# wiedenhoeft/HaMMLET

Hardware: AMD Instinct MI355X
Metric: block-updates/sec (Gibbs sweep) + HBM GB/s, 10^8 pos / 5 states (higher is better)
Workload: dtype f32; 1 GPU; c3_1e8_k5_dynamic; positions=100000000, states=5, block_structure=dynamic, chains=1, parallelism=chain-parallel x1

## Files before the change

### hammlet_amd/capi.py

```python
import ctypes as C
import os

import numpy as np

from . import build as _build

_lib = None


class HmlError(RuntimeError):
    def __init__(self, code, msg):
        super().__init__(msg)
        self.code = code


class HmlStats(C.Structure):
    _fields_ = [("sweeps", C.c_uint64), ("block_updates", C.c_uint64), ("uniform_fallbacks", C.c_uint64),
                ("forward_refits", C.c_uint64), ("forward_serial", C.c_uint64), ("forward_warmup", C.c_uint64),
                ("fused_fallbacks", C.c_uint64), ("buffer_growths", C.c_uint64), ("block_capacity", C.c_uint64)]


RECORD_CB = C.CFUNCTYPE(None, C.c_void_p, C.c_uint64, C.c_void_p)

_P = C.c_void_p
SIGNATURES = {
    "hml_last_error": (C.c_char_p, []),
    "hml_abi_version": (C.c_uint32, []),
    "hml_device_arch": (C.c_char_p, []),
    "hml_device_count": (C.c_int, [C.POINTER(C.c_int)]),
    "hml_create": (C.c_int, [C.POINTER(_P), C.c_int, C.c_uint64, C.c_uint32, _P]),
    "hml_destroy": (None, [_P]),
    "hml_load_observations": (C.c_int, [_P, _P, C.c_uint64]),
    "hml_load_observations_device": (C.c_int, [_P, _P, C.c_uint64]),
    "hml_attach_observations": (C.c_int, [_P, _P]),
    "hml_text_open": (C.c_int, [C.POINTER(_P), C.c_int, C.c_uint64]),
    "hml_text_close": (None, [_P]),
    "hml_text_buffer": (C.c_int, [_P, C.POINTER(_P), C.POINTER(C.c_uint64)]),
    "hml_text_commit": (C.c_int, [_P, C.c_uint64]),
    "hml_text_feed": (C.c_int, [_P, C.c_char_p, C.c_uint64]),
    "hml_text_reserve": (C.c_int, [_P, C.c_uint64]),
    "hml_text_finish": (C.c_int, [_P, C.POINTER(C.c_uint64), C.POINTER(C.c_int)]),
    "hml_text_values": (C.c_int, [_P, _P]),
    "hml_text_counters": (C.c_int, [_P, C.POINTER(C.c_uint64), C.POINTER(C.c_uint64), C.POINTER(C.c_uint64)]),
    "hml_set_dimensions": (C.c_int, [_P, C.c_int, C.c_int]),
    "hml_get_dimensions": (C.c_int, [_P, C.POINTER(C.c_int), C.POINTER(C.c_int)]),
    "hml_set_weights": (C.c_int, [_P, _P, C.c_uint64]),
    "hml_noise_sigma": (C.c_int, [_P, C.POINTER(C.c_double)]),
    "hml_scale_weights": (C.c_int, [_P, C.c_float]),
    "hml_autoprior": (C.c_int, [_P, C.c_float, C.c_float, _P]),
    "hml_set_model": (C.c_int, [_P, C.c_int, _P, C.c_float, C.c_float, C.c_float, C.c_int]),
    "hml_set_self_transitions": (C.c_int, [_P, C.c_int]),
    "hml_sample_prior": (C.c_int, [_P]),
    "hml_set_static_blocks": (C.c_int, [_P]),
    "hml_set_dynamic": (C.c_int, [_P, C.c_int]),
    "hml_create_blocks": (C.c_int, [_P, C.c_float]),
    "hml_iterate": (C.c_int, [_P, C.c_char, C.c_uint64, C.c_uint64]),
    "hml_iterate_many": (C.c_int, [_P, C.c_int, C.c_char, C.c_uint64, C.c_uint64]),
    "hml_set_recording": (C.c_int, [_P, C.c_int, RECORD_CB, _P]),
    "hml_set_option": (C.c_int, [_P, C.c_char_p, C.c_int]),
    "hml_sync": (C.c_int, [_P]),
    "hml_get_num_blocks": (C.c_int, [_P, C.POINTER(C.c_uint64)]),
    "hml_get_blocks": (C.c_int, [_P, _P]),
    "hml_get_block_stats": (C.c_int, [_P, _P, _P]),
    "hml_get_states": (C.c_int, [_P, _P]),
    "hml_get_theta": (C.c_int, [_P, _P]),
    "hml_get_transitions": (C.c_int, [_P, _P, _P]),
    "hml_set_parameters": (C.c_int, [_P, _P, _P, _P]),
    "hml_get_threshold": (C.c_int, [_P, C.POINTER(C.c_float)]),
    "hml_enable_probes": (C.c_int, [_P, C.c_int]),
    "hml_get_block_loglik": (C.c_int, [_P, _P]),
    "hml_get_forward_rows": (C.c_int, [_P, _P]),
    "hml_get_counts": (C.c_int, [_P, _P, _P, _P, _P, _P]),
    "hml_get_weights": (C.c_int, [_P, _P]),
    "hml_get_coefficients": (C.c_int, [_P, _P]),
    "hml_get_integral_array": (C.c_int, [_P, _P, _P]),
    "hml_marginals_rle": (C.c_int, [_P, C.POINTER(C.c_uint64), C.POINTER(C.c_int), _P, _P]),
    "hml_max_segmentation": (C.c_int, [_P, C.POINTER(C.c_uint64), _P, _P]),
    "hml_marginals_dense_device": (C.c_int, [_P, _P, _P]),
    "hml_recorded_sweeps": (C.c_int, [_P, C.POINTER(C.c_uint64)]),
    "hml_set_level_recording": (C.c_int, [_P, C.c_int]),
    "hml_levels_rle": (C.c_int, [_P, C.POINTER(C.c_uint64), C.POINTER(C.c_uint64), _P, _P, _P]),
    "hml_levels_dense_device": (C.c_int, [_P, _P]),
    "hml_levels_merge": (C.c_int, [_P, _P]),
    "hml_levels_on_segments": (C.c_int, [_P, C.c_uint64, _P, _P, _P]),
    "hml_levels_agreement_rle": (C.c_int, [_P, C.c_int, C.POINTER(C.c_uint64), C.POINTER(C.c_uint64), _P, _P, _P, _P]),
    "hml_levels_agreement_dense_device": (C.c_int, [_P, C.c_int, _P]),
    "hml_levels_agreement_summary": (C.c_int, [_P, C.c_int, C.c_double, _P, _P, _P]),
    "hml_set_break_recording": (C.c_int, [_P, C.c_int]),
    "hml_breaks_list": (C.c_int, [_P, C.POINTER(C.c_uint64), C.POINTER(C.c_uint64), _P, _P]),
    "hml_breaks_dense_device": (C.c_int, [_P, _P, C.c_uint32]),
    "hml_breaks_merge": (C.c_int, [_P, _P]),
    "hml_breaks_consensus": (C.c_int, [_P, C.c_uint32, C.c_uint64, C.POINTER(C.c_uint64), _P, _P, _P]),
    "hml_set_level_bands": (C.c_int, [_P, C.c_int, _P]),
    "hml_get_level_bands": (C.c_int, [_P, C.POINTER(C.c_int), _P]),
    "hml_bands_rle": (C.c_int, [_P, C.POINTER(C.c_uint64), C.POINTER(C.c_int), C.POINTER(C.c_uint64), _P, _P]),
    "hml_bands_dense_device": (C.c_int, [_P, _P, C.c_int]),
    "hml_bands_call": (C.c_int, [_P, C.c_uint64, C.POINTER(C.c_uint64), _P, _P]),
    "hml_bands_merge": (C.c_int, [_P, _P]),
    "hml_categorical_draw": (C.c_int, [_P, _P, C.c_int, C.POINTER(C.c_uint32)]),
    "hml_relabel_permutation": (C.c_int, [_P, _P]),
    "hml_pool_payload_size": (C.c_int, [_P, C.POINTER(C.c_uint64)]),
    "hml_pool_export": (C.c_int, [_P, _P, _P]),
    "hml_pool_install": (C.c_int, [_P, _P]),
    "hml_pool_unique_id": (C.c_int, [_P]),
    "hml_pool_create": (C.c_int, [C.POINTER(_P), C.c_int, C.c_int, C.c_int, _P]),
    "hml_pool_destroy": (None, [_P]),
    "hml_pool_marginals": (C.c_int, [_P, _P, _P]),
    "hml_pool_info": (C.c_int, [_P, C.POINTER(C.c_int), C.POINTER(C.c_int), C.POINTER(C.c_double), C.POINTER(C.c_uint64), C.POINTER(C.c_int)]),
    "hml_pool_set_form": (C.c_int, [_P, C.c_int]),
    "hml_pool_last": (C.c_int, [_P, C.POINTER(C.c_int), C.POINTER(C.c_uint64)]),
    "hml_allreduce_marginals": (C.c_int, [_P, C.c_int]),
    "hml_allreduce_marginals_perm": (C.c_int, [_P, C.c_int, _P]),
    "hml_pool_permutation": (C.c_int, [_P, _P]),
    "hml_get_stats": (C.c_int, [_P, C.POINTER(HmlStats)]),
    "hml_profile_enable": (C.c_int, [_P, C.c_int]),
    "hml_profile_get": (C.c_int, [_P, C.c_char_p, C.POINTER(C.c_double), C.POINTER(C.c_uint64)]),
    "hml_debug_eval": (C.c_int, [C.c_int, C.c_int, _P, _P, _P, C.c_uint64, C.c_uint64]),
    "hml_synth_depth": (C.c_int, [_P, _P, C.c_uint64, C.c_double, C.c_double, C.c_uint64, C.c_int]),
    "hml_synth_gauss": (C.c_int, [_P, _P, C.c_uint64, C.c_int, _P, C.c_float, C.c_double, C.c_uint64, C.c_int]),
}


ABI_VERSION = 5


def load_library(path=None):
    global _lib
    if _lib is not None and path is None:
        return _lib
    path = path or os.environ.get("HML_LIBRARY") or _build.LIB_PATH
    if not os.path.exists(path):
        raise HmlError(-1, "%s is missing: build it with `python -c 'import __graft_entry__ as g; g.build()'` "
                           "(hipcc --offload-arch=gfx950); there is no CPU fallback" % path)
    lib = C.CDLL(path, mode=C.RTLD_GLOBAL)
    for name, (res, args) in SIGNATURES.items():
        fn = getattr(lib, name)
        fn.restype = res
        fn.argtypes = args
    if lib.hml_abi_version() != ABI_VERSION:
        raise HmlError(-1, "%s has ABI version %d, this package expects %d: rebuild the library" % (path, lib.hml_abi_version(), ABI_VERSION))
    _lib = lib
    return lib


def _check(rc):
    if rc != 0:
        raise HmlError(rc, load_library().hml_last_error().decode())


def parse_text(source, device=0, chunk_bytes=0, feed_bytes=None, with_info=False):
    lib = load_library()
    h = _P()
    _check(lib.hml_text_open(C.byref(h), device, chunk_bytes))
    try:
        if isinstance(source, (bytes, bytearray, memoryview)):
            data = bytes(source)
            step = feed_bytes or max(len(data), 1)
            for i in range(0, len(data), step):
                part = data[i:i + step]
                _check(lib.hml_text_feed(h, part, len(part)))
        else:
            with open(source, "rb", buffering=0) as f:
                while True:
                    buf, cap = _P(), C.c_uint64()
                    _check(lib.hml_text_buffer(h, C.byref(buf), C.byref(cap)))
                    view = (C.c_char * cap.value).from_address(buf.value)
                    n = f.readinto(view)
                    if not n:
                        break
                    _check(lib.hml_text_commit(h, n))
        n, stopped = C.c_uint64(), C.c_int()
        _check(lib.hml_text_finish(h, C.byref(n), C.byref(stopped)))
        out = np.empty(n.value, np.float32)
        _check(lib.hml_text_values(h, out.ctypes.data))
        if not with_info:
            return out
        a, b, c = C.c_uint64(), C.c_uint64(), C.c_uint64()
        _check(lib.hml_text_counters(h, C.byref(a), C.byref(b), C.byref(c)))
        return out, {"stopped": bool(stopped.value), "bytes": a.value, "irregular_tokens": b.value, "host_chunks": c.value}
    finally:
        lib.hml_text_close(h)


def synth_gauss(T, K, mu, sigma, dwell, seed, nthreads=8, with_states=False):
    lib = load_library()
    x = np.empty(T, np.float32)
    mu = np.ascontiguousarray(mu, np.float32)
    st = np.empty(T, np.int16) if with_states else None
    _check(lib.hml_synth_gauss(x.ctypes.data, st.ctypes.data if with_states else None, T, K, mu.ctypes.data, sigma,
                               dwell, seed, nthreads))
    return (x, st) if with_states else x


def synth_depth(T, depth=15.0, ln_sigma=0.15, seed=5, nthreads=8, with_states=False):
    lib = load_library()
    x = np.empty(T, np.float32)
    st = np.empty(T, np.int16) if with_states else None
    _check(lib.hml_synth_depth(x.ctypes.data, st.ctypes.data if with_states else None, T, depth, ln_sigma, seed, nthreads))
    return (x, st) if with_states else x


def debug_eval(fn, a, b=None, seed=0, device=0):
    lib = load_library()
    a = np.ascontiguousarray(a, np.float32)
    out = np.empty_like(a)
    if b is not None:
        b = np.ascontiguousarray(b, np.float32)
    _check(lib.hml_debug_eval(device, fn, a.ctypes.data, b.ctypes.data if b is not None else None, out.ctypes.data, a.size, seed))
    return out


class Chain:

    def __init__(self, device=0, seed=0, chain_id=0, stream=None):
        self.lib = load_library()
        h = _P()
        _check(self.lib.hml_create(C.byref(h), device, seed, chain_id, stream))
        self.h = h
        self.K = None
        self.T = None
        self.D = 1
        self.P = None
        self._cb = None

    def close(self):
        if self.h:
            self.lib.hml_destroy(self.h)
            self.h = None

    def __del__(self):
        try:
            self.close()
        except Exception:
            pass

    def set_dimensions(self, D, P):
        _check(self.lib.hml_set_dimensions(self.h, D, P))
        self.D, self.P = D, P

    def load(self, x):
        x = np.ascontiguousarray(x, np.float32)
        self.T = int(x.size) // self.D
        _check(self.lib.hml_load_observations(self.h, x.ctypes.data, x.size))

    def load_device(self, ptr, T):
        self.T = int(T)
        _check(self.lib.hml_load_observations_device(self.h, ptr, T))

    def attach(self, source):
        _check(self.lib.hml_attach_observations(self.h, source.h))
        self.T, self.D, self.P = source.T, source.D, source.P

    def noise_sigma(self):
        v = C.c_double()
        _check(self.lib.hml_noise_sigma(self.h, C.byref(v)))
        return v.value

    def scale_weights(self, m):
        _check(self.lib.hml_scale_weights(self.h, m))

    def set_weights(self, w):
        w = np.ascontiguousarray(w, np.float32)
        _check(self.lib.hml_set_weights(self.h, w.ctypes.data, w.size))

    def autoprior(self, s2=0.2, p=0.9):
        out = np.empty(4, np.float32)
        _check(self.lib.hml_autoprior(self.h, s2, p, out.ctypes.data))
        return out

    def set_model(self, K, nig4, a_off=0.5, a_diag=0.5, pi_alpha=0.5, self_trans=True):
        nig4 = np.ascontiguousarray(nig4, np.float32)
        self.K = K
        _check(self.lib.hml_set_model(self.h, K, nig4.ctypes.data, a_off, a_diag, pi_alpha, 1 if self_trans else 0))

    def sample_prior(self):
        _check(self.lib.hml_sample_prior(self.h))

    def set_self_transitions(self, on=True):
        _check(self.lib.hml_set_self_transitions(self.h, 1 if on else 0))

    def set_static_blocks(self):
        _check(self.lib.hml_set_static_blocks(self.h))

    def set_dynamic(self, on=True):
        _check(self.lib.hml_set_dynamic(self.h, 1 if on else 0))

    def create_blocks(self, thr):
        _check(self.lib.hml_create_blocks(self.h, thr))

    def iterate(self, method, iterations, thinning=0):
        _check(self.lib.hml_iterate(self.h, method.encode()[0:1], iterations, thinning))

    def set_recording(self, marginals=True, callback=None):
        if callback is not None:
            def tramp(_ctx, sweep, _user):
                callback(self, sweep)
            self._cb = RECORD_CB(tramp)
        else:
            self._cb = C.cast(None, RECORD_CB)
        _check(self.lib.hml_set_recording(self.h, 1 if marginals else 0, self._cb, None))

    def set_option(self, name, value):
        _check(self.lib.hml_set_option(self.h, name.encode(), int(value)))

    def sync(self):
        _check(self.lib.hml_sync(self.h))

    def num_blocks(self):
        v = C.c_uint64()
        _check(self.lib.hml_get_num_blocks(self.h, C.byref(v)))
        return v.value

    def blocks(self):
        B = self.num_blocks()
        s = np.empty(B + 1, np.uint32)
        _check(self.lib.hml_get_blocks(self.h, s.ctypes.data))
        return s

    def block_stats(self):
        B = self.num_blocks()
        a = np.empty((self.D, B), np.float32)
        b = np.empty((self.D, B), np.float32)
        _check(self.lib.hml_get_block_stats(self.h, a.ctypes.data, b.ctypes.data))
        return (a[0], b[0]) if self.D == 1 else (a, b)

    def states(self):
        B = self.num_blocks()
        q = np.empty(B, np.int16)
        _check(self.lib.hml_get_states(self.h, q.ctypes.data))
        return q

    def theta(self):
        t = np.empty(2 * (self.P or self.K), np.float32)
        _check(self.lib.hml_get_theta(self.h, t.ctypes.data))
        return t

    def transitions(self):
        A = np.empty((self.K, self.K), np.float32)
        pi = np.empty(self.K, np.float32)
        _check(self.lib.hml_get_transitions(self.h, A.ctypes.data, pi.ctypes.data))
        return A, pi

    def set_parameters(self, mean_var, A, pi):
        mv = np.ascontiguousarray(mean_var, np.float32)
        A = np.ascontiguousarray(A, np.float32)
        pi = np.ascontiguousarray(pi, np.float32)
        _check(self.lib.hml_set_parameters(self.h, mv.ctypes.data, A.ctypes.data, pi.ctypes.data))

    def threshold(self):
        v = C.c_float()
        _check(self.lib.hml_get_threshold(self.h, C.byref(v)))
        return v.value

    def enable_probes(self, on=True):
        _check(self.lib.hml_enable_probes(self.h, 1 if on else 0))

    def block_loglik(self):
        B = self.num_blocks()
        E = np.empty((B, self.K), np.float32)
        _check(self.lib.hml_get_block_loglik(self.h, E.ctypes.data))
        return E

    def forward_rows(self):
        B = self.num_blocks()
        r = np.empty((B + 1, self.K), np.float32)
        _check(self.lib.hml_get_forward_rows(self.h, r.ctypes.data))
        return r

    def counts(self):
        K = self.K
        trans = np.empty((K, K), np.uint64)
        occ = np.empty(K, np.uint64)
        s = np.empty(K, np.float32)
        q = np.empty(K, np.float32)
        n = np.empty(K, np.uint64)
        _check(self.lib.hml_get_counts(self.h, trans.ctypes.data, occ.ctypes.data, s.ctypes.data, q.ctypes.data, n.ctypes.data))
        return trans, occ, s, q, n

    def weights(self):
        w = np.empty(self.T, np.float32)
        _check(self.lib.hml_get_weights(self.h, w.ctypes.data))
        return w

    def coefficients(self):
        w = np.empty(self.T, np.float32)
        _check(self.lib.hml_get_coefficients(self.h, w.ctypes.data))
        return w

    def integral_array(self):
        a = np.empty(self.T + 1, np.float32)
        b = np.empty(self.T + 1, np.float32)
        _check(self.lib.hml_get_integral_array(self.h, a.ctypes.data, b.ctypes.data))
        return a, b

    def recorded_sweeps(self):
        v = C.c_uint64()
        _check(self.lib.hml_recorded_sweeps(self.h, C.byref(v)))
        return v.value

    def marginals_rle(self):
        n = C.c_uint64()
        k = C.c_int()
        _check(self.lib.hml_marginals_rle(self.h, C.byref(n), C.byref(k), None, None))
        seg = np.empty(n.value, np.uint64)
        cnt = np.empty((n.value, max(k.value, 0)), np.int32)
        _check(self.lib.hml_marginals_rle(self.h, C.byref(n), C.byref(k), seg.ctypes.data, cnt.ctypes.data if k.value else None))
        return seg, cnt

    def max_segmentation(self):
        n = C.c_uint64()
        _check(self.lib.hml_max_segmentation(self.h, C.byref(n), None, None))
        ln = np.empty(n.value, np.uint64)
        st = np.empty(n.value, np.int32)
        _check(self.lib.hml_max_segmentation(self.h, C.byref(n), ln.ctypes.data, st.ctypes.data))
        return ln, st

    def marginals_dense_device(self, out_ptr, perm=None):
        p = None
        if perm is not None:
            perm = np.ascontiguousarray(perm, np.int32)
            p = perm.ctypes.data
        _check(self.lib.hml_marginals_dense_device(self.h, out_ptr, p))

    def set_level_recording(self, on=True):
        _check(self.lib.hml_set_level_recording(self.h, 1 if on else 0))

    def levels_rle(self):
        m, n = C.c_uint64(), C.c_uint64()
        _check(self.lib.hml_levels_rle(self.h, C.byref(m), C.byref(n), None, None, None))
        seg = np.empty(m.value, np.uint64)
        s1 = np.empty((self.D, m.value), np.float64)
        s2 = np.empty((self.D, m.value), np.float64)
        _check(self.lib.hml_levels_rle(self.h, C.byref(m), C.byref(n), seg.ctypes.data, s1.ctypes.data, s2.ctypes.data))
        return seg, n.value, s1, s2

    def levels_dense_device(self, out_ptr):
        _check(self.lib.hml_levels_dense_device(self.h, out_ptr))

    def merge_levels(self, other):
        _check(self.lib.hml_levels_merge(self.h, other.h))

    def levels_on_segments(self, cuts):
        cuts = np.ascontiguousarray(cuts, np.uint32)
        n = cuts.size
        s1 = np.empty((self.D, n + 1), np.float64)
        s2 = np.empty((self.D, n + 1), np.float64)
        _check(self.lib.hml_levels_on_segments(self.h, n, cuts.ctypes.data if n else None, s1.ctypes.data, s2.ctypes.data))
        return s1, s2

    def set_break_recording(self, on=True):
        _check(self.lib.hml_set_break_recording(self.h, 1 if on else 0))

    def breaks_list(self):
        m, n = C.c_uint64(), C.c_uint64()
        _check(self.lib.hml_breaks_list(self.h, C.byref(m), C.byref(n), None, None))
        pos = np.empty(m.value, np.uint32)
        cnt = np.empty(m.value, np.uint32)
        if m.value:
            _check(self.lib.hml_breaks_list(self.h, C.byref(m), C.byref(n), pos.ctypes.data, cnt.ctypes.data))
        return pos, cnt, n.value

    def breaks_dense(self, out_ptr, window=0):
        _check(self.lib.hml_breaks_dense_device(self.h, out_ptr, window))

    def breaks_merge(self, other):
        _check(self.lib.hml_breaks_merge(self.h, other.h))

    def breaks_consensus(self, window, min_count):
        s = C.c_uint64()
        _check(self.lib.hml_breaks_consensus(self.h, window, min_count, C.byref(s), None, None, None))
        pos = np.empty(s.value, np.uint32)
        mass = np.empty(s.value, np.uint64)
        peak = np.empty(s.value, np.uint32)
        if s.value:
            _check(self.lib.hml_breaks_consensus(self.h, window, min_count, C.byref(s), pos.ctypes.data, mass.ctypes.data, peak.ctypes.data))
        return pos, mass, peak

    def set_level_bands(self, edges):
        edges = np.ascontiguousarray(edges, np.float32)
        _check(self.lib.hml_set_level_bands(self.h, edges.size, edges.ctypes.data if edges.size else None))

    def level_bands(self):
        n = C.c_int()
        edges = np.zeros(31, np.float32)
        _check(self.lib.hml_get_level_bands(self.h, C.byref(n), edges.ctypes.data))
        return edges[:n.value].copy()

    def bands_rle(self):
        m, ncol, n = C.c_uint64(), C.c_int(), C.c_uint64()
        _check(self.lib.hml_bands_rle(self.h, C.byref(m), C.byref(ncol), C.byref(n), None, None))
        seg = np.empty(m.value, np.uint64)
        cnt = np.empty((m.value, ncol.value), np.int32)
        _check(self.lib.hml_bands_rle(self.h, C.byref(m), C.byref(ncol), C.byref(n), seg.ctypes.data, cnt.ctypes.data))
        return seg, cnt, n.value

    def bands_dense_device(self, out_ptr, cumulative=False):
        _check(self.lib.hml_bands_dense_device(self.h, out_ptr, 1 if cumulative else 0))

    def bands_call(self, rank=0):
        r = C.c_uint64()
        _check(self.lib.hml_bands_call(self.h, rank, C.byref(r), None, None))
        ln = np.empty(r.value, np.uint64)
        band = np.empty((self.D, r.value), np.int32)
        _check(self.lib.hml_bands_call(self.h, rank, C.byref(r), ln.ctypes.data, band.ctypes.data))
        return ln, band

    def merge_bands(self, other):
        _check(self.lib.hml_bands_merge(self.h, other.h))

    def relabel_permutation(self):
        perm = np.empty(self.K, np.int32)
        _check(self.lib.hml_relabel_permutation(self.h, perm.ctypes.data))
        return perm

    def pool_payload_size(self):
        n = C.c_uint64()
        _check(self.lib.hml_pool_payload_size(self.h, C.byref(n)))
        return n.value

    def pool_export(self, payload_ptr):
        perm = np.empty(self.K, np.int32)
# ... 197 lines not shown
```

### hammlet_amd/csrc/hml_capi.hip

```cpp
#include "hml_capi_shared.hpp"

static thread_local std::string g_err;
int hml_set_err(int code, const std::string& msg) { g_err = msg; return code; }

static const hml_ktab* ktab(int K);
#define HML_KTAB(KV, tab) const hml_ktab* tab = ktab(KV); if (!tab) return set_err(HML_ERR_ARG, "number of states must be in [2,16]")

std::atomic<int> hml_live_ctx[64];
int hml_ctx_bind(hml_ctx* c) { return ctx_bind(c); }
int hml_ctx_fetch_model(hml_ctx* c, hml_model* out) { return fetch_model(c, out); }

HML_KERNEL void hml_k_debug_eval(int fn, const float* __restrict__ a, const float* __restrict__ b, float* __restrict__ out,
                                 uint64_t n, uint64_t seed) {
    if (fn == 24) {
        const uint64_t nw = ((uint64_t)gridDim.x * blockDim.x) >> 6;
        if ((threadIdx.x & 63) != 0) return;
        for (uint64_t i = ((uint64_t)blockIdx.x * blockDim.x + threadIdx.x) >> 6; i < n; i += nw) {
            hml_dev_src src;
            src.s = hml_stream_open(hml_make_key(seed, 0), HML_KIND_THETA, seed, (uint32_t)i);
            out[i] = hml_gamma_f32<hml_devmath>(src, a[i], b[i]);
        }
        return;
    }
    const uint64_t stride = (uint64_t)gridDim.x * blockDim.x;
// ... 3 lines not shown
        switch (fn) {
            case 0: r = hml_expf(x); break;
            case 1: r = hml_logf(x); break;
            case 2: r = hml_powf_unit(x, y); break;
            case 3: r = HML_SQRTF(x); break;
            case 4: r = x / y; break;
            case 5: {
                hml_dev_src src;
                src.s = hml_stream_open(hml_make_key(seed, 0), HML_KIND_THETA, seed, (uint32_t)i);
                r = hml_gamma_f32<hml_devmath>(src, x, y);
            } break;
            case 6: {
                hml_dev_src src;
                src.s = hml_stream_open(hml_make_key(seed, 0), HML_KIND_PI, seed, (uint32_t)i);
                hml_normal_f32<hml_devmath> nd;
                r = nd.draw(src, x, y);
            } break;
            case 7: r = (float)hml_log((double)x); break;
            case 8: r = (float)hml_exp_nonpos((double)x); break;
            case 9: r = (float)((double)x / (double)y); break;
            case 40: r = hml_glibc_expf(x); break;
            case 41: r = hml_glibc_logf(x); break;
            case 42: r = hml_glibc_powf_unit(x, y); break;
            case 43: { const double Zd = (double)y; r = hml_tr2_quotient(x, Zd, hml_tr2_reciprocal(Zd)); } break;
            case 10: r = (float)(1.0 / (double)x); break;
            case 12: case 13: case 14: case 15: case 16: case 17: case 18: case 19: case 20: case 21: case 22: case 23: {
                hml_dev_src src; src.s = hml_stream_open(hml_make_key(seed, 0), HML_KIND_THETA, seed, (uint32_t)i);
                const float alpha = x, beta = y; (void)beta;
                const float malpha = alpha < 1.0f ? alpha + 1.0f : alpha;
                const float a1 = malpha - 1.0f / 3.0f;
                const float a2 = 1.0f / hml_devmath::sqrtf_(9.0f * a1);
                hml_normal_f32<hml_devmath> nd;
                float n = nd.draw(src, 0.0f, 1.0f);
                float v = 1.0f + a2 * n;
                float v3 = v * v * v;
                float u = hml_canonical_f32(src);
                const bool c1 = (double)u > (double)1.0f - 0.0331 * (double)n * (double)n * (double)n * (double)n;
                const bool c2 = ((double)hml_devmath::logf_(u) > (0.5 * (double)n * (double)n + (double)a1 * ((1.0 - (double)v3) + (double)hml_devmath::logf_(v3))));
                float n2 = nd.draw(src, 0.0f, 1.0f);
                float vb = 1.0f + a2 * n2;
                float vb3 = vb * vb * vb;
                float ub = hml_canonical_f32(src);
                const bool d1 = (double)ub > (double)1.0f - 0.0331 * (double)n2 * (double)n2 * (double)n2 * (double)n2;
                const bool d2 = ((double)hml_devmath::logf_(ub) > (0.5 * (double)n2 * (double)n2 + (double)a1 * ((1.0 - (double)vb3) + (double)hml_devmath::logf_(vb3))));
                r = fn == 12 ? n : fn == 13 ? v3 : fn == 14 ? u : fn == 15 ? (float)(c1 ? 1 : 0) + 2.0f * (c2 ? 1 : 0) : fn == 16 ? n2 : fn == 17 ? a2
                    : fn == 18 ? vb3 : fn == 19 ? ub : fn == 20 ? (float)(d1 ? 1 : 0) + 2.0f * (d2 ? 1 : 0) : fn == 21 ? (float)src.s.n : 0.0f;
                if (fn == 22) r = nd.draw(src, 0.0f, 1.0f);
                if (fn == 23) { hml_normal_f32<hml_devmath> nf; r = nf.draw(src, 0.0f, 1.0f); r = nf.draw(src, 0.0f, 1.0f); }
            } break;
            case 30: case 31: {
                r = 0.0f;
                const int Kc = fn == 30 ? 16 : 5;
                if (i % Kc == 0 && i + Kc <= n) {
                    bool unsure = false;
                    int fastr, lit;
                    if (fn == 30) { float w[16]; for (int j = 0; j < 16; ++j) w[j] = a[i + j]; fastr = hml_categorical_k_fast<16>(w, (double)y, unsure); lit = hml_categorical_k_literal<16>(w, (double)y); if (unsure) fastr = lit; }
                    else { float w[5]; for (int j = 0; j < 5; ++j) w[j] = a[i + j]; fastr = hml_categorical_k_fast<5>(w, (double)y, unsure); lit = hml_categorical_k_literal<5>(w, (double)y); if (unsure) fastr = lit; }
                    out[i] = (float)fastr; out[i + 1] = (float)lit; out[i + 2] = unsure ? 1.0f : 0.0f;
                }
                continue;
            }
            case 11: { const double d = HML_SQRT((double)x * 1.0000001); r = (float)((d - (double)(float)d) * 1e9); } break;
        }
        out[i] = r;
    }
}

static bool parse_band_edges(const char* text, int* n, float* edges) {
    *n = 0;
    const char* p = text;
    while (*p) {
        char* end = nullptr;
        const float v = strtof(p, &end);
        if (end == p || *n >= HML_MAX_BAND_EDGES) return false;
        edges[(*n)++] = v;
        p = end;
        if (*p == ',') ++p; else if (*p) return false;
    }
    return *n > 0;
}

static const char* band_edges_fault(int n, const float* edges) {
    if (n < 1 || n > HML_MAX_BAND_EDGES) return "level bands take 1 to 31 edges";
    for (int j = 0; j < n; ++j) {
        if (!std::isfinite(edges[j])) return "the edges of the level bands must be finite";
        if (j > 0 && !(edges[j - 1] < edges[j])) return "the edges of the level bands must be strictly ascending";
    }
    return nullptr;
}

static int bands_from_env(hml_ctx* c) {
    if (const char* e = getenv("HML_BANDS")) {
        int n = 0; float edges[HML_MAX_BAND_EDGES];
        if (!parse_band_edges(e, &n, edges)) return set_err(HML_ERR_ARG, "HML_BANDS: expected up to 31 comma-separated numbers");
        if (const char* why = band_edges_fault(n, edges)) return set_err(HML_ERR_ARG, std::string("HML_BANDS: ") + why);
        c->n_band_edges = n;
        memcpy(c->band_edges, edges, (size_t)n * sizeof(float));
        c->rec[HML_REC_BANDS].on = c->rec[HML_REC_BANDS].asked = true;
    }
    return 0;
}

extern "C" {

const char* hml_last_error(void) { return g_err.c_str(); }
uint32_t hml_abi_version(void) { return 5; }
const char* hml_device_arch(void) { return "gfx950"; }
int hml_device_count(int* n) {
    if (!n) return set_err(HML_ERR_ARG, "null argument");
    HIPCHK(hipGetDeviceCount(n));
    return 0;
}

static void free_all(hml_ctx* c);

static int create_inner(hml_ctx* c, void* stream) {
    HIPCHK(hipSetDevice(c->device));
    if (stream) { c->stream = (hipStream_t)stream; c->own_stream = false; }
    else { HIPCHK(hipStreamCreateWithFlags(&c->stream, hipStreamNonBlocking)); c->own_stream = true; }
    HIPCHK(hipMalloc(&c->d_mdl, sizeof(hml_model)));
    HIPCHK(hipMemsetAsync(c->d_mdl, 0, sizeof(hml_model), c->stream));
    HIPCHK(hipHostMalloc(&c->h_B, 4 * sizeof(uint32_t), hipHostMallocMapped));
    c->h_B[0] = 0; c->h_B[1] = 0; c->h_B[2] = 0; c->h_B[3] = 0;
    HIPCHK(hipHostGetDevicePointer((void**)&c->d_hB, c->h_B, 0));
    return 0;
}

int hml_create(hml_ctx** out, int device, uint64_t seed, uint32_t chain_id, void* stream) {
    if (!out) return set_err(HML_ERR_ARG, "null output pointer");
    int n = 0;
    HIPCHK(hipGetDeviceCount(&n));
    if (n <= 0) return set_err(HML_ERR_HIP, "no HIP device available: the MI355X kernels cannot run (there is no CPU fallback)");
    if (device < 0 || device >= n) return set_err(HML_ERR_ARG, "device index out of range");
    hml_ctx* c = new hml_ctx();
    c->device = device; c->seed = seed; c->chain = chain_id;
    if (int r = create_inner(c, stream)) {
        free_all(c);
        if (c->own_stream && c->stream) hipStreamDestroy(c->stream);
        delete c;
        return r;
    }
    if (const char* e = getenv("HML_FWD_CHUNK")) { int l = std::max(1, atoi(e)); int sh = 0; while ((1 << (sh + 1)) <= l && sh < 10) ++sh; c->fwdL = 1 << sh; }
    if (const char* e = getenv("HML_FWD_WARMUP")) c->fwdW = c->fwdW_init = std::max(0, atoi(e));
    if (const char* e = getenv("HML_FWD_BURNIN_SWEEPS")) c->fwd_burnin_sweeps = (uint32_t)std::max(0, atoi(e));
    if (const char* e = getenv("HML_FWD_QUIET")) c->fwd_quiet_need = (uint32_t)std::max(1, atoi(e));
    if (const char* e = getenv("HML_FWD_CHUNK_MANY")) { int l = std::max(1, atoi(e)); int sh = 0; while ((1 << (sh + 1)) <= l && sh < 6) ++sh; c->fwdL_many = 1 << sh; }
    if (const char* e = getenv("HML_FWD_CHUNK_MID")) { int l = std::max(1, atoi(e)); int sh = 0; while ((1 << (sh + 1)) <= l && sh < 10) ++sh; c->fwdL_mid = 1 << sh; }
    if (const char* e = getenv("HML_MID_MIN_BLOCKS")) c->mid_min_blocks = (uint32_t)strtoul(e, nullptr, 10);
    if (const char* e = getenv("HML_FWD_CHUNK_DENSE")) { int l = std::max(1, atoi(e)); int sh = 0; while ((1 << (sh + 1)) <= l && sh < 10) ++sh; c->fwdL_dense = 1 << sh; }
    if (const char* e = getenv("HML_DENSE_MIN_BLOCKS")) c->dense_min_blocks = (uint32_t)strtoul(e, nullptr, 10);
    if (const char* e = getenv("HML_USE_GRAPH")) c->use_graph = atoi(e) != 0;
    if (const char* e = getenv("HML_WEIGHT_KEYS")) c->use_keys = atoi(e) != 0;
    if (const char* e = getenv("HML_FUSED_BLOCKS")) { c->fused_blocks = atoi(e) != 0; c->fused_keep = atoi(e) == 2; }
    if (const char* e = getenv("HML_TRELLIS_FUSED")) c->tre_fused = atoi(e) != 0;
    if (const char* e = getenv("HML_TRELLIS_L")) { const int l = atoi(e); c->tre_L = (l <= 0) ? 0u : (l >= HML_TRE_MAX_L) ? (uint32_t)HML_TRE_MAX_L : (l < 32) ? 32u : (uint32_t)l / 32u * 32u; }
    if (const char* e = getenv("HML_TRELLIS_CKPT")) c->tre_ckpt = atoi(e) != 0;
    if (const char* e = getenv("HML_TRELLIS_REFIT_ROUNDS")) { const int r = atoi(e); c->tre_refit_rounds = r < 0 ? 0u : r > 6 ? 6u : (uint32_t)r; }
    if (const char* e = getenv("HML_STAGE_BITS")) c->stage_bits = atoi(e) != 0;
    if (const char* e = getenv("HML_TRELLIS_ROWS")) c->tre_rows = atoi(e) != 0;
    if (const char* e = getenv("HML_LATE_RESCALE")) c->late_rescale = atoi(e) != 0;
    if (const char* e = getenv("HML_PARAMS_SPREAD")) c->params_spread = atoi(e) != 0;
    if (const char* e = getenv("HML_COMPAT_CHUNKS")) c->compat_chunks = atoi(e);
    if (const char* e = getenv("HML_COMPAT_WARMUP")) c->compat_warmup = atoi(e);
    if (const char* e = getenv("HML_WIDE_LANES")) c->wide_lanes = atoi(e);
    if (const char* e = getenv("HML_WIDE_W0")) c->wide_w0 = std::max(8, atoi(e));
    if (const char* e = getenv("HML_WIDE_MAX_CHUNKS")) c->wide_max_chunks = (uint32_t)std::max(64, atoi(e));
    if (const char* e = getenv("HML_WIDE_L")) {
        const int L = atoi(e);
        if (L >= 1) { int sh = 0; while ((1 << sh) < L && sh < 20) ++sh; c->wide_lshift = sh; }
    }
    if (const char* e = getenv("HML_COMPAT")) c->compat = atoi(e) != 0;
    if (const char* e = getenv("HML_TRELLIS_TUNE")) c->tre_autotune = atoi(e) != 0;
    if (const char* e = getenv("HML_FUSED_SPIN_LIMIT")) c->fused_spin_limit = (uint32_t)strtoul(e, nullptr, 10);
    if (const char* e = getenv("HML_LEVELS")) c->rec[HML_REC_LEVELS].on = c->rec[HML_REC_LEVELS].asked = atoi(e) != 0;
    if (const char* e = getenv("HML_BREAKS")) c->rec[HML_REC_BREAKS].on = c->rec[HML_REC_BREAKS].asked = atoi(e) != 0;
    if (const char* e = getenv("HML_MAX_BLOCKS")) c->cap_opt = strtoull(e, nullptr, 10);
    if (device < 64) g_live_ctx[device].fetch_add(1);
    if (int r = bands_from_env(c)) { hml_destroy(c); return r; }
    *out = c;
    return 0;
}

static void trace_release(hml_ctx* c) {
    if (c->trace) {
        if (c->trace->refs.fetch_sub(1) == 1) {
            void* ptrs[] = {c->trace->d_w, c->trace->d_summary, c->trace->d_coeff, c->trace->d_ia};
            for (void* p : ptrs) if (p) hipFree(p);
            delete c->trace;
        }
        c->trace = nullptr;
    } else {
        void* ptrs[] = {c->d_w, c->d_summary, c->d_coeff, c->d_ia};
        for (void* p : ptrs) if (p) hipFree(p);
    }
    c->d_w = nullptr; c->d_summary = nullptr; c->d_coeff = nullptr; c->d_ia = nullptr;
}
static bool trace_shared(const hml_ctx* c) { return c->trace && c->trace->refs.load() > 1; }

static void free_sweep_buffers(hml_ctx* c, bool keep_engine = false) {
    void** ptrs[] = {(void**)&c->d_em, (void**)&c->d_gsc, (void**)&c->d_rows, (void**)&c->d_entry, (void**)&c->d_exitA, (void**)&c->d_redo, (void**)&c->d_touched,
                     (void**)&c->d_fb, (void**)&c->d_smap, (void**)&c->d_cmap, (void**)&c->d_scmap, (void**)&c->d_super, (void**)&c->d_bentry2, (void**)&c->d_bentry,
                     (void**)&c->d_q, (void**)&c->d_partial, (void**)&c->d_redo2, (void**)&c->d_tre_bitmap, (void**)&c->d_tre_ckpt, (void**)&c->d_crows, (void**)&c->d_cchunk, (void**)&c->d_cdraws, (void**)&c->d_clists, (void**)&c->d_wacc, (void**)&c->d_wA};
    for (void** p : ptrs) if (*p) { hipFree(*p); *p = nullptr; }
    if (!keep_engine && c->d_mt) { hipFree(c->d_mt); c->d_mt = nullptr; }
}

static void free_all(hml_ctx* c) {
    trace_release(c);
    free_sweep_buffers(c);
    void* ptrs[] = {c->d_group_word, c->d_wave_total, c->d_stage, c->d_span_count, c->d_starts, c->d_bstat, c->d_eprobe, c->d_aprobe, c->d_coarse1,
                    c->d_diff, c->d_boundary, c->d_mdl, c->d_many};
    for (void* p : ptrs) if (p) hipFree(p);
    for (hml_recorder& r : c->rec) { if (r.d_acc) hipFree(r.d_acc); if (r.d_boundary) hipFree(r.d_boundary); }
    if (c->h_B) hipHostFree(c->h_B);
    c->h_B = nullptr;
}


void hml_destroy(hml_ctx* c) {
    if (!c) return;
    if (c->device < 64) g_live_ctx[c->device].fetch_sub(1);
    hipSetDevice(c->device);
    hipStreamSynchronize(c->stream);
    for (auto& kv : c->prof) for (auto& p : kv.second.pending) { hipEventDestroy(p.first); hipEventDestroy(p.second); }
    for (auto e : c->ev_pool) hipEventDestroy(e);
    if (c->graph_exec) hipGraphExecDestroy(c->graph_exec);
    free_all(c);
    if (c->own_stream) hipStreamDestroy(c->stream);
    delete c;
}

static int build_keys(hml_ctx* c) {
    if (!c->use_keys) return 0;
    const uint64_t T = c->T;
    if (!c->d_summary) {
        const uint64_t n_spans = (T + HML_SPAN - 1) / HML_SPAN;
        HIPCHK(hipMalloc(&c->d_summary, n_spans * (HML_SPAN / 16) + 16));
        HIPCHK(hipMemsetAsync(c->d_summary, 0, n_spans * (HML_SPAN / 16) + 16, c->stream));
    }
    const float thr0 = (float)(std::sqrt(2 * std::log((double)std::max<uint64_t>(T, 2))) * c->sigma * c->key_scale);
    uint32_t u; memcpy(&u, &thr0, 4);
    c->key_base = (std::isfinite(thr0) && thr0 > 0 ? (int32_t)(u >> 20) : (int32_t)(0x3f800000u >> 20)) - 128;
    hipLaunchKernelGGL(hml_k_build_summary, dim3(grid_for((T + 15) / 16, 256, 1, 65536)), dim3(256), 0, c->stream, c->d_w, T,
                       c->key_base, c->d_summary);
    KLAUNCH_CHECK();
    return 0;
}

HML_KERNEL void hml_k_max_inplace(float* __restrict__ a, const float* __restrict__ b, uint64_t n) {
    const uint64_t stride = (uint64_t)gridDim.x * blockDim.x;
    for (uint64_t i = (uint64_t)blockIdx.x * blockDim.x + threadIdx.x; i < n; i += stride) { const float x = a[i], y = b[i]; a[i] = (x < y) ? y : x; }
}

static int alloc_block_buffers(hml_ctx* c) {
    const uint64_t T = c->T;
    c->n_spans = (uint32_t)((T + HML_SPAN - 1) / HML_SPAN);
    HIPCHK(hipMalloc(&c->d_stage, (uint64_t)c->n_spans * HML_SPAN * sizeof(uint16_t)));
    HIPCHK(hipMalloc(&c->d_span_count, c->n_spans * sizeof(uint32_t)));
    HIPCHK(hipMalloc(&c->d_starts, (c->cap + 1) * sizeof(uint32_t)));
    HIPCHK(hipMalloc(&c->d_coarse1, ((c->n_spans + HML_GROUP_SPANS - 1) / HML_GROUP_SPANS + 1u) * sizeof(uint32_t)));
    {
        const uint64_t n_tiles = (T + HML_FUSED_SUB_POSITIONS - 1) / HML_FUSED_SUB_POSITIONS;
        HIPCHK(hipMalloc(&c->d_group_word, (n_tiles + 1) * sizeof(unsigned long long)));
        HIPCHK(hipMemsetAsync(c->d_group_word, 0, (n_tiles + 1) * sizeof(unsigned long long), c->stream));
        HIPCHK(hipMalloc(&c->d_wave_total, (n_tiles + 1) * (HML_FUSED_WAVES + 2) * sizeof(uint32_t)));
        if (getenv("HML_FUSED_DEBUG")) { HIPCHK(hipMalloc(&c->d_dbg, 4096 * 8 * 8)); HIPCHK(hipMemset(c->d_dbg, 0, 4096 * 8 * 8)); }
    }
    HIPCHK(hipMalloc(&c->d_bstat, c->cap * (uint64_t)c->D * sizeof(float2)));
    const uint32_t cap32 = (uint32_t)c->cap;
    HIPCHK(hipMemcpyAsync(&c->d_mdl->cap, &cap32, sizeof cap32, hipMemcpyHostToDevice, c->stream));
    return 0;
}

static void choose_capacity(hml_ctx* c, bool attached) {
    const uint64_t T = c->T;
    uint64_t cap = T;
    if (c->D == 1) {
        if (c->cap_opt) cap = c->cap_opt;
        else if (attached) cap = std::max<uint64_t>(1ull << 20, T / 16);
    }
    c->cap = std::min<uint64_t>(std::max<uint64_t>(cap, 64), T);
}

static int build_from_device_x(hml_ctx* c, const float* const* d_x, const float* const* h_x) {
    const uint64_t T = c->T;
    const int D = c->D;
    {
        trace_release(c);
        void** stale[] = {(void**)&c->d_stage, (void**)&c->d_span_count, (void**)&c->d_starts, (void**)&c->d_coarse1, (void**)&c->d_group_word, (void**)&c->d_wave_total, (void**)&c->d_bstat};
        for (void** q : stale) if (*q) { hipFree(*q); *q = nullptr; }
    }
    {
        const float sqrt2 = (float)std::sqrt(2.0);
        const float sqrt2half = (float)(sqrt2 / 2.0);
        double acc = 0; uint64_t cnt = 0;
        for (uint64_t i = 1; i < T; i += 2) {
            float mx = 0.0f;
            for (int d = 0; d < D; ++d) {
                const float df = std::abs(h_x[d][i - 1] - h_x[d][i]);
                const float cf = sqrt2half * df;
                mx = (mx < cf) ? cf : mx;
            }
            acc += mx;
            cnt++;
        }
        acc /= cnt;
// ... 633 lines not shown
        hipLaunchKernelGGL(HIP_KERNEL_NAME(hml_k_compat_backward<KC, PAD>), dim3(C), dim3(64), 0, s, c->d_mdl, c->d_crows, c->d_cdraws, c->d_q, ch);
        if (C > 1u) hipLaunchKernelGGL(HIP_KERNEL_NAME(hml_k_compat_backward_check<KC, PAD>), dim3(1), dim3(256), 0, s, c->d_mdl, c->d_crows, c->d_cdraws, c->d_q, ch, C);
    }
}

static int sweep_compat(hml_ctx* c, char method, bool record) {
    hipStream_t s = c->stream;
    if (c->dynamic || !c->blocks_valid) {
        if (int r = launch_compact(c, false, 0.0f)) return r;
        if (!c->dynamic) c->blocks_valid = true;
    }
    refresh_hint(c);
    const uint32_t hint = c->B_hint ? c->B_hint : (uint32_t)std::min<uint64_t>(c->T, 1u << 20);
    const int mix = method == HML_METHOD_MIXTURE ? 1 : 0;
    hml_mt_state* const mt = (hml_mt_state*)c->d_mt;
    hipLaunchKernelGGL(HIP_KERNEL_NAME(hml_k_compat_emission<hml_glibc_exp>), dim3(grid_for(hint, 256, 64, 16384)), dim3(256), 0, s, c->d_mdl, c->d_starts, c->d_bstat, c->d_em, c->d_gsc, mix,
                       c->probes ? c->d_eprobe : nullptr);
    if (mix) hipLaunchKernelGGL(hml_k_compat_mixture, dim3(1), dim3(64), 0, s, c->d_mdl, mt, c->d_em, c->d_q);
    else {
        float* const aprobe = c->probes ? c->d_aprobe : nullptr;
        uint32_t C = 1u;
        if (!c->probes && c->compat_chunks > 1) C = std::min<uint32_t>((uint32_t)c->compat_chunks, HML_COMPAT_MAX_CHUNKS);
        else if (!c->probes && c->compat_chunks == 0 && hint >= 8192u) C = std::min<uint32_t>((uint32_t)HML_COMPAT_MAX_CHUNKS, hint / 64u);
        hml_compat_chunks ch = chunk_views(c);
        ch.W = c->compat_warmup > 0 ? (uint32_t)c->compat_warmup : c->compat_warmup < 0 ? 0u : HML_CHUNK_W_ADAPTIVE;
        hipLaunchKernelGGL(hml_k_compat_draws, dim3(1), dim3(256), 0, s, c->d_mdl, mt, c->d_cdraws, 2u);
#define HML_COMPAT_FB(KC) case KC: launch_chunked_fb<KC, hml_glibc_exp, false>(c, s, C, ch, aprobe); break;
        switch (c->K <= HML_MAX_K ? c->K : 0) {
            HML_COMPAT_FB(2) HML_COMPAT_FB(3) HML_COMPAT_FB(4) HML_COMPAT_FB(5) HML_COMPAT_FB(6) HML_COMPAT_FB(7) HML_COMPAT_FB(8) HML_COMPAT_FB(9)
            HML_COMPAT_FB(10) HML_COMPAT_FB(11) HML_COMPAT_FB(12) HML_COMPAT_FB(13) HML_COMPAT_FB(14) HML_COMPAT_FB(15) HML_COMPAT_FB(16)
            default:
                if (c->K <= 32) launch_chunked_fb<32, hml_glibc_exp, true>(c, s, C, ch, aprobe);
                else launch_chunked_fb<64, hml_glibc_exp, true>(c, s, C, ch, aprobe);
        }
#undef HML_COMPAT_FB
    }
    hml_compat_lists pl;
    {
        const uint64_t tiles = (c->cap + HML_COMPAT_PART_TILE - 1) / HML_COMPAT_PART_TILE;
        char* base = (char*)c->d_clists;
        pl.sx = (float*)base; base += compat_list_entries(c) * sizeof(float);
        pl.sq = (float*)base; base += compat_list_entries(c) * sizeof(float);
        pl.n = (uint32_t*)base; base += compat_list_entries(c) * sizeof(uint32_t);
        pl.offdiag = (unsigned long long*)base; base += (uint64_t)HML_CAP_K * HML_CAP_K * sizeof(unsigned long long);
        pl.tile_count = (uint32_t*)base; base += tiles * c->K * sizeof(uint32_t);
        pl.state_off = (uint32_t*)base;
    }
    const int by_state = (c->D == 1 && c->T < (1ull << 31) && (c->compat_chunks > 1 || (c->compat_chunks == 0 && hint >= 8192u))) ? 1 : 0;
    if (by_state) {
        const unsigned tiles_now = (unsigned)(((uint64_t)hint + hint / 8 + HML_COMPAT_PART_TILE) / HML_COMPAT_PART_TILE);
        const unsigned tg = std::min<uint64_t>(std::max(1u, tiles_now), (c->cap + HML_COMPAT_PART_TILE - 1) / HML_COMPAT_PART_TILE);
        hipLaunchKernelGGL(hml_k_compat_part_count, dim3(tg), dim3(256), 0, s, c->d_mdl, c->d_q, pl);
        hipLaunchKernelGGL(hml_k_compat_part_scan, dim3(1), dim3(64), 0, s, c->d_mdl, pl);
        hipLaunchKernelGGL(hml_k_compat_part_scatter, dim3(tg), dim3(256), 0, s, c->d_mdl, c->d_q, c->d_starts, c->d_bstat, pl);
    }
    hipLaunchKernelGGL(hml_k_compat_update, dim3(1), dim3(by_state ? 256 : 64), 0, s, c->d_mdl, mt, c->d_starts, c->d_bstat, c->d_q, mix, pl, by_state);
    if (record && c->rec_marginals) {
        if (c->pooled) return set_err(HML_ERR_ARG, "the marginals of this context are pooled (common labels, several chains): further sweeps cannot be recorded into them");
        if (int r = ensure_marginal_buffers(c)) return r;
        hipLaunchKernelGGL(hml_k_record, dim3(grid_for(hint, 256, 64, 16384)), dim3(256), 0, s, c->d_q, c->d_starts, c->d_mdl, c->d_diff, c->d_boundary);
    }
    if (record) { if (int r = launch_recorders(c, s, hint)) return r; }
    KLAUNCH_CHECK();
    return 0;
}

static int sweep_wide(hml_ctx* c, char method, bool record) {
    hipStream_t s = c->stream;
    if (c->dynamic || !c->blocks_valid) {
        if (int r = launch_compact(c, false, 0.0f)) return r;
        if (!c->dynamic) c->blocks_valid = true;
    }
    refresh_hint(c);
    const uint32_t hint = c->B_hint ? c->B_hint : (uint32_t)std::min<uint64_t>(c->T, 1u << 20);
    const int mix = method == HML_METHOD_MIXTURE ? 1 : 0;
    const bool lanes = c->wide_lanes != 0 && !c->probes && !mix && c->compat_chunks == 0;
    if (lanes) {
        hml_compat_chunks ch = chunk_views(c);
        ch.W = c->compat_warmup > 0 ? (uint32_t)c->compat_warmup : c->compat_warmup < 0 ? 0u : HML_CHUNK_W_ADAPTIVE;
        const uint64_t room = (uint64_t)hint + hint / 4 + 1024;
        hipLaunchKernelGGL(hml_k_wl_prepare, dim3(1), dim3(256), 0, s, c->d_mdl, c->d_wA, c->wide_lshift, wide_max_chunks_of(c));
        hipLaunchKernelGGL(hml_k_wl_gtable, dim3(grid_for((uint64_t)c->K * HML_WL_GTAB, 256, 1, 512)), dim3(256), 0, s, c->d_mdl, c->d_wA + HML_WL_PITCH * HML_WL_PITCH);
        {
            ProfScope ps(c, "stats_emission");
            hipLaunchKernelGGL(hml_k_wl_emission, dim3(grid_for(room, 64 * HML_WL_EMIT_ROWS * 4, 1, 32768)), dim3(256), 0, s, c->d_mdl, c->d_starts, c->d_bstat, c->d_em, c->d_gsc, c->d_wA + HML_WL_PITCH * HML_WL_PITCH);
        }
        const uint64_t minL = c->wide_lshift >= 0 ? (1ull << c->wide_lshift) : (1ull << HML_WL_MIN_LSHIFT);
        const int tiles = grid_for(room, (int)std::min<uint64_t>(64 * minL, 1u << 30), 1, HML_WL_MAX_CHUNKS / 64);
#define HML_WL_FB(KC)                                                                                                                                   \
        case KC: {                                                                                                                                      \
            constexpr int KS = (KC <= 32) ? 32 : 64;                                                                                                    \
            {                                                                                                                                           \
                ProfScope ps(c, "forward");                                                                                                             \
                hipLaunchKernelGGL(HIP_KERNEL_NAME(hml_k_wl_forward<KC>), dim3(tiles), dim3(64), 0, s, c->d_mdl, c->d_wA, c->d_em, c->d_gsc, c->d_crows, ch, 0); \
                hipLaunchKernelGGL(hml_k_wl_forward_verify, dim3(grid_for(room / 16 * c->K, 256, 1, 4096)), dim3(256), 0, s, c->d_mdl, ch, 0);          \
                                      \
                hipLaunchKernelGGL(hml_k_wl_retry_decide, dim3(1), dim3(256), 0, s, c->d_mdl, ch);                                                      \
                hipLaunchKernelGGL(HIP_KERNEL_NAME(hml_k_wl_forward<KC>), dim3(tiles), dim3(64), 0, s, c->d_mdl, c->d_wA, c->d_em, c->d_gsc, c->d_crows, ch, 1); \
                hipLaunchKernelGGL(hml_k_wl_forward_verify, dim3(grid_for(room / 16 * c->K, 256, 1, 4096)), dim3(256), 0, s, c->d_mdl, ch, 1);          \
                hipLaunchKernelGGL(HIP_KERNEL_NAME(hml_k_wl_forward_check<KS>), dim3(1), dim3(256), 0, s, c->d_mdl, c->d_em, c->d_gsc, c->d_crows, ch);  \
            }                                                                                                                                           \
            {                                                                                                                                           \
                ProfScope ps(c, "backward_maps");                                                                                                       \
                hipLaunchKernelGGL(HIP_KERNEL_NAME(hml_k_wl_backward<KC>), dim3(tiles), dim3(64), 0, s, c->d_mdl, c->d_crows, c->d_q, ch);               \
                hipLaunchKernelGGL(hml_k_wl_backward_verify, dim3(grid_for(room / 16, 256, 1, 256)), dim3(256), 0, s, c->d_mdl, ch);                     \
                hipLaunchKernelGGL(HIP_KERNEL_NAME(hml_k_wl_backward_check<KS>), dim3(1), dim3(256), 0, s, c->d_mdl, c->d_crows, c->d_q, ch);          \
            }                                                                                                                                           \
        } break;
        switch ((c->K + 3) / 4 * 4) {
            HML_WL_FB(4) HML_WL_FB(8) HML_WL_FB(12) HML_WL_FB(16)
            HML_WL_FB(20) HML_WL_FB(24) HML_WL_FB(28) HML_WL_FB(32) HML_WL_FB(36) HML_WL_FB(40) HML_WL_FB(44) HML_WL_FB(48) HML_WL_FB(52) HML_WL_FB(56)
            HML_WL_FB(60) HML_WL_FB(64)
            default: return set_err(HML_ERR_HIP, "internal error: a model of this many states on the path for more than 16");
        }
#undef HML_WL_FB
    } else {
    {
        ProfScope ps(c, "stats_emission");
        hipLaunchKernelGGL(hml_k_wide_emission, dim3(grid_for(hint, 256, 1, 4096)), dim3(256), 0, s, c->d_mdl, c->d_starts, c->d_bstat,
                           c->d_em, c->d_gsc, mix, c->probes ? c->d_eprobe : nullptr);
    }
    if (mix) hipLaunchKernelGGL(hml_k_wide_mixture, dim3(grid_for(hint, 256, 1, 16384)), dim3(256), 0, s, c->d_mdl, c->d_em, c->d_q);
    else {
        float* const aprobe = c->probes ? c->d_aprobe : nullptr;
        uint32_t C = 1u;
        if (!c->probes && c->compat_chunks > 1) C = std::min<uint32_t>((uint32_t)c->compat_chunks, HML_COMPAT_MAX_CHUNKS);
        else if (!c->probes && c->compat_chunks == 0 && hint >= 2048u) C = std::min<uint32_t>((uint32_t)HML_COMPAT_MAX_CHUNKS, hint / 64u);
        hml_compat_chunks ch = chunk_views(c);
        ch.W = c->compat_warmup > 0 ? (uint32_t)c->compat_warmup : c->compat_warmup < 0 ? 0u : HML_CHUNK_W_ADAPTIVE;
        hipLaunchKernelGGL(hml_k_wide_uniforms, dim3(grid_for((hint + 1u) / 2u, 256, 1, 4096)), dim3(256), 0, s, c->d_mdl, c->d_cdraws);
        if (c->K <= 32) launch_chunked_fb<32, hml_dev_exp, true>(c, s, C, ch, aprobe);
        else launch_chunked_fb<64, hml_dev_exp, true>(c, s, C, ch, aprobe);
    }
    }
    {
        ProfScope ps(c, "counts");
        hipLaunchKernelGGL(hml_k_wide_counts, dim3(HML_REDUCE_GROUPS), dim3(256), 0, s, c->d_q, c->d_starts, c->d_bstat, c->d_mdl, c->d_partial, (hml_wide_acc*)c->d_wacc);
    }
    if (record && c->rec_marginals) {
        if (c->pooled) return set_err(HML_ERR_ARG, "the marginals of this context are pooled (common labels, several chains): further sweeps cannot be recorded into them");
        if (int r = ensure_marginal_buffers(c)) return r;
        hipLaunchKernelGGL(hml_k_record, dim3(grid_for(hint, 256, 64, 16384)), dim3(256), 0, s, c->d_q, c->d_starts, c->d_mdl, c->d_diff, c->d_boundary);
    }
    {
        ProfScope ps(c, "params");
        hipLaunchKernelGGL(hml_k_wide_params, dim3(1), dim3(1024), 0, s, c->d_mdl, c->d_partial, (hml_wide_acc*)c->d_wacc, 0);
    }
    if (record) { if (int r = launch_recorders(c, s, hint)) return r; }
    KLAUNCH_CHECK();
    return 0;
}

static int sweep_dispatch(hml_ctx* c, char method, bool record) {
    if (c->compat) return sweep_compat(c, method, record);
    if (c->wide) return sweep_wide(c, method, record);
    HML_KTAB(c->K, kt);
    return kt->sweep(c, method, record);
}

extern "C" {

int hml_iterate(hml_ctx* c, char method, uint64_t iterations, uint64_t thinning) {
    if (!c || !c->model_set) return set_err(HML_ERR_ARG, "model not set");
    if (method != HML_METHOD_FB && method != HML_METHOD_MIXTURE)
        return set_err(HML_ERR_ARG, std::string("Unknown sampling type ") + method + "!");
    if (int r = ctx_bind(c)) return r;
    c->call_base = c->requested;
    if (thinning > 0 && thinning <= iterations && c->rec_marginals && c->pooled)
        return set_err(HML_ERR_ARG, "the marginals of this context are pooled (common labels, several chains): further sweeps cannot be recorded into them");
    for (uint64_t i = 0; i < iterations; ++i) {
        const bool record = thinning > 0 && ((i + 1) % thinning == 0);
        if (chain_halted(c)) { if (int r = hml_settle(c)) return r; }
        refresh_hint(c);
        const bool tre_path = c->tre_fused && c->D == 1 && method == HML_METHOD_FB && c->B_hint >= c->dense_min_blocks;
        if (c->use_graph && !c->compat && !record && !c->profiling && !c->probes && (c->dynamic || c->blocks_valid) &&
            !(tre_path && tre_wants_measurement(c, c->B_hint))) {
            const uint32_t hint = c->B_hint;
            bool unused = false;
            const bool wants_fused = c->fused_blocks && !(c->h_B[1] && !c->fused_keep) && !shares_device(c);
            const bool stale = !c->graph_exec || c->graph_method != method || c->graph_dynamic != c->dynamic ||
                               hint > c->graph_hint || hint * 2u < c->graph_hint || c->graph_fused != wants_fused ||
                               c->graph_dense != (hint >= c->dense_min_blocks) || c->graph_mid != (hint >= c->mid_min_blocks) ||
                               (tre_path && c->graph_tre_L != tre_pick_L(c, hint, true, &unused));
            if (stale && hint) {
                if (c->graph_exec) { hipGraphExecDestroy(c->graph_exec); c->graph_exec = nullptr; }
                hipGraph_t g = nullptr;
                HIPCHK(hipStreamBeginCapture(c->stream, hipStreamCaptureModeThreadLocal));
                int rr = sweep_dispatch(c, method, false);
                const hipError_t ec = hipStreamEndCapture(c->stream, &g);
                if (rr || ec != hipSuccess) {
                    if (g) hipGraphDestroy(g);
                    (void)hipGetLastError();
                    return rr ? rr : set_err(HML_ERR_HIP, std::string("hipStreamEndCapture: ") + hipGetErrorString(ec));
                }
                const hipError_t ei = hipGraphInstantiate(&c->graph_exec, g, nullptr, nullptr, 0);
                hipGraphDestroy(g);
                if (ei != hipSuccess) { c->graph_exec = nullptr; return set_err(HML_ERR_HIP, std::string("hipGraphInstantiate: ") + hipGetErrorString(ei)); }
                c->graph_method = method; c->graph_dynamic = c->dynamic; c->graph_hint = c->B_hint; c->graph_fused = wants_fused;
                c->graph_dense = c->B_hint >= c->dense_min_blocks;
                c->graph_mid = c->B_hint >= c->mid_min_blocks;
            }
            if (c->graph_exec) {
                log_sweep(c, method, false);
                HIPCHK(hipGraphLaunch(c->graph_exec, c->stream));
                if (tre_path) c->tre_dense_sweeps++;
                continue;
            }
        }
        log_sweep(c, method, record);
        if (int r = sweep_dispatch(c, method, record)) return r;
        if (record && c->cb) {
            HIPCHK(hipStreamSynchronize(c->stream));
            if (chain_halted(c)) { if (int r = hml_settle(c)) return r; continue; }
            if (int r = check_device_error(c)) return r;
            c->cb(c, i, c->cb_user);
        }
    }
    return 0;
}

}

extern "C" int hml_iterate_many(hml_ctx* const* cs, int n, char method, uint64_t iterations, uint64_t thinning) {
    if (!cs || n < 1) return set_err(HML_ERR_ARG, "no contexts");
    for (int i = 0; i < n; ++i) if (!cs[i] || !cs[i]->model_set) return set_err(HML_ERR_ARG, "model not set");
    if (method != HML_METHOD_FB && method != HML_METHOD_MIXTURE) return set_err(HML_ERR_ARG, std::string("Unknown sampling type ") + method + "!");
    for (int i = 0; i < n; ++i) cs[i]->call_base = cs[i]->requested;
    uint64_t done = 0;
    while (done < iterations && many_eligible(cs, n, method)) {
        if (int r = ctx_bind(cs[0])) return r;
        for (int i = 0; i < n; ++i) {
            hml_ctx* c = cs[i];
            if (int r = settle_if_limited(c)) return r;
            if (c->hint_stale) { launch_compact_pair(c, 0, 0.0f); KLAUNCH_CHECK(); }
            HIPCHK(hipStreamSynchronize(c->stream));
            c->hint_stale = false;
            if (c->graph_exec) { hipGraphExecDestroy(c->graph_exec); c->graph_exec = nullptr; }
        }
        int r = 0;
        uint64_t reached = done;
        { HML_KTAB(cs[0]->K, kt); r = kt->iterate_many(cs, n, done, iterations, thinning, &reached); }
        if (r) return r;
        hipEvent_t ev = ev_get(cs[0]);
        HIPCHK(hipEventRecord(ev, cs[0]->stream));
        for (int i = 1; i < n; ++i) HIPCHK(hipStreamWaitEvent(cs[i]->stream, ev, 0));
        cs[0]->ev_pool.push_back(ev);
        if (reached == iterations) return 0;
        HIPCHK(hipStreamSynchronize(cs[0]->stream));
        bool halted = false;
        for (int i = 0; i < n; ++i) halted = halted || chain_halted(cs[i]);
        const bool progress = reached > done;
        done = reached;
        if (!halted && !progress) break;
        if (!halted) { bool sparse = true; for (int i = 0; i < n; ++i) sparse = sparse && many_sparse(cs[i]); if (!sparse) break; }
    }
    for (int i = 0; i < n; ++i) if (int r = settle_if_limited(cs[i])) return r;
    for (uint64_t i = done; i < iterations; ++i) {
        const bool record = thinning > 0 && ((i + 1) % thinning == 0);
        for (int k = 0; k < n; ++k) {
            hml_ctx* c = cs[k];
            if (int r = ctx_bind(c)) return r;
            if (record && c->rec_marginals && c->pooled) return set_err(HML_ERR_ARG, "the marginals of a context are pooled (common labels, several chains): further sweeps cannot be recorded into them");
            if (chain_halted(c)) { if (int r = hml_settle(c)) return r; }
            log_sweep(c, method, record);
            if (int r = sweep_dispatch(c, method, record)) return r;
            if (record && c->cb) {
                HIPCHK(hipStreamSynchronize(c->stream));
                if (chain_halted(c)) { if (int r = hml_settle(c)) return r; continue; }
                if (int r = check_device_error(c)) return r;
                c->cb(c, i, c->cb_user);
            }
        }
    }
    return 0;
}

extern "C" {

int hml_set_option(hml_ctx* c, const char* name, int value) {
    if (!c || !name) return set_err(HML_ERR_ARG, "null argument");
    if (std::string(name) == "weight_keys") {
        if (c->loaded) return set_err(HML_ERR_ARG, "weight_keys must be set before the observations are loaded");
        c->use_keys = value != 0;
        c->summary_always = value == 2;
        return 0;
    }
    if (std::string(name) == "max_blocks") {
        if (c->loaded) return set_err(HML_ERR_ARG, "max_blocks must be set before the observations are loaded");
        if (value < 0) return set_err(HML_ERR_ARG, "max_blocks: a number of blocks, or 0 for the default");
        c->cap_opt = (uint64_t)value;
        return 0;
    }
    if (std::string(name) == "fused_blocks") {
        c->fused_blocks = value != 0;
        c->fused_keep = value == 2;
        if (c->graph_exec) { hipGraphExecDestroy(c->graph_exec); c->graph_exec = nullptr; }
        return 0;
    }
    if (std::string(name) == "compat") {
        if (c->model_set) return set_err(HML_ERR_ARG, "compat must be set before the model");
        c->compat = value != 0;
        return 0;
    }
    if (std::string(name) == "trellis_L") {
        if (value < 0 || value > HML_TRE_MAX_L || value % 32) return set_err(HML_ERR_ARG, "trellis_L: 0 or a multiple of 32 up to 1024");
        c->tre_L = (uint32_t)value;
        return 0;
    }
    return set_err(HML_ERR_ARG, std::string("unknown option ") + name);
}

int hml_sync(hml_ctx* c) {
    if (!c) return set_err(HML_ERR_ARG, "null context");
    if (int r = ctx_bind(c)) return r;
    if (int r = hml_settle(c)) return r;
    if (c->d_dbg && getenv("HML_FUSED_DEBUG") && atoi(getenv("HML_FUSED_DEBUG")) == 2) {
        std::vector<unsigned long long> h(4096 * 8);
        hipMemcpy(h.data(), c->d_dbg, h.size() * 8, hipMemcpyDeviceToHost);
        uint32_t n = 0; while (n < 4096 && h[n * 8]) ++n;
        unsigned long long t0 = ~0ull; for (uint32_t i = 0; i < n; ++i) t0 = std::min(t0, h[i * 8]);
        double mx[5] = {0, 0, 0, 0, 0}, av[5] = {0, 0, 0, 0, 0};
        if (n) for (uint32_t i = 0; i < n; ++i) for (int k = 0; k < 5; ++k) { const double d = (double)(h[i * 8 + k] - t0) * 0.01; mx[k] = std::max(mx[k], d); av[k] += d / n; }
        if (n) fprintf(stderr, "[fused-many dbg] n=%u start avg %.2f max %.2f | phaseA avg %.2f max %.2f | requested avg %.2f max %.2f | offsets avg %.2f max %.2f | end avg %.2f max %.2f (us)\n",
                n, av[0], mx[0], av[1], mx[1], av[2], mx[2], av[3], mx[3], av[4], mx[4]);
        if (n) for (uint32_t i : {0u, n / 4, n / 2, n - 1}) if (i < n) fprintf(stderr, "   wg %u: %.2f %.2f %.2f %.2f %.2f | wavefront 0: parameters in LDS %.2f, weights arrived %.2f, its lists done %.2f\n", i, (h[i*8]-t0)*0.01, (h[i*8+1]-t0)*0.01, (h[i*8+2]-t0)*0.01, (h[i*8+3]-t0)*0.01, (h[i*8+4]-t0)*0.01,
                                                                                  (h[i*8+5]-t0)*0.01, (h[i*8+6]-t0)*0.01, (h[i*8+7]-t0)*0.01);
    } else if (c->d_dbg) {
        std::vector<unsigned long long> h(4096 * 4);
        hipMemcpy(h.data(), c->d_dbg, h.size() * 8, hipMemcpyDeviceToHost);
        const uint32_t n = (uint32_t)std::min<uint64_t>(4096, (c->T + HML_FUSED_SUB_POSITIONS - 1) / HML_FUSED_SUB_POSITIONS);
        unsigned long long t0 = ~0ull; for (uint32_t i = 0; i < n; ++i) if (h[i * 4]) t0 = std::min(t0, h[i * 4]);
        double mx[4] = {0, 0, 0, 0}, av[4] = {0, 0, 0, 0};
        for (uint32_t i = 0; i < n; ++i) for (int k = 0; k < 4; ++k) { const double d = (double)(h[i * 4 + k] - t0) * 0.01; mx[k] = std::max(mx[k], d); av[k] += d / n; }
        fprintf(stderr, "[fused dbg] n=%u start avg %.2f max %.2f | phaseA avg %.2f max %.2f | offsets avg %.2f max %.2f | end avg %.2f max %.2f (us)\n", n, av[0], mx[0], av[1], mx[1], av[2], mx[2], av[3], mx[3]);
        { uint32_t late = 0, first_late = n; for (uint32_t i = 0; i < n; ++i) if ((h[i * 4] - t0) * 0.01 > 2.0) { ++late; first_late = std::min(first_late, i); }
          fprintf(stderr, "   late starters: %u, first index %u\n", late, first_late); }
        for (uint32_t i : {0u, n / 4, n / 2, n - 1}) fprintf(stderr, "   wg %u: %.2f %.2f %.2f %.2f\n", i, (h[i*4]-t0)*0.01, (h[i*4+1]-t0)*0.01, (h[i*4+2]-t0)*0.01, (h[i*4+3]-t0)*0.01);
    }
    if (c->model_set && getenv("HML_PARAMS_DEBUG")) {
        hml_model m;
        if (fetch_model(c, &m) == 0) {
            fprintf(stderr, "[params dbg] us since the kernel's start: accumulators read %.2f | tree %.2f | theta drawn %.2f | A gammas %.2f | barrier %.2f | end %.2f\n",
                    (m.dbg_t[1] - m.dbg_t[0]) * 0.01, (m.dbg_t[2] - m.dbg_t[0]) * 0.01, (m.dbg_t[3] - m.dbg_t[0]) * 0.01, (m.dbg_t[4] - m.dbg_t[0]) * 0.01,
                    (m.dbg_t[5] - m.dbg_t[0]) * 0.01, (m.dbg_t[6] - m.dbg_t[0]) * 0.01);
            fprintf(stderr, "[params dbg]   theta's gamma core + normal drawn %.2f | last wavefront's tree %.2f\n", (m.dbg_t[7] - m.dbg_t[0]) * 0.01, (m.dbg_t[8] - m.dbg_t[0]) * 0.01);
        }
    }
    if (c->model_set) return check_device_error(c);
    return 0;
}


static int current_B(hml_ctx* c, uint32_t* B) {
    HIPCHK(hipMemcpyAsync(c->h_B, &c->d_mdl->B, sizeof(uint32_t), hipMemcpyDeviceToHost, c->stream));
    HIPCHK(hipStreamSynchronize(c->stream));
    *B = *c->h_B;
    return 0;
}

int hml_get_num_blocks(hml_ctx* c, uint64_t* B) {
    NEED_LOADED();
    uint32_t b; if (int r = current_B(c, &b)) return r;
    *B = b; return 0;
}
int hml_get_blocks(hml_ctx* c, uint32_t* starts) {
    NEED_LOADED();
    uint32_t b; if (int r = current_B(c, &b)) return r;
    HIPCHK(hipMemcpy(starts, c->d_starts, ((uint64_t)b + 1) * sizeof(uint32_t), hipMemcpyDeviceToHost));
    return 0;
}
int hml_get_block_stats(hml_ctx* c, float* sum, float* sum_sq) {
    NEED_LOADED();
    uint32_t b; if (int r = current_B(c, &b)) return r;
    std::vector<float2> v(b);
    for (int d = 0; d < c->D; ++d) {
        HIPCHK(hipMemcpy(v.data(), c->d_bstat + (uint64_t)d * c->T, (uint64_t)b * sizeof(float2), hipMemcpyDeviceToHost));
        for (uint32_t i = 0; i < b; ++i) { sum[(uint64_t)d * b + i] = v[i].x; sum_sq[(uint64_t)d * b + i] = v[i].y; }
    }
    return 0;
}
int hml_get_states(hml_ctx* c, int16_t* q) {
    NEED_MODEL();
    uint32_t b; if (int r = current_B(c, &b)) return r;
    HIPCHK(hipMemcpy(q, c->d_q, (uint64_t)b * sizeof(int16_t), hipMemcpyDeviceToHost));
    return 0;
}
int hml_get_theta(hml_ctx* c, float* mean_var) {
    NEED_MODEL();
    hml_model m; if (int r = fetch_model(c, &m)) return r;
    for (int k = 0; k < m.P; ++k) { mean_var[2 * k] = m.mu[k]; mean_var[2 * k + 1] = m.var[k]; }
    return 0;
}
int hml_get_dimensions(hml_ctx* c, int* D, int* P) {
    if (!c) return set_err(HML_ERR_ARG, "null context");
    if (D) *D = c->D;
    if (P) *P = c->P > 0 ? c->P : c->K;
    return 0;
}
int hml_get_transitions(hml_ctx* c, float* A, float* pi) {
    NEED_MODEL();
    hml_model m; if (int r = fetch_model(c, &m)) return r;
    if (A) memcpy(A, m.A, (size_t)c->K * c->K * sizeof(float));
    if (pi) memcpy(pi, m.pi, (size_t)c->K * sizeof(float));
    return 0;
}
int hml_set_parameters(hml_ctx* c, const float* mean_var, const float* A, const float* pi) {
    NEED_MODEL();
    hml_model m; if (int r = fetch_model(c, &m)) return r;
    const int K = c->K;
    for (int k = 0; k < m.P; ++k) {
        const float mean = mean_var[2 * k], var = mean_var[2 * k + 1];
        if (!std::isfinite(mean)) return set_err(HML_ERR_MODEL, "Mean (" + std::to_string(mean) + ") must be set to a finite value!");
        if (!std::isfinite(var)) return set_err(HML_ERR_MODEL, "Variance(" + std::to_string(var) + ") must be set to a finite value!");
        if (var <= 0) return set_err(HML_ERR_MODEL, "Variance (" + std::to_string(var) + ") must be positive!");
        m.mu[k] = mean; m.var[k] = var; m.sd[k] = sqrtf(var);
    }
    memcpy(m.A, A, (size_t)K * K * sizeof(float));
    memcpy(m.pi, pi, (size_t)K * sizeof(float));
    HIPCHK(hipMemcpyAsync(c->d_mdl, &m, sizeof m, hipMemcpyHostToDevice, c->stream));
    if (c->compat) hipLaunchKernelGGL(hml_k_compat_derive, dim3(1), dim3(64), 0, c->stream, c->d_mdl);
    else if (c->wide) hipLaunchKernelGGL(hml_k_wide_derive, dim3(1), dim3(64), 0, c->stream, c->d_mdl);
    else { HML_KTAB(K, kt); kt->derive(c); }
    KLAUNCH_CHECK();
    HIPCHK(hipStreamSynchronize(c->stream));
    if (c->dynamic) c->blocks_valid = false;
    return 0;
}
int hml_get_threshold(hml_ctx* c, float* thr) {
    NEED_MODEL();
    hml_model m; if (int r = fetch_model(c, &m)) return r;
    *thr = m.thr; return 0;
}
int hml_get_block_loglik(hml_ctx* c, float* E) {
    NEED_MODEL();
    if (!c->probes) return set_err(HML_ERR_ARG, "probes are not enabled");
    uint32_t b; if (int r = current_B(c, &b)) return r;
    HIPCHK(hipMemcpy(E, c->d_eprobe, (uint64_t)b * c->K * sizeof(float), hipMemcpyDeviceToHost));
    return 0;
}
int hml_get_forward_rows(hml_ctx* c, float* rows) {
    NEED_MODEL();
    if (!c->probes) return set_err(HML_ERR_ARG, "probes are not enabled");
    uint32_t b; if (int r = current_B(c, &b)) return r;
    HIPCHK(hipMemcpy(rows, c->d_aprobe, ((uint64_t)b + 1) * c->K * sizeof(float), hipMemcpyDeviceToHost));
    return 0;
}
int hml_get_counts(hml_ctx* c, uint64_t* trans, uint64_t* occ, float* sum, float* sum_sq, uint64_t* nterms) {
    NEED_MODEL();
    hml_model m; if (int r = fetch_model(c, &m)) return r;
    const int K = c->K;
    for (int i = 0; i < K * K; ++i) trans[i] = m.last_trans[i];
    for (int k = 0; k < K; ++k) { occ[k] = m.last_occ[k]; nterms[k] = m.last_occ[k]; sum[k] = m.last_sum[k]; sum_sq[k] = m.last_sumsq[k]; }
    return 0;
}
int hml_get_weights(hml_ctx* c, float* w) {
    NEED_LOADED();
    HIPCHK(hipStreamSynchronize(c->stream));
    HIPCHK(hipMemcpy(w, c->d_w, c->T * sizeof(float), hipMemcpyDeviceToHost));
    return 0;
}
int hml_get_coefficients(hml_ctx* c, float* cf) {
    NEED_LOADED();
    HIPCHK(hipStreamSynchronize(c->stream));
    HIPCHK(hipMemcpy(cf, c->d_coeff, c->T * sizeof(float), hipMemcpyDeviceToHost));
    return 0;
}
int hml_get_integral_array(hml_ctx* c, float* sum, float* sum_sq) {
    NEED_LOADED();
    HIPCHK(hipStreamSynchronize(c->stream));
    std::vector<float2> v(c->T + 1);
    HIPCHK(hipMemcpy(v.data(), c->d_ia, (c->T + 1) * sizeof(float2), hipMemcpyDeviceToHost));
    for (uint64_t i = 0; i <= c->T; ++i) { sum[i] = v[i].x; sum_sq[i] = v[i].y; }
    return 0;
}

int hml_recorded_sweeps(hml_ctx* c, uint64_t* n) {
    NEED_MODEL();
    hml_model m; if (int r = fetch_model(c, &m)) return r;
    *n = m.n_recorded; return 0;
}

int hml_relabel_permutation(hml_ctx* c, int32_t* perm) {
    NEED_MODEL();
    if (!perm) return set_err(HML_ERR_ARG, "null argument");
    hml_model m; if (int r = fetch_model(c, &m)) return r;
    const int K = c->K, D = m.D;
    std::vector<int32_t> p(K);
    for (int k = 0; k < K; ++k) p[k] = k;
    std::stable_sort(p.begin(), p.end(), [&](int32_t a, int32_t b) {
        for (int d = 0; d < D; ++d) {
            const float ma = m.mu[m.map[a][d]], mb = m.mu[m.map[b][d]];
            if (ma < mb) return true;
            if (mb < ma) return false;
        }
        return false;
    });
    for (int k = 0; k < K; ++k) perm[k] = p[k];
    return 0;
}

int hml_categorical_draw(hml_ctx* c, const float* weights, int K, uint32_t* index) {
    if (!c || !weights || !index || K < 1) return set_err(HML_ERR_ARG, "invalid argument");
    if (K == 1) { *index = 0; return 0; }
    const uint64_t n = c->host_draws++;
    const hml_u32x4 o = hml_stream4(hml_make_key(c->seed, c->chain), HML_KIND_HOST, n >> 32, (uint32_t)n, 0);
    *index = (uint32_t)hml_categorical(weights, K, hml_canonical_f64(o.v[0], o.v[1]));
    return 0;
}

int hml_get_stats(hml_ctx* c, hml_stats* out) {
    NEED_MODEL();
    hml_model m; if (int r = fetch_model(c, &m)) return r;
    out->sweeps = m.sweeps; out->block_updates = m.block_updates; out->uniform_fallbacks = m.uniform_fallbacks;
    out->forward_refits = m.forward_refits; out->forward_serial = m.forward_serial;
    out->forward_warmup = m.fwd_W;
    out->fused_fallbacks = m.fused_fallbacks;
    out->buffer_growths = c->grown; out->block_capacity = c->cap;
    return 0;
}

int hml_profile_enable(hml_ctx* c, int on) {
    if (!c) return set_err(HML_ERR_ARG, "null context");
    if (on && c->ev_pool.size() < 64) {
        if (int r = ctx_bind(c)) return r;
        while (c->ev_pool.size() < 64) { hipEvent_t e; HIPCHK(hipEventCreate(&e)); c->ev_pool.push_back(e); }
    }
    c->profiling = on;
    return 0;
}

int hml_profile_get(hml_ctx* c, const char* name, double* total_ms, uint64_t* launches) {
    if (!c) return set_err(HML_ERR_ARG, "null context");
    if (int r = ctx_bind(c)) return r;
    HIPCHK(hipStreamSynchronize(c->stream));
    auto& acc = c->prof[name];
    for (auto& p : acc.pending) {
        float ms = 0;
        hipEventElapsedTime(&ms, p.first, p.second);
        acc.ms += ms; acc.n++;
        c->ev_pool.push_back(p.first); c->ev_pool.push_back(p.second);
    }
    acc.pending.clear();
    if (total_ms) *total_ms = acc.ms;
    if (launches) *launches = acc.n;
    return 0;
}

int hml_debug_eval(int device, int fn, const float* a, const float* b, float* out, uint64_t n, uint64_t seed) {
    HIPCHK(hipSetDevice(device));
    float *d_a = nullptr, *d_b = nullptr, *d_o = nullptr;
    HIPCHK(hipMalloc(&d_a, n * 4)); HIPCHK(hipMalloc(&d_o, n * 4));
    HIPCHK(hipMemcpy(d_a, a, n * 4, hipMemcpyHostToDevice));
    if (b) { HIPCHK(hipMalloc(&d_b, n * 4)); HIPCHK(hipMemcpy(d_b, b, n * 4, hipMemcpyHostToDevice)); }
    hipLaunchKernelGGL(hml_k_debug_eval, dim3(1024), dim3(256), 0, 0, fn, d_a, d_b, d_o, n, seed);
    KLAUNCH_CHECK();
    HIPCHK(hipMemcpy(out, d_o, n * 4, hipMemcpyDeviceToHost));
    hipFree(d_a); hipFree(d_o); if (d_b) hipFree(d_b);
    return 0;
}

int hml_synth_gauss(float* x, int16_t* states, uint64_t T, int K, const float* mu, float sigma, double mean_dwell,
                    uint64_t seed, int nthreads) {
    if (!x || !mu || K < 1) return set_err(HML_ERR_ARG, "invalid argument");
    hml_synth_gauss_trace(x, states, T, K, mu, sigma, mean_dwell, seed, nthreads);
    return 0;
}


int hml_synth_depth(float* x, int16_t* states, uint64_t T, double depth, double ln_sigma, uint64_t seed, int nthreads) {
    if (!x) return set_err(HML_ERR_ARG, "invalid argument");
    hml_synth_depth_trace(x, states, T, depth, ln_sigma, seed, nthreads);
    return 0;
}

}


#if defined(HML_ONLY_K)
#define HML_DECLARE_KTAB_(K) extern hml_ktab hml_ktab_##K; static const hml_ktab* ktab(int k) { return k == K ? &hml_ktab_##K : nullptr; }
#define HML_DECLARE_KTAB(K) HML_DECLARE_KTAB_(K)
HML_DECLARE_KTAB(HML_ONLY_K)
#else
#define HML_EXT_KTAB(K) extern hml_ktab hml_ktab_##K;
HML_EXT_KTAB(2) HML_EXT_KTAB(3) HML_EXT_KTAB(4) HML_EXT_KTAB(5) HML_EXT_KTAB(6) HML_EXT_KTAB(7) HML_EXT_KTAB(8) HML_EXT_KTAB(9)
HML_EXT_KTAB(10) HML_EXT_KTAB(11) HML_EXT_KTAB(12) HML_EXT_KTAB(13) HML_EXT_KTAB(14) HML_EXT_KTAB(15) HML_EXT_KTAB(16)
static const hml_ktab* ktab(int k) {
    static const hml_ktab* const tabs[17] = {nullptr, nullptr, &hml_ktab_2, &hml_ktab_3, &hml_ktab_4, &hml_ktab_5, &hml_ktab_6, &hml_ktab_7, &hml_ktab_8,
                                             &hml_ktab_9, &hml_ktab_10, &hml_ktab_11, &hml_ktab_12, &hml_ktab_13, &hml_ktab_14, &hml_ktab_15, &hml_ktab_16};
    return (k >= 2 && k <= 16) ? tabs[k] : nullptr;
}
#endif
```

### hammlet_amd/csrc/hml_ctx.hpp

```cpp
#ifndef HML_CTX_HPP
#define HML_CTX_HPP

#include <hip/hip_runtime.h>

#include <atomic>
#include <map>
#include <string>
#include <utility>
#include <vector>

#include "../../include/hml.h"
#include "hml_host_common.hpp"
#include "hml_state.h"

struct hml_trace {
    std::atomic<int> refs{1};
    float* d_w = nullptr;
    uint8_t* d_summary = nullptr;
    float* d_coeff = nullptr;
    float2* d_ia = nullptr;
};

struct ProfAcc { double ms = 0; uint64_t n = 0; uint32_t tick = 0; std::vector<std::pair<hipEvent_t, hipEvent_t>> pending; };

enum { HML_REC_LEVELS = 0, HML_REC_BREAKS = 1, HML_REC_BANDS = 2, HML_REC_KINDS = 3 };
struct hml_recorder {
    bool on = false;
    bool asked = false;
    void* d_acc = nullptr;
    uint32_t* d_boundary = nullptr;
    template <class E> E* acc() const { return static_cast<E*>(d_acc); }
};

struct hml_ctx {
    int device = 0;
    hipStream_t stream = nullptr;
    bool own_stream = false;
    uint64_t seed = 0;
    uint32_t chain = 0;
    uint64_t T = 0;
    int K = 0;
    int D = 1, P = 0;
    bool loaded = false, model_set = false;
    bool dynamic = true;
    bool blocks_valid = false;
    double sigma = 0;
    hml_trace* trace = nullptr;
    float* d_w = nullptr;
    uint8_t* d_summary = nullptr;
    int32_t key_base = 0;
    double key_scale = 1.0;
    bool use_keys = true;
    bool fused_blocks = true;
    uint64_t host_draws = 0;
    bool summary_always = false;
    float* d_coeff = nullptr;
    float2* d_ia = nullptr;
    uint16_t* d_stage = nullptr;
    uint32_t *d_span_count = nullptr, *d_starts = nullptr;
    float2* d_bstat = nullptr;
    uint32_t n_spans = 0;
    uint32_t* d_coarse1 = nullptr;
    unsigned long long* d_group_word = nullptr;
    uint32_t* d_wave_total = nullptr;
    int fused_slots = 0;
    uint32_t fused_spin_limit = 4096;
    bool fused_keep = false;
    unsigned long long* d_dbg = nullptr;
    bool use_graph = false;
    hipGraphExec_t graph_exec = nullptr;
    char graph_method = 0;
    uint32_t graph_hint = 0;
    bool graph_dynamic = false, graph_valid_blocks = false;
    bool graph_fused = false;
    float *d_em = nullptr, *d_gsc = nullptr, *d_rows = nullptr, *d_eprobe = nullptr, *d_aprobe = nullptr;
    float *d_entry = nullptr, *d_exitA = nullptr;
    uint32_t* d_redo = nullptr;
    uint32_t* d_redo2 = nullptr;
    uint32_t* d_tre_bitmap = nullptr;
    uint32_t* d_tre_ckpt = nullptr;
    bool late_rescale = true;
    uint32_t tre_L = 0;
    bool tre_autotune = true;
    uint32_t tre_tuned_L = 0, tre_tuned_hint = 0;
    int tre_tune_step = -1;
    float tre_tune_ms[8] = {0, 0, 0, 0, 0, 0, 0, 0};
    uint32_t tre_cand[8] = {0, 0, 0, 0, 0, 0, 0, 0};
    int tre_cand_n = 0;
    uint64_t tre_dense_sweeps = 0;
    uint32_t graph_tre_L = 0;
    int tre_slots = 0;
    bool stage_bits = true;
    uint32_t tre_refit_rounds = 2;
    bool tre_ckpt = true;
    bool tre_rows = true;
    bool tre_fused = true;
    uint32_t* d_touched = nullptr;
    uint32_t* d_fb = nullptr;
    unsigned long long *d_smap = nullptr, *d_cmap = nullptr;
    unsigned long long *d_scmap = nullptr, *d_super = nullptr;
    uint8_t *d_bentry = nullptr, *d_bentry2 = nullptr;
    int16_t* d_q = nullptr;
    double* d_partial = nullptr;
    bool params_spread = false;
    int32_t* d_diff = nullptr;
    uint32_t* d_boundary = nullptr;
    hml_recorder rec[HML_REC_KINDS];
    int n_band_edges = 0;
    float band_edges[31] = {};
    hml_model* d_mdl = nullptr;
    uint32_t* h_B = nullptr;
    uint64_t cap = 0;
    uint64_t cap_opt = 0;
    std::vector<uint8_t> sweep_log;
    unsigned long long log_base = 0;
    unsigned long long requested = 0;
    unsigned long long call_base = 0;
    uint64_t grown = 0;
    uint32_t* d_hB = nullptr;
    uint32_t B_hint = 0;
    bool hint_stale = true;
    int fwdL = 4, fwdW = 12;
    uint32_t fwd_burnin_sweeps = 64, fwd_quiet_need = 16;
    int fwdW_init = 24;
    hml_layout lay = {2, 0};
    int fwdL_dense = 16;
    hml_layout lay_dense = {4, 0};
    int fwdL_mid = 8;
    hml_layout lay_mid = {3, 0};
    uint32_t mid_min_blocks = 1u << 18;
    int fwdL_many = 8;
    hml_layout lay_many = {3, 0};
    uint32_t dense_min_blocks = 1u << 22;
    bool graph_dense = false, graph_mid = false;
    bool probes = false;
    bool rec_marginals = true;
    hml_record_cb cb = nullptr;
    void* cb_user = nullptr;
    int fm_slots = 0;
    void* d_many = nullptr;
    int many_cap = 0;
    bool compat = false;
    void* d_mt = nullptr;
    float* d_crows = nullptr;
    void* d_cchunk = nullptr;
    uint32_t* d_cdraws = nullptr;
    void* d_clists = nullptr;
    int compat_chunks = 0;
    int compat_warmup = 0;
    bool wide = false;
    void* d_wacc = nullptr;
    float* d_wA = nullptr;
    int wide_lanes = 1;
    int wide_w0 = 32;
    uint32_t wide_max_chunks = 0;
    uint64_t wide_chunks_cap = 0;
    int wide_lshift = -1;
    bool pooled = false;
    std::vector<int32_t> pool_perm;
    int profiling = 0;
    uint32_t prof_tick = 0;
    std::map<std::string, ProfAcc> prof;
    std::vector<hipEvent_t> ev_pool;
};

int hml_ctx_bind(hml_ctx* c);
int hml_ctx_fetch_model(hml_ctx* c, hml_model* out);
int hml_ctx_ensure_marginal_buffers(hml_ctx* c);
int hml_settle(hml_ctx* c);
int hml_ctx_gather_marginal_segments(hml_ctx* c, uint64_t* M, DevBuf& d_seg, DevBuf& d_g);

#endif
```

### hammlet_amd/csrc/hml_k_blocks_fused.h

```cpp
#ifndef HML_K_BLOCKS_FUSED_H
#define HML_K_BLOCKS_FUSED_H

#include "hml_k_blocks.h"
#include "hml_k_forward.h"

#define HML_FUSED_WAVES 8
#define HML_FUSED_WAVE_BATCH (HML_SUM_SPANS * HML_SPAN)
#define HML_FUSED_SUB_POSITIONS (HML_FUSED_WAVES * HML_FUSED_WAVE_BATCH)
#define HML_FUSED_MAX_SUB 4
#define HML_FUSED_POS_BITS 19
#define HML_FUSED_GEN_MASK ((1u << (64 - 2 * HML_FUSED_POS_BITS - 1)) - 1u)
#define HML_FUSED_WAVE_LIST 256
__device__ __forceinline__ unsigned long long hml_group_word(uint32_t gen, uint32_t total, uint32_t last_rel) {
    return ((unsigned long long)(gen & HML_FUSED_GEN_MASK) << (2 * HML_FUSED_POS_BITS + 1)) |
           ((unsigned long long)total << HML_FUSED_POS_BITS) | (unsigned long long)last_rel;
}
__device__ __forceinline__ uint32_t hml_fused_generation(const hml_model* mdl) { return ((uint32_t)mdl->epoch + 1u) & HML_FUSED_GEN_MASK; }

__device__ __forceinline__ unsigned long long hml_fused_tile_word(const uint8_t* __restrict__ summary, const float* __restrict__ w, uint32_t T,
                                                               float thr, int32_t base, uint32_t tile, uint32_t n_sub, uint32_t gen) {
    const uint32_t n_spans = (uint32_t)(((uint64_t)T + HML_SPAN - 1) / HML_SPAN);
    const uint32_t kthr = (thr != thr) ? 0u : hml_weight_key(thr, base);
    const uint32_t first_span = tile * (uint32_t)HML_FUSED_WAVES * n_sub * HML_SUM_SPANS;
    const uint32_t spans = (uint32_t)HML_FUSED_WAVES * n_sub * HML_SUM_SPANS;
    uint32_t total = 0u, last1 = 0u;
    for (uint32_t s = 0; s < spans && first_span + s < n_spans; ++s) {
        const uint32_t span = first_span + s;
        for (uint32_t g = 0; g < 256u; ++g) {
            const uint32_t key = summary[(uint64_t)span * 256u + (uint64_t)(g & 63u) * 4u + (g >> 6)];
            const bool origin = (span == 0u && g == 0u);
            if (key < kthr && !origin) continue;
            uint32_t m16 = hml_group_mask16(w, (uint64_t)span * HML_SPAN + (uint64_t)g * 16u, T, thr);
            if (origin) m16 |= 1u;
            if (m16) {
                total += (uint32_t)__popc(m16);
                last1 = s * HML_SPAN + g * 16u + (31u - (uint32_t)__clz((int)m16)) + 1u;
            }
        }
    }
    return hml_group_word(gen, total, last1 ? last1 - 1u : 0u);
}

template <int K>
HML_KERNEL __launch_bounds__(HML_FUSED_WAVES * 64, 6) void hml_k_blocks_fused(const uint8_t* __restrict__ summary, const float* __restrict__ w,
                                                          const float2* __restrict__ ia, uint32_t T,
                                                          hml_model* __restrict__ mdl, int32_t base,
                                                          unsigned long long* __restrict__ group_word,
                                                          uint16_t* __restrict__ stage, uint32_t* __restrict__ starts,
                                                          float2* __restrict__ bstat, float* __restrict__ em,
                                                          float* __restrict__ gsc, float* __restrict__ eprobe, int mixture,
                                                          const hml_layout lay, uint32_t* __restrict__ host_words,
                                                          uint32_t n_sub, uint32_t spin_limit, unsigned long long* __restrict__ dbg,
                                                          const hml_model* __restrict__ mdl_ro) {
    if (dbg && threadIdx.x == 0) dbg[blockIdx.x * 4 + 0] = wall_clock64();
    static_assert(HML_FUSED_MAX_SUB * HML_FUSED_SUB_POSITIONS == (1 << HML_FUSED_POS_BITS), "tile geometry (bit fields of hml_group_word)");
    static_assert(HML_FUSED_MAX_SUB * HML_FUSED_WAVE_BATCH <= 65536, "16-bit offsets into a wavefront's eighth");
    constexpr int NW = HML_FUSED_WAVES;
    constexpr uint32_t NT = NW * 64;
    __shared__ uint16_t listed_all[NW][HML_SUM_SPANS * 256];
    __shared__ uint16_t mask_all[NW][HML_SUM_SPANS * 256];
    __shared__ uint16_t wave_list[NW][HML_FUSED_WAVE_LIST];
    __shared__ uint32_t wave_total[NW], wave_last[NW];
    __shared__ unsigned long long red_sum[NW], red_near[NW];
    __shared__ uint64_t sm_exp_tab[32];
    if (threadIdx.x < 32u) sm_exp_tab[threadIdx.x] = HML_EXP2F_TAB[threadIdx.x];
    constexpr bool LOOPED = K > 6;
    __shared__ hml_emit_lds<LOOPED ? K : 1> sm_emit;
    if (LOOPED) hml_emit_lds_fill<LOOPED ? K : 1>(sm_emit, mdl_ro, (int)threadIdx.x);

    const int lane = threadIdx.x & 63, wave = threadIdx.x >> 6;
    const uint32_t g = blockIdx.x;
    const uint32_t n_spans = (uint32_t)(((uint64_t)T + HML_SPAN - 1) / HML_SPAN);
    const uint32_t eighth = n_sub * (uint32_t)HML_FUSED_WAVE_BATCH;
    const uint32_t tile_positions = eighth * (uint32_t)NW;
    const uint64_t wave_base = ((uint64_t)g * NW + (uint32_t)wave) * eighth;
    const uint32_t gen = hml_fused_generation(mdl_ro);
    uint16_t* listed = listed_all[wave];
    uint16_t* masks = mask_all[wave];
    const float thr = mdl_ro->thr;
    const uint32_t cap = mdl_ro->cap;

    uint32_t total = 0u, last1 = 0u;
    uint32_t placed = 0u;
    uint32_t n_listed = 0u, last_batch = 0u;
    auto expand = [&](uint32_t j, uint32_t n_l) {
        for (uint32_t i0 = 0; i0 < n_l; i0 += 64u) {
            const uint32_t i = i0 + (uint32_t)lane;
            uint32_t m16 = 0u, in_eighth = 0u;
            if (i < n_l) {
                const uint32_t sg = listed[i];
                m16 = masks[i];
                in_eighth = j * (uint32_t)HML_FUSED_WAVE_BATCH + (sg >> 8) * HML_SPAN + (sg & 255u) * 16u;
            }
            const uint32_t c = (uint32_t)__popc(m16);
            uint32_t r, sum;
            const unsigned long long some = __ballot(c != 0u);
            if (__ballot(c > 1u) == 0ull) {
                r = placed + hml_mbcnt(some);
                sum = (uint32_t)__popcll(some);
            } else {
                uint32_t incl = c;
#pragma unroll
                for (int d = 1; d < 64; d <<= 1) {
                    const uint32_t o = __shfl_up(incl, d);
                    if (lane >= d) incl += o;
                }
                r = placed + incl - c;
                sum = __shfl(incl, 63);
            }
            while (m16) {
                const int bit = __ffs(m16) - 1;
                m16 &= m16 - 1u;
                const uint16_t off = (uint16_t)(in_eighth + (uint32_t)bit);
                if (r < (uint32_t)HML_FUSED_WAVE_LIST) wave_list[wave][r] = off;
                else stage[wave_base + r] = off;
                ++r;
            }
            placed += sum;
        }
    };
    {
        const uint32_t kthr = (thr != thr) ? 0u : hml_weight_key(thr, base);
        const hml_swar_ge sw_ge = hml_swar_ge_make(kthr);
        auto load_batch = [&](uint32_t j, uint32_t (&gw)[HML_SUM_SPANS]) {
            const uint32_t span0 = (uint32_t)(wave_base / HML_SPAN) + j * HML_SUM_SPANS;
#pragma unroll
            for (int s = 0; s < HML_SUM_SPANS; ++s)
                gw[s] = (j < n_sub && span0 + s < n_spans)
                            ? __builtin_nontemporal_load(reinterpret_cast<const uint32_t*>(summary) + (uint64_t)(span0 + s) * 64u + lane)
                            : 0u;
        };
        uint32_t gw[HML_SUM_SPANS];
        load_batch(0u, gw);
        for (uint32_t j = 0; j < n_sub; ++j) {
            const uint32_t span0 = (uint32_t)(wave_base / HML_SPAN) + j * HML_SUM_SPANS;
            if (span0 >= n_spans) break;
            if (j > 0u) expand(j - 1u, n_listed);
            n_listed = 0u;
            last_batch = j;
#pragma unroll
            for (int s = 0; s < HML_SUM_SPANS; ++s) {
                const uint32_t fl = (span0 + s < n_spans) ? hml_swar_ge_apply(sw_ge, gw[s]) : 0u;
#pragma unroll
                for (int q = 0; q < 4; ++q) {
                    const bool open = ((fl >> (8 * q + 7)) & 1u) || (span0 + s == 0u && q == 0 && lane == 0);
                    const unsigned long long m = __ballot(open);
                    if (open) listed[n_listed + hml_mbcnt(m)] = (uint16_t)((s << 8) | (64 * q + lane));
                    n_listed += (uint32_t)__popcll(m);
                }
            }
            load_batch(j + 1u, gw);
            for (uint32_t i0 = 0; i0 < n_listed; i0 += 64u) {
                const uint32_t i = i0 + (uint32_t)lane;
                uint32_t m16 = 0u;
                if (i < n_listed) {
                    const uint32_t sg = listed[i];
                    const uint32_t in_batch = (sg >> 8) * HML_SPAN + (sg & 255u) * 16u;
                    m16 = hml_group_mask16(w, (uint64_t)span0 * HML_SPAN + in_batch, T, thr);
                    if (span0 == 0u && i == 0u) m16 |= 1u;
                    masks[i] = (uint16_t)m16;
                    if (m16) last1 = (uint32_t)wave * eighth + j * (uint32_t)HML_FUSED_WAVE_BATCH + in_batch + (31u - (uint32_t)__clz((int)m16)) + 1u;
                }
                total += (uint32_t)__popc(m16);
            }
        }
        total = hml_wave_sum_u32(total);
#pragma unroll
        for (int m = 1; m < 64; m <<= 1) { const uint32_t o = __shfl_xor(last1, m); last1 = o > last1 ? o : last1; }
    }
    if (lane == 0) { wave_total[wave] = total; wave_last[wave] = last1; }
    __syncthreads();
    if (dbg && threadIdx.x == 0) dbg[blockIdx.x * 4 + 1] = wall_clock64();
    uint32_t wg_total = 0u, wg_last1 = 0u;
#pragma unroll
    for (int k = 0; k < NW; ++k) {
        wg_total += wave_total[k];
        wg_last1 = wave_last[k] > wg_last1 ? wave_last[k] : wg_last1;
    }
    if (threadIdx.x == 0) {
        const uint32_t l1 = wg_last1;
        __hip_atomic_store(&group_word[g], hml_group_word(gen, wg_total, l1 ? l1 - 1u : 0u), __ATOMIC_RELAXED, __HIP_MEMORY_SCOPE_AGENT);
    }
    if ((uint32_t)(wave_base / HML_SPAN) < n_spans) expand(last_batch, n_listed);
    __syncthreads();

    auto start_at = [&](uint32_t k) -> uint32_t {
        uint32_t wv = 0u, first = 0u, run = 0u;
#pragma unroll
        for (int q = 0; q < NW - 1; ++q) {
            run += wave_total[q];
            if (k >= run) { wv = (uint32_t)q + 1u; first = run; }
        }
        const uint32_t idx = k - first;
        const uint64_t wb = ((uint64_t)g * NW + wv) * eighth;
        const uint32_t off = (idx < (uint32_t)HML_FUSED_WAVE_LIST) ? (uint32_t)wave_list[wv][idx] : (uint32_t)stage[wb + idx];
        return (uint32_t)(wb + off);
    };
    const bool last_wg = (g == gridDim.x - 1u);
    const uint32_t n_items = wg_total + (last_wg ? 1u : 0u);

    const uint32_t k_first = threadIdx.x;
    bool have_first = false;
    uint32_t first_t = 0u, first_n = 0u;
    float first_sx = 0.0f, first_sq = 0.0f;
    if (k_first > 0u && k_first < n_items) {
        first_t = (k_first < wg_total) ? start_at(k_first) : T;
        const uint32_t prev_t = start_at(k_first - 1u);
        first_n = first_t - prev_t;
        hml_block_stats_one(ia, prev_t, first_t, first_sx, first_sq);
        have_first = true;
    }

    unsigned long long acc = 0ull, near = 0ull;
    {
        for (uint32_t i = threadIdx.x; i < g; i += NT) {
            unsigned long long d = spin_limit ? __hip_atomic_load(&group_word[i], __ATOMIC_RELAXED, __HIP_MEMORY_SCOPE_AGENT)
                                              : hml_group_word(gen + 1u, 0u, 0u);
            uint32_t tries = 0u;
            while ((uint32_t)(d >> (2 * HML_FUSED_POS_BITS + 1)) != gen) {
                if (tries++ >= spin_limit) {
                    d = hml_fused_tile_word(summary, w, T, thr, base, i, n_sub, gen);
                    __hip_atomic_store(&group_word[i], d, __ATOMIC_RELAXED, __HIP_MEMORY_SCOPE_AGENT);
                    if (host_words) __hip_atomic_store(host_words + 1, 1u, __ATOMIC_RELAXED, __HIP_MEMORY_SCOPE_SYSTEM);
                    atomicAdd(&mdl->fused_fallbacks, 1ull);
                    break;
                }
                __builtin_amdgcn_s_sleep(1);
                d = __hip_atomic_load(&group_word[i], __ATOMIC_RELAXED, __HIP_MEMORY_SCOPE_AGENT);
            }
            const uint32_t tot = (uint32_t)(d >> HML_FUSED_POS_BITS) & ((2u << HML_FUSED_POS_BITS) - 1u);
            acc += tot;
            if (tot) near = ((unsigned long long)(i + 1u) << HML_FUSED_POS_BITS) | (d & ((1ull << HML_FUSED_POS_BITS) - 1ull));
        }
    }
#pragma unroll
    for (int m = 1; m < 64; m <<= 1) {
        acc += __shfl_xor(acc, m);
        const unsigned long long o = __shfl_xor(near, m);
        near = o > near ? o : near;
    }
    if (lane == 0) { red_sum[wave] = acc; red_near[wave] = near; }
    __syncthreads();
    if (dbg && threadIdx.x == 0) dbg[blockIdx.x * 4 + 2] = wall_clock64();
    unsigned long long sum_all = 0ull, nr = 0ull;
#pragma unroll
    for (int k = 0; k < NW; ++k) { sum_all += red_sum[k]; nr = red_near[k] > nr ? red_near[k] : nr; }
    const uint32_t before_group = (uint32_t)sum_all;
    const uint32_t prev_group_start =
        nr ? (uint32_t)(((nr >> HML_FUSED_POS_BITS) - 1ull) * tile_positions + (nr & ((1ull << HML_FUSED_POS_BITS) - 1ull))) : 0u;

    hml_emit_params<LOOPED ? 1 : K> p;
    if (!LOOPED) hml_emit_load<LOOPED ? 1 : K>(p, mdl_ro, mixture);
    const bool self_trans = mdl_ro->self_trans != 0;
    {
        uint32_t t = first_t, n = first_n;
        float sx = first_sx, sq = first_sq;
        bool gathered = have_first;
        for (uint32_t k = threadIdx.x; k < n_items; k += NT) {
            const uint32_t b = before_group + k;
            if (!gathered) {
                t = (k < wg_total) ? start_at(k) : T;
                if (t != 0u) {
                    const uint32_t prev_t = (k > 0u) ? start_at(k - 1u) : prev_group_start;
                    n = t - prev_t;
                    hml_block_stats_one(ia, prev_t, t, sx, sq);
                }
            }
            gathered = false;
            if (b > cap) continue;
            starts[b] = t;
            if (t == 0u) continue;
            bstat[b - 1u] = make_float2(sx, sq);
            if constexpr (LOOPED)
                hml_emit_block_looped<K>(reinterpret_cast<const hml_emit_lds<K>&>(sm_emit), mdl, self_trans, b - 1u, sx, sq, (float)n, em, gsc, eprobe, mixture, lay, sm_exp_tab);
            else
                hml_emit_block<LOOPED ? 1 : K, true>(p, mdl, b - 1u, sx, sq, (float)n, em, gsc, eprobe, mixture, lay, sm_exp_tab);
        }
    }
    if (dbg) { __syncthreads(); if (threadIdx.x == 0) dbg[blockIdx.x * 4 + 3] = wall_clock64(); }
    if (last_wg && threadIdx.x == 0) {
        const uint32_t Bn = before_group + wg_total;
        if (Bn > cap) { hml_halt(mdl, Bn, host_words); return; }
        mdl->B = Bn;
        hml_warmup_for_many_blocks(mdl, Bn);
        if (host_words) __hip_atomic_store(host_words, Bn, __ATOMIC_RELAXED, __HIP_MEMORY_SCOPE_SYSTEM);
    }
}

#endif
```

### hammlet_amd/csrc/hml_k_forward.h

```cpp
#ifndef HML_K_FORWARD_H
#define HML_K_FORWARD_H

#include "hml_k_blocks.h"
#include "hml_math.h"
#include "hml_state.h"

__device__ __forceinline__ void hml_raise(hml_model* mdl, uint32_t code, float value) {
    if (atomicCAS(&mdl->err_code, 0u, code) == 0u) mdl->err_value = value;
    atomicAdd(&mdl->err_count, 1ull);
}

__device__ __forceinline__ bool hml_isfinite(float x) { return (hml_f2u(x) & 0x7f800000u) != 0x7f800000u; }

template <int K>
struct hml_emit_params {
    float mu[K], var[K], logN[K], logA[K];
    double rvar[K];
    bool self;
};

__device__ __forceinline__ float hml_inner_product(float mu, float var, double rvar, float sx, float sq) {
    const double num = 2.0 * (double)mu * (double)sx - (double)sq;
    double ipd = num * rvar;
    const uint64_t bits = hml_d2u(ipd);
    const uint32_t low = (uint32_t)bits & 0x1fffffffu;
    const uint32_t ex = (uint32_t)(bits >> 52) & 0x7ffu;
    const bool close = (low - 0x0ffffffcu) <= 8u;
    if (close || ex < 923u || ex > 1150u) {
        if (ipd != 0.0 || close) ipd = num / (2.0 * (double)var);
    }
    return (float)ipd;
}

template <int K>
__device__ __forceinline__ void hml_emit_load(hml_emit_params<K>& p, const hml_model* mdl, int mixture) {
#pragma unroll
    for (int s = 0; s < K; ++s) { p.mu[s] = mdl->mu[s]; p.var[s] = mdl->var[s]; p.logN[s] = mdl->logN[s]; p.logA[s] = mdl->logA[s]; p.rvar[s] = mdl->rvar2[s]; }
    p.self = mdl->self_trans != 0 && !mixture;
}

template <int K, bool LEAN = false>
__device__ __forceinline__ void hml_emit_compute(const hml_emit_params<K>& p, hml_model* mdl, float sx, float sq, float N, int mixture,
                                                 float (&E)[K], float (&ev)[K], float (&gv)[K], bool want_g = true,
                                                 const uint64_t* exp_tab = nullptr) {
    const uint64_t* const tab = exp_tab ? exp_tab : HML_EXP2F_TAB;
    float maxE = -3.40282346638528859812e+38f;
#pragma unroll
    for (int s = 0; s < K; ++s) {
        const float ip = hml_inner_product(p.mu[s], p.var[s], p.rvar[s], sx, sq);
        if (!hml_isfinite(ip)) hml_raise(mdl, HML_DEVERR_IP_NOT_FINITE, ip);
        float e = (0.0f + ip) - N * p.logN[s];
        if (p.self) e += (N - 1.0f) * p.logA[s];
        E[s] = e;
        maxE = (e < maxE) ? maxE : e;
    }
#pragma unroll
    for (int s = 0; s < K; ++s) {
        ev[s] = LEAN ? hml_expf_lean(E[s] - maxE, tab) : hml_expf_tab(E[s] - maxE, tab);
        gv[s] = (want_g && !mixture && p.self) ? hml_expf_tab((N - 1.0f) * p.logA[s], tab) : 1.0f;
    }
}

template <int K>
__device__ __forceinline__ void hml_emit_store(uint32_t b, const float (&E)[K], const float (&ev)[K], const float (&gv)[K],
                                               float* __restrict__ em, float* __restrict__ gsc, float* __restrict__ eprobe,
                                               int mixture, const hml_layout lay) {
#pragma unroll
    for (int s = 0; s < K; ++s) {
        if (eprobe) eprobe[(uint64_t)b * K + s] = E[s];
        em[hml_bk(lay, b, K, s)] = ev[s];
        if (!mixture && gsc) gsc[hml_bk(lay, b, K, s)] = gv[s];
    }
}

template <int K, bool LEAN = false>
__device__ __forceinline__ void hml_emit_block(const hml_emit_params<K>& p, hml_model* mdl, uint32_t b, float sx, float sq,
                                               float N, float* __restrict__ em, float* __restrict__ gsc,
                                               float* __restrict__ eprobe, int mixture, const hml_layout lay,
                                               const uint64_t* exp_tab = nullptr) {
    float E[K], ev[K], gv[K];
    hml_emit_compute<K, LEAN>(p, mdl, sx, sq, N, mixture, E, ev, gv, gsc != nullptr, exp_tab);
    hml_emit_store<K>(b, E, ev, gv, em, gsc, eprobe, mixture, lay);
}

template <int K>
struct hml_emit_lds {
    float mu[K], var[K], logN[K], logA[K];
    double rvar[K];
};
template <int K>
__device__ __forceinline__ void hml_emit_lds_fill(hml_emit_lds<K>& l, const hml_model* mdl, int tid) {
    if (tid < K) { l.mu[tid] = mdl->mu[tid]; l.var[tid] = mdl->var[tid]; l.logN[tid] = mdl->logN[tid]; l.logA[tid] = mdl->logA[tid]; l.rvar[tid] = mdl->rvar2[tid]; }
}
template <int K>
__device__ __forceinline__ float hml_emit_E(const hml_emit_lds<K>& l, hml_model* mdl, int s, bool self, float sx, float sq, float N) {
    const float ip = hml_inner_product(l.mu[s], l.var[s], l.rvar[s], sx, sq);
    if (!hml_isfinite(ip)) hml_raise(mdl, HML_DEVERR_IP_NOT_FINITE, ip);
    float e = (0.0f + ip) - N * l.logN[s];
    if (self) e += (N - 1.0f) * l.logA[s];
    return e;
}
template <int K>
__device__ __forceinline__ void hml_emit_block_looped(const hml_emit_lds<K>& l, hml_model* mdl, bool self_trans, uint32_t b, float sx, float sq,
                                                      float N, float* __restrict__ em, float* __restrict__ gsc,
                                                      float* __restrict__ eprobe, int mixture, const hml_layout lay,
                                                      const uint64_t* exp_tab) {
    const bool self = self_trans && !mixture;
    float maxE = -3.40282346638528859812e+38f;
#pragma unroll 1
    for (int s = 0; s < K; ++s) {
        const float e = hml_emit_E<K>(l, mdl, s, self, sx, sq, N);
        maxE = (e < maxE) ? maxE : e;
    }
#pragma unroll 1
    for (int s = 0; s < K; ++s) {
        const float e = hml_emit_E<K>(l, mdl, s, self, sx, sq, N);
        if (eprobe) eprobe[(uint64_t)b * K + s] = e;
        em[hml_bk(lay, b, K, s)] = hml_expf_lean(e - maxE, exp_tab);
        if (!mixture && gsc) gsc[hml_bk(lay, b, K, s)] = self ? hml_expf_lean((N - 1.0f) * l.logA[s], exp_tab) : 1.0f;
    }
}

template <int K>
HML_KERNEL __launch_bounds__(256) void hml_k_emission(const float2* __restrict__ bstat,
                                                      const uint32_t* __restrict__ starts, hml_model* __restrict__ mdl,
                                                      float* __restrict__ em, float* __restrict__ gsc,
                                                      float* __restrict__ eprobe, int mixture, const hml_layout lay) {
    const uint32_t B = mdl->B;
    hml_emit_params<K> p;
    hml_emit_load<K>(p, mdl, mixture);
    const uint32_t stride = gridDim.x * blockDim.x;
    for (uint32_t b = blockIdx.x * blockDim.x + threadIdx.x; b < B; b += stride) {
        const float2 st = bstat[b];
        const float N = (float)(starts[b + 1] - starts[b]);
        hml_emit_block<K>(p, mdl, b, st.x, st.y, N, em, gsc, eprobe, mixture, lay);
    }
}

template <int K>
__device__ __forceinline__ void hml_b_stats_emission(const float2* __restrict__ ia, const uint32_t* __restrict__ starts,
                                                            hml_model* __restrict__ mdl, float2* __restrict__ bstat,
                                                            float* __restrict__ em, float* __restrict__ gsc,
                                                            float* __restrict__ eprobe, int mixture, const hml_layout lay) {
    const uint32_t B = mdl->B;
    hml_emit_params<K> p;
    hml_emit_load<K>(p, mdl, mixture);
    const uint32_t stride = gridDim.x * blockDim.x;
    for (uint32_t b = blockIdx.x * blockDim.x + threadIdx.x; b < B; b += stride) {
        const uint32_t s = starts[b], e = starts[b + 1];
        float sx, sq;
        hml_block_stats_one(ia, s, e, sx, sq);
        bstat[b] = make_float2(sx, sq);
        hml_emit_block<K>(p, mdl, b, sx, sq, (float)(e - s), em, gsc, eprobe, mixture, lay);
    }
}
template <int K>
HML_KERNEL __launch_bounds__(256) void hml_k_stats_emission(const float2* __restrict__ ia, const uint32_t* __restrict__ starts,
                                                            hml_model* __restrict__ mdl, float2* __restrict__ bstat,
                                                            float* __restrict__ em, float* __restrict__ gsc,
                                                            float* __restrict__ eprobe, int mixture, const hml_layout lay) {
    hml_b_stats_emission<K>(ia, starts, mdl, bstat, em, gsc, eprobe, mixture, lay);
}


template <int K, bool STATS>
HML_KERNEL __launch_bounds__(256) void hml_k_emission_mv(const float2* __restrict__ ia, const uint32_t* __restrict__ starts,
                                                         hml_model* __restrict__ mdl, float2* __restrict__ bstat,
                                                         float* __restrict__ em, float* __restrict__ gsc,
                                                         float* __restrict__ eprobe, int mixture, const hml_layout lay) {
    __shared__ float s_mu[HML_MAX_K], s_var[HML_MAX_K], s_logNs[K], s_logA[K];
    __shared__ double s_rvar[HML_MAX_K];
    __shared__ uint8_t s_map[K][HML_MAX_D];
    __shared__ uint64_t s_tab[32];
    const uint32_t B = mdl->B;
    const int D = mdl->D;
    const uint64_t T = mdl->T;
    const bool self = mdl->self_trans != 0 && !mixture;
    if (threadIdx.x < (unsigned)mdl->P) { s_mu[threadIdx.x] = mdl->mu[threadIdx.x]; s_var[threadIdx.x] = mdl->var[threadIdx.x]; s_rvar[threadIdx.x] = mdl->rvar2[threadIdx.x]; }
    if (threadIdx.x < (unsigned)K) {
        s_logNs[threadIdx.x] = mdl->logNs[threadIdx.x]; s_logA[threadIdx.x] = mdl->logA[threadIdx.x];
        for (int d = 0; d < HML_MAX_D; ++d) s_map[threadIdx.x][d] = mdl->map[threadIdx.x][d];
    }
    if (threadIdx.x >= 64 && threadIdx.x < 96) s_tab[threadIdx.x - 64] = HML_EXP2F_TAB[threadIdx.x - 64];
    __syncthreads();
    const uint32_t stride = gridDim.x * blockDim.x;
    for (uint32_t b = blockIdx.x * blockDim.x + threadIdx.x; b < B; b += stride) {
        const uint32_t st = starts[b], en = starts[b + 1];
        float sx[HML_MAX_D], sq[HML_MAX_D];
        for (int d = 0; d < D; ++d) {
            if (STATS) {
                hml_block_stats_one(ia + (uint64_t)d * (T + 1u), st, en, sx[d], sq[d]);
                bstat[(uint64_t)d * T + b] = make_float2(sx[d], sq[d]);
            } else {
                const float2 v = bstat[(uint64_t)d * T + b];
                sx[d] = v.x; sq[d] = v.y;
            }
        }
        const float N = (float)(en - st);
        float E[K];
        float maxE = -3.40282346638528859812e+38f;
#pragma unroll
        for (int s = 0; s < K; ++s) {
            float r = 0.0f;
// ... 432 lines not shown
```

### hammlet_amd/csrc/hml_state.h

```cpp
#ifndef HML_STATE_H
#define HML_STATE_H

#include "hml_common.h"
#include "hml_philox.h"

#define HML_TRE_HALO_MAX 128
#define HML_SPAN 4096
#define HML_GROUP_SPANS 16
#define HML_REDUCE_CHUNK 256
#define HML_REDUCE_GROUPS 1024
#define HML_BWD_CHUNK 64
#define HML_FWD_GROUP 16
struct hml_layout {
    uint32_t lshift;
    uint32_t cstride;
};
HML_HD uint64_t hml_bk(const hml_layout lay, uint32_t b, int K, int s) {
    const uint32_t r = b & ((1u << lay.lshift) - 1u), c = b >> lay.lshift;
    return ((uint64_t)r * (uint32_t)K + (uint32_t)s) * lay.cstride + c;
}

#define HML_CNT_SPLIT 16

enum {
    HML_DEVERR_NONE = 0,
    HML_DEVERR_IP_NOT_FINITE = 1,
    HML_DEVERR_NEG_BACKWARD = 2,
    HML_DEVERR_NEG_SUMSQ = 3,
    HML_DEVERR_NIG_ALPHA = 4,
    HML_DEVERR_NIG_BETA = 5,
    HML_DEVERR_NIG_NU = 6,
    HML_DEVERR_NIG_MU0 = 7,
    HML_DEVERR_MEAN_NOT_FINITE = 8,
    HML_DEVERR_VAR_NOT_FINITE = 9,
    HML_DEVERR_VAR_NOT_POSITIVE = 10,
    HML_DEVERR_TOO_MANY_RECORDS = 11,
    HML_DEVERR_LAUNCH_GEOMETRY = 12
};

#define HML_MAX_D 4

struct hml_model {
    int32_t K;
    int32_t D, P;
    uint8_t map[HML_CAP_K][HML_MAX_D];
    float logNs[HML_CAP_K];
    uint64_t stat_stride;
    int32_t self_trans;
    int32_t dynamic;
    uint32_t T;
    float nig_prior[4];
    float a_off, a_diag, pi_alpha;
    hml_key key;
    float mu[HML_CAP_K], var[HML_CAP_K], sd[HML_CAP_K];
    double rvar2[HML_CAP_K];
    float logN[HML_CAP_K];
    float logA[HML_CAP_K];
    float A[HML_CAP_K * HML_CAP_K];
    float pi[HML_CAP_K];
    float thr;
    float thr_theta;
    float nig_post[HML_CAP_K][4];
    float dirA[HML_CAP_K * HML_CAP_K];
    float dirPi[HML_CAP_K];
    uint32_t B;
    uint32_t n_spans;
    uint32_t cap;
    uint32_t halted;
    unsigned long long trans[HML_CNT_SPLIT][HML_MAX_K * HML_MAX_K];
    unsigned long long occ[HML_CNT_SPLIT][HML_MAX_K];
    unsigned long long last_trans[HML_CAP_K * HML_CAP_K];
    unsigned long long last_occ[HML_CAP_K];
    float last_sum[HML_CAP_K], last_sumsq[HML_CAP_K];
    unsigned long long epoch;
    unsigned long long sweeps, block_updates, uniform_fallbacks, forward_refits, forward_serial;
    unsigned long long fused_fallbacks;
    unsigned long long n_recorded;
    int32_t max_state_recorded;
    uint32_t err_code;
    float err_value;
    unsigned long long err_count;
    uint32_t fwd_mismatch;
    uint32_t fwd_mismatch2;
    uint32_t fwd_W, fwd_W0, fwd_serial_ran, fwd_quiet;
    uint32_t fwd_W_burnin;
    uint32_t fwd_burnin_sweeps;
    uint32_t fwd_quiet_need;
    uint32_t tre_fused;
    uint32_t tre_hi_shift, tre_lo_shift;
    uint32_t tre_W_floor, tre_floor_age;
    unsigned long long fwd_refits_seen, fwd_serial_seen;
    uint32_t params_ticket;
    unsigned long long dbg_t[12];
    uint32_t wl_lshift, wl_cstride;
    uint32_t wl_bwd_W, wl_bwd_quiet;
    uint32_t wl_W_need, wl_need_age;
    uint32_t wl_retry;
    unsigned long long n_levels_recorded;
    unsigned long long n_breaks_recorded;
    unsigned long long n_bands_recorded;
};

#if defined(__HIPCC__)
__device__ __forceinline__ void hml_halt(hml_model* mdl, uint32_t found, uint32_t* host_words) {
    mdl->B = 0u;
    mdl->halted = found;
    if (host_words) {
        __hip_atomic_store(host_words, found, __ATOMIC_RELAXED, __HIP_MEMORY_SCOPE_SYSTEM);
        __hip_atomic_store(host_words + 2, found, __ATOMIC_RELAXED, __HIP_MEMORY_SCOPE_SYSTEM);
    }
}
__device__ __forceinline__ void hml_warmup_for_many_blocks(hml_model* mdl, uint32_t B) {
    if (B >= (1u << 22) && !mdl->tre_fused && mdl->sweeps < 4ull && mdl->fwd_W < 4u * mdl->fwd_W_burnin) mdl->fwd_W = 4u * mdl->fwd_W_burnin;
    if (B >= (1u << 22) && mdl->tre_fused && mdl->sweeps < 4ull && mdl->fwd_W < 64u) mdl->fwd_W = 64u;
}
#endif

#endif
```

### hammlet_amd/csrc/hml_sweep.hip

```cpp
#include "hml_capi_shared.hpp"

template <int KK>
static bool fused_geometry(hml_ctx* c, uint32_t* n_sub, uint32_t* n_wg) {
    if (c->fused_slots == 0) {
        int per_cu = 0, cus = 0;
        if (hipOccupancyMaxActiveBlocksPerMultiprocessor(&per_cu, hml_k_blocks_fused<KK>, HML_FUSED_WAVES * 64, 0) != hipSuccess ||
            hipDeviceGetAttribute(&cus, hipDeviceAttributeMultiprocessorCount, c->device) != hipSuccess || per_cu <= 0 || cus <= 0) {
            (void)hipGetLastError();
            c->fused_slots = -1;
        } else {
            c->fused_slots = per_cu * cus;
        }
        if (const char* e = getenv("HML_FUSED_SLOTS")) c->fused_slots = atoi(e);
    }
    if (c->fused_slots <= 0) return false;
    const uint64_t batches = (c->T + HML_FUSED_SUB_POSITIONS - 1) / HML_FUSED_SUB_POSITIONS;
    const uint64_t m = (batches + (uint64_t)c->fused_slots - 1) / (uint64_t)c->fused_slots;
    if (m > HML_FUSED_MAX_SUB) return false;
    *n_sub = (uint32_t)m;
    *n_wg = (uint32_t)((c->T + m * HML_FUSED_SUB_POSITIONS - 1) / (m * HML_FUSED_SUB_POSITIONS));
    return true;
}


template <int KK>
static int sweep_k(hml_ctx* c, char method, bool record) {
    hipStream_t s = c->stream;
    const bool mix = (method == HML_METHOD_MIXTURE);
    const uint32_t T = (uint32_t)c->T;
    bool emitted = false, fused = false;
    if (c->hint_stale && (c->dynamic || !c->blocks_valid)) {
        hipStreamCaptureStatus cap = hipStreamCaptureStatusNone;
        if (hipStreamIsCapturing(s, &cap) == hipSuccess && cap == hipStreamCaptureStatusNone) {
            launch_compact_pair(c, 0, 0.0f);
            KLAUNCH_CHECK();
            HIPCHK(hipStreamSynchronize(s));
        }
    }
    c->hint_stale = false;
    refresh_hint(c);
    const bool dense_geo = c->B_hint >= c->dense_min_blocks;
    const bool trellis = dense_geo && !mix && c->D == 1 && c->tre_fused;
    const bool mid_geo = !dense_geo && c->fwdL_mid > c->fwdL && c->B_hint >= c->mid_min_blocks;
    const int L = dense_geo ? c->fwdL_dense : mid_geo ? c->fwdL_mid : c->fwdL;
    const hml_layout lay = dense_geo ? c->lay_dense : mid_geo ? c->lay_mid : c->lay;
    float* const gsc_plane = (!dense_geo && c->late_rescale) ? nullptr : c->d_gsc;
    const uint32_t* const starts_for_maps = gsc_plane ? nullptr : c->d_starts;
    if (c->dynamic || !c->blocks_valid) {
        uint32_t n_sub = 0u, n_wg = 0u;
        if (c->h_B[1] && !c->fused_keep) c->fused_blocks = false;
        if (c->D == 1 && c->use_keys && c->fused_blocks && !shares_device(c) &&
            !(!c->summary_always && c->B_hint && (uint64_t)c->B_hint * 24u > c->T) && fused_geometry<KK>(c, &n_sub, &n_wg)) {
            ProfScope ps(c, "blocks_compact", 1);
            hipLaunchKernelGGL(HIP_KERNEL_NAME(hml_k_blocks_fused<KK>), dim3(n_wg), dim3(HML_FUSED_WAVES * 64), 0, s, c->d_summary, c->d_w, c->d_ia,
                               T, c->d_mdl, c->key_base, c->d_group_word, c->d_stage, c->d_starts, c->d_bstat, c->d_em,
                               gsc_plane, c->probes ? c->d_eprobe : nullptr, mix ? 1 : 0, lay, c->d_hB, n_sub, c->fused_spin_limit, c->d_dbg, c->d_mdl);
            fused = true;
        } else {
            launch_compact_pair(c, 0, 0.0f);
        }
        if (!fused && !trellis) {
            refresh_hint(c);
            const uint32_t h0 = c->B_hint ? c->B_hint : (uint32_t)std::min<uint64_t>(c->T, 1u << 20);
            ProfScope ps(c, "stats_emission");
            if (c->D > 1)
                hipLaunchKernelGGL(HIP_KERNEL_NAME(hml_k_emission_mv<KK, true>), dim3(grid_for(h0, 256, 64, 16384)), dim3(256), 0, s,
                                   c->d_ia, c->d_starts, c->d_mdl, c->d_bstat, c->d_em, gsc_plane, c->probes ? c->d_eprobe : nullptr,
                                   mix ? 1 : 0, lay);
            else if (dense_geo && L <= hml_emit_tile<KK>::MAXL)
                hipLaunchKernelGGL(HIP_KERNEL_NAME(hml_k_emission_tiled<KK, true>), dim3(grid_for(h0, hml_emit_tile<KK>::BLOCKS, 64, 65536)),
                                   dim3(256), 0, s, c->d_ia, c->d_starts, c->d_mdl, c->d_bstat, c->d_em, gsc_plane,
                                   c->probes ? c->d_eprobe : nullptr, mix ? 1 : 0, lay);
            else
            hipLaunchKernelGGL(HIP_KERNEL_NAME(hml_k_stats_emission<KK>), dim3(grid_for(h0, 256, 64, 16384)), dim3(256), 0, s,
                               c->d_ia, c->d_starts, c->d_mdl, c->d_bstat, c->d_em, gsc_plane, c->probes ? c->d_eprobe : nullptr,
                               mix ? 1 : 0, lay);
        }
        KLAUNCH_CHECK();
        emitted = true;
        if (!c->dynamic) c->blocks_valid = true;
    }
    refresh_hint(c);
    const uint32_t hint = c->B_hint ? c->B_hint : (uint32_t)std::min<uint64_t>(c->T, 1u << 20);
    const int gB = grid_for(hint, 256, 64, 16384);
    if (!emitted && !trellis) {
        ProfScope ps(c, "emission");
        if (c->D > 1)
            hipLaunchKernelGGL(HIP_KERNEL_NAME(hml_k_emission_mv<KK, false>), dim3(gB), dim3(256), 0, s, c->d_ia, c->d_starts, c->d_mdl,
                               c->d_bstat, c->d_em, gsc_plane, c->probes ? c->d_eprobe : nullptr, mix ? 1 : 0, lay);
        else if (dense_geo && L <= hml_emit_tile<KK>::MAXL)
            hipLaunchKernelGGL(HIP_KERNEL_NAME(hml_k_emission_tiled<KK, false>), dim3(grid_for(hint, hml_emit_tile<KK>::BLOCKS, 64, 65536)),
                               dim3(256), 0, s, c->d_ia, c->d_starts, c->d_mdl, c->d_bstat, c->d_em, gsc_plane,
                               c->probes ? c->d_eprobe : nullptr, mix ? 1 : 0, lay);
        else
        hipLaunchKernelGGL(HIP_KERNEL_NAME(hml_k_emission<KK>), dim3(gB), dim3(256), 0, s, c->d_bstat, c->d_starts, c->d_mdl,
                           c->d_em, gsc_plane, c->probes ? c->d_eprobe : nullptr, mix ? 1 : 0, lay);
    }
    if (trellis) {
        hipStreamCaptureStatus capst = hipStreamCaptureStatusNone;
        (void)hipStreamIsCapturing(s, &capst);
        bool measure = false;
        if (c->tre_rows && c->tre_slots == 0) {
            int per_cu = 0, cus = 0;
            if (hipOccupancyMaxActiveBlocksPerMultiprocessor(&per_cu, hml_k_trellis_rows<KK, false>, 64 * HML_TR2_WAVES, 0) == hipSuccess &&
                hipDeviceGetAttribute(&cus, hipDeviceAttributeMultiprocessorCount, c->device) == hipSuccess && per_cu > 0 && cus > 0)
                c->tre_slots = per_cu * cus * HML_TR2_WAVES;
            else { (void)hipGetLastError(); c->tre_slots = -1; }
            if (const char* e = getenv("HML_TRELLIS_SLOTS")) c->tre_slots = atoi(e);
        }
        const uint32_t TL = tre_pick_L(c, hint, capst != hipStreamCaptureStatusNone, &measure);
        hipEvent_t tev0 = nullptr, tev1 = nullptr;
        if (measure) { tev0 = ev_get(c); tev1 = ev_get(c); hipEventRecord(tev0, s); }
        if (c->graph_tre_L != TL && getenv("HML_TRELLIS_TUNE_DEBUG")) fprintf(stderr, "[trellis] chunk length %u for %u blocks (%d wavefront slots)\n", TL, hint, c->tre_slots);
        c->graph_tre_L = TL;
        const uint64_t tchunks = ((uint64_t)hint + TL - 1) / TL;
        const uint64_t tgroups = (tchunks + HML_TRE_NCH - 1) / HML_TRE_NCH;
        float* ep = c->probes ? c->d_eprobe : nullptr;
        float* ap = c->probes ? c->d_aprobe : nullptr;
        {
            ProfScope ps(c, "trellis", 1);
            if (c->tre_rows && hint > 1024u && ((uint64_t)hint - 1024u) * 8u >= c->T * 9u)
                hipLaunchKernelGGL(HIP_KERNEL_NAME(hml_k_trellis_rows<KK, true>), dim3(grid_for(tgroups, HML_TR2_WAVES, 4, 1 << 20)), dim3(64 * HML_TR2_WAVES), 0, s,
                                   c->d_ia, c->d_starts, c->d_mdl, c->d_mdl, c->d_bstat, c->d_smap, c->d_cmap, c->d_entry, c->d_exitA, c->d_fb, ep, ap, c->d_tre_ckpt, TL);
            else if (c->tre_rows)
                hipLaunchKernelGGL(HIP_KERNEL_NAME(hml_k_trellis_rows<KK, false>), dim3(grid_for(tgroups, HML_TR2_WAVES, 4, 1 << 20)), dim3(64 * HML_TR2_WAVES), 0, s,
                                   c->d_ia, c->d_starts, c->d_mdl, c->d_mdl, c->d_bstat, c->d_smap, c->d_cmap, c->d_entry, c->d_exitA, c->d_fb, ep, ap, c->d_tre_ckpt, TL);
            else
            hipLaunchKernelGGL(HIP_KERNEL_NAME(hml_k_trellis_tile<KK>), dim3(grid_for(tgroups, 1, 16, 1 << 20)), dim3(64), 0, s,
                               c->d_ia, c->d_starts, c->d_mdl, c->d_mdl, c->d_bstat, c->d_smap, c->d_cmap, c->d_entry, c->d_exitA, c->d_fb, ep, ap, TL);
        }
        {
            ProfScope ps(c, "trellis_repair");
            hipLaunchKernelGGL(HIP_KERNEL_NAME(hml_k_trellis_verify<KK>), dim3(grid_for(tchunks, 256, 16, 1 << 14)), dim3(256), 0, s, c->d_mdl,
                               c->d_entry, c->d_exitA, c->d_redo, TL);
            int in_a = 1;
            for (uint32_t round = 0; round < c->tre_refit_rounds; ++round, in_a ^= 1) {
                uint32_t* lin = in_a ? c->d_redo : c->d_redo2;
                uint32_t* lout = in_a ? c->d_redo2 : c->d_redo;
                hipLaunchKernelGGL(HIP_KERNEL_NAME(hml_k_trellis_refit<KK>), dim3(4096), dim3(64), 0, s, c->d_ia, c->d_starts, c->d_mdl, c->d_smap,
                                   c->d_cmap, c->d_entry, c->d_exitA, c->d_fb, ep, ap, lin, in_a, (c->tre_rows && c->tre_ckpt) ? c->d_tre_ckpt : nullptr, TL);
                hipLaunchKernelGGL(HIP_KERNEL_NAME(hml_k_trellis_verify_list<KK>), dim3(64), dim3(256), 0, s, c->d_mdl, c->d_entry, c->d_exitA,
                                   lin, lout, c->d_touched, in_a, round, TL);
            }
            hipLaunchKernelGGL(HIP_KERNEL_NAME(hml_k_trellis_serial<KK>), dim3(1), dim3(256), 0, s, c->d_ia, c->d_starts, c->d_mdl, c->d_smap,
                               c->d_cmap, c->d_entry, c->d_exitA, c->d_fb, ep, ap, in_a ? c->d_redo : c->d_redo2, in_a, c->d_tre_bitmap, TL);
        }
        {
            ProfScope ps(c, "backward_chain");
            const uint64_t supers = (tchunks + 63) / 64;
            hipLaunchKernelGGL(HIP_KERNEL_NAME(hml_k_trellis_super<KK>), dim3(grid_for(supers * 64, 256, 16, 1 << 16)), dim3(256), 0, s, c->d_cmap,
                               c->d_mdl, c->d_scmap, c->d_super, TL);
            hipLaunchKernelGGL(HIP_KERNEL_NAME(hml_k_trellis_chain<KK>), dim3(1), dim3(1024), 0, s, c->d_super, c->d_mdl, c->d_bentry2, TL);
            hipLaunchKernelGGL(HIP_KERNEL_NAME(hml_k_trellis_states<KK>), dim3(grid_for(tgroups, 1, 16, 1 << 20)), dim3(64), 0, s, c->d_smap,
                               c->d_scmap, c->d_bentry2, c->d_mdl, c->d_q, TL);
        }
        if (measure) {
            hipEventRecord(tev1, s);
            float ms = 0.0f;
            const bool ok = hipEventSynchronize(tev1) == hipSuccess && hipEventElapsedTime(&ms, tev0, tev1) == hipSuccess;
            c->ev_pool.push_back(tev0);
            c->ev_pool.push_back(tev1);
            if (ok) tre_tune_report(c, hint, ms); else { (void)hipGetLastError(); c->tre_autotune = false; }
        }
        c->tre_dense_sweeps++;
        {
            ProfScope ps(c, "counts");
            hipLaunchKernelGGL(HIP_KERNEL_NAME(hml_k_counts_dense<KK, false>), dim3(HML_REDUCE_GROUPS), dim3(256), 0, s, c->d_q,
                               c->d_starts, c->d_bstat, c->d_mdl, c->d_partial, (const unsigned long long*)nullptr, (const uint8_t*)nullptr);
        }
    } else if (!mix) {
        const uint64_t chunks = ((uint64_t)hint + L - 1) / L;
        const int gF = grid_for(chunks, 256, 16, 1 << 20);
        {
            ProfScope ps(c, "forward");
            hipLaunchKernelGGL(HIP_KERNEL_NAME(hml_k_forward<KK>), dim3(gF), dim3(256), 0, s, c->d_em, gsc_plane, c->d_mdl, c->d_rows,
                               c->probes ? c->d_aprobe : nullptr, c->d_entry, c->d_exitA, c->d_fb, L, lay);
        }
        {
            const uint64_t bch = ((uint64_t)hint + HML_BWD_CHUNK - 1) / HML_BWD_CHUNK;
            {
                ProfScope ps(c, "backward_maps");
                hipLaunchKernelGGL(HIP_KERNEL_NAME(hml_k_backward_maps<KK>), dim3(grid_for(bch * 64, 256, 16, 1 << 18)), dim3(256), 0,
                                   s, c->d_rows, c->d_mdl, c->d_smap, c->d_cmap, lay, c->d_entry, c->d_exitA, c->d_redo, L, starts_for_maps, c->d_mdl);
            }
            ProfScope ps(c, "backward_chain");
            if (!dense_geo) {
                hipLaunchKernelGGL(HIP_KERNEL_NAME(hml_k_backward_chain<KK>), dim3(1), dim3(1024), 0, s, c->d_cmap, c->d_mdl,
                                   c->d_bentry, c->d_em, gsc_plane, c->d_rows, c->probes ? c->d_aprobe : nullptr, c->d_entry,
                                   c->d_exitA, c->d_fb, c->d_redo, c->d_touched, c->d_smap, L, lay, 3, 0, starts_for_maps);
            } else {
                hipLaunchKernelGGL(HIP_KERNEL_NAME(hml_k_backward_chain<KK>), dim3(1), dim3(1024), 0, s, c->d_cmap, c->d_mdl,
                                   c->d_bentry, c->d_em, gsc_plane, c->d_rows, c->probes ? c->d_aprobe : nullptr, c->d_entry,
                                   c->d_exitA, c->d_fb, c->d_redo, c->d_touched, c->d_smap, L, lay, 1, 0, starts_for_maps);
                hipLaunchKernelGGL(HIP_KERNEL_NAME(hml_k_backward_super<KK>), dim3(grid_for(bch, 256, 16, 1 << 16)), dim3(256), 0, s,
                                   c->d_cmap, c->d_mdl, c->d_scmap, c->d_super);
                hipLaunchKernelGGL(HIP_KERNEL_NAME(hml_k_backward_chain<KK>), dim3(1), dim3(1024), 0, s, c->d_super, c->d_mdl,
                                   c->d_bentry2, c->d_em, gsc_plane, c->d_rows, c->probes ? c->d_aprobe : nullptr, c->d_entry,
                                   c->d_exitA, c->d_fb, c->d_redo, c->d_touched, c->d_smap, L, lay, 2, 1, starts_for_maps);
                hipLaunchKernelGGL(hml_k_backward_entries, dim3(grid_for(bch, 256, 16, 1 << 16)), dim3(256), 0, s, c->d_scmap,
                                   c->d_bentry2, c->d_mdl, c->d_bentry);
            }
        }
        {
            ProfScope ps(c, "counts");
            if (c->D > 1)
                hipLaunchKernelGGL(HIP_KERNEL_NAME(hml_k_counts<KK, true, true>), dim3(HML_REDUCE_GROUPS), dim3(256), 0, s, c->d_q,
                                   c->d_starts, c->d_bstat, c->d_mdl, c->d_partial, c->d_smap, c->d_bentry);
            else if (dense_geo)
                hipLaunchKernelGGL(HIP_KERNEL_NAME(hml_k_counts_dense<KK, true>), dim3(HML_REDUCE_GROUPS), dim3(256), 0, s, c->d_q,
                                   c->d_starts, c->d_bstat, c->d_mdl, c->d_partial, c->d_smap, c->d_bentry);
            else
            hipLaunchKernelGGL(HIP_KERNEL_NAME(hml_k_counts<KK, true>), dim3(HML_REDUCE_GROUPS), dim3(256), 0, s, c->d_q,
                               c->d_starts, c->d_bstat, c->d_mdl, c->d_partial, c->d_smap, c->d_bentry);
        }
    } else {
        {
            ProfScope ps(c, "mixture");
            hipLaunchKernelGGL(HIP_KERNEL_NAME(hml_k_mixture<KK>), dim3(gB), dim3(256), 0, s, c->d_em, c->d_mdl, c->d_q, lay);
        }
        {
            ProfScope ps(c, "counts");
            if (c->D > 1)
                hipLaunchKernelGGL(HIP_KERNEL_NAME(hml_k_counts<KK, false, true>), dim3(HML_REDUCE_GROUPS), dim3(256), 0, s, c->d_q,
                                   c->d_starts, c->d_bstat, c->d_mdl, c->d_partial, (const unsigned long long*)nullptr,
                                   (const uint8_t*)nullptr);
            else if (dense_geo)
                hipLaunchKernelGGL(HIP_KERNEL_NAME(hml_k_counts_dense<KK, false>), dim3(HML_REDUCE_GROUPS), dim3(256), 0, s, c->d_q,
                                   c->d_starts, c->d_bstat, c->d_mdl, c->d_partial, (const unsigned long long*)nullptr,
                                   (const uint8_t*)nullptr);
            else
            hipLaunchKernelGGL(HIP_KERNEL_NAME(hml_k_counts<KK, false>), dim3(HML_REDUCE_GROUPS), dim3(256), 0, s, c->d_q,
                               c->d_starts, c->d_bstat, c->d_mdl, c->d_partial, (const unsigned long long*)nullptr,
                               (const uint8_t*)nullptr);
        }
    }
    if (record && c->rec_marginals) {
        if (c->pooled) return set_err(HML_ERR_ARG, "the marginals of this context are pooled (common labels, several chains): further sweeps cannot be recorded into them");
        if (int r = ensure_marginal_buffers(c)) return r;
        ProfScope ps(c, "marginals");
        hipLaunchKernelGGL(hml_k_record, dim3(gB), dim3(256), 0, s, c->d_q, c->d_starts, c->d_mdl, c->d_diff, c->d_boundary);
    }
    {
        ProfScope ps(c, "params");
        if (c->params_spread) hipLaunchKernelGGL(HIP_KERNEL_NAME(hml_k_params_spread<KK>), dim3(HML_PARAMS_TREE_WGS), dim3(1024), 0, s, c->d_mdl, c->d_partial);
        else hipLaunchKernelGGL(HIP_KERNEL_NAME(hml_k_params<KK>), dim3(1), dim3(1024), 0, s, c->d_mdl, c->d_partial, 0);
    }
    if (record) { if (int r = launch_recorders(c, s, hint)) return r; }
    KLAUNCH_CHECK();
    return 0;
}


template <int KK>
static int iterate_many_k(hml_ctx* const* cs, int n, uint64_t first, uint64_t iterations, uint64_t thinning, uint64_t* done) {
    hml_ctx* c0 = cs[0];
    hipStream_t s = c0->stream;
    const uint32_t T = (uint32_t)c0->T;
    const int L = c0->fwdL_many;
    const int with_gsc = c0->late_rescale ? 0 : 1;
    const uint32_t n_groups = (c0->n_spans + HML_GROUP_SPANS - 1) / HML_GROUP_SPANS;
    const bool records = thinning > 0 && thinning <= iterations;
    unsigned long long rec_mask = 0ull;
    for (int i = 0; i < n; ++i) {
        if (records) { if (int r = ensure_recorders(cs[i])) return r; }
        if (records && cs[i]->rec_marginals) {
            if (cs[i]->pooled) return set_err(HML_ERR_ARG, "the marginals of a context are pooled (common labels, several chains): further sweeps cannot be recorded into them");
            if (int r = ensure_marginal_buffers(cs[i])) return r;
            rec_mask |= 1ull << i;
        }
    }
    std::vector<hml_chain_dev> h(n);
    for (int i = 0; i < n; ++i) {
        hml_ctx* c = cs[i];
        hml_chain_dev& d = h[i];
        d.summary = c->d_summary; d.w = c->d_w; d.ia = c->d_ia; d.key_base = c->key_base; d.n_spans = c->n_spans;
        d.stage = c->d_stage; d.span_count = c->d_span_count; d.coarse1 = c->d_coarse1; d.starts = c->d_starts; d.host_B = c->d_hB;
        d.bstat = c->d_bstat; d.mdl = c->d_mdl; d.em = c->d_em; d.gsc = c->d_gsc; d.rows = c->d_rows; d.entry = c->d_entry; d.exitv = c->d_exitA;
        d.fb = c->d_fb; d.redo = c->d_redo; d.touched = c->d_touched; d.smap = c->d_smap; d.cmap = c->d_cmap; d.bentry = c->d_bentry;
        d.q = c->d_q; d.partial = c->d_partial; d.diff = c->d_diff; d.boundary = c->d_boundary; d.lay = c->lay_many;
    }
    if (c0->many_cap < n) {
        if (c0->d_many) HIPCHK(hipFree(c0->d_many));
        c0->d_many = nullptr; c0->many_cap = 0;
        HIPCHK(hipMalloc(&c0->d_many, n * sizeof(hml_chain_dev)));
        c0->many_cap = n;
    }
    HIPCHK(hipMemcpyAsync(c0->d_many, h.data(), n * sizeof(hml_chain_dev), hipMemcpyHostToDevice, s));
    HIPCHK(hipStreamSynchronize(s));
    const hml_chain_dev* d_cs = (const hml_chain_dev*)c0->d_many;
    int G = n >= 2 ? 2 : 1;
    if (const char* e = getenv("HML_MANY_GROUPS")) G = std::max(1, std::min(std::min(atoi(e), 4), n));
    struct Grp { int first, count; hipStream_t s; };
    std::vector<Grp> grp(G);
    for (int g = 0; g < G; ++g) { grp[g].first = (int)((int64_t)g * n / G); grp[g].count = (int)((int64_t)(g + 1) * n / G) - grp[g].first; grp[g].s = cs[grp[g].first]->stream; }
    bool fm = c0->trace != nullptr && c0->fused_blocks;
    for (int k = 0; k < n; ++k) fm = fm && cs[k]->trace == c0->trace && cs[k]->fused_blocks && cs[k]->key_base == c0->key_base;
    uint32_t fm_sub = 0u, fm_wg = 0u;
    bool fm_split = true;
    if (const char* e = getenv("HML_FM_SPLIT")) fm_split = atoi(e) != 0;
    uint32_t fs_sub = 1u, fs_wg = 0u;
    const uint64_t fs_tiles1 = (c0->T + HML_FUSED_SUB_POSITIONS - 1) / HML_FUSED_SUB_POSITIONS;
    {
        const uint64_t batches = (c0->T + HML_FUSED_SUB_POSITIONS - 1) / HML_FUSED_SUB_POSITIONS;
        fs_sub = (uint32_t)std::max<uint64_t>(1, (batches + 4095) / 4096);
        if (const char* e = getenv("HML_FM_SPLIT_SUB")) fs_sub = (uint32_t)std::max(1, atoi(e));
        if (fs_sub > HML_FUSED_MAX_SUB) fm_split = false;
        fs_wg = (uint32_t)((c0->T + (uint64_t)fs_sub * HML_FUSED_SUB_POSITIONS - 1) / ((uint64_t)fs_sub * HML_FUSED_SUB_POSITIONS));
    }
    if (fm && !fm_split) {
        if (c0->fm_slots == 0) {
            int per_cu = 0, cus = 0;
            if (hipOccupancyMaxActiveBlocksPerMultiprocessor(&per_cu, hml_m_blocks_fused<KK>, HML_FUSED_WAVES * 64, 0) != hipSuccess ||
                hipDeviceGetAttribute(&cus, hipDeviceAttributeMultiprocessorCount, c0->device) != hipSuccess || per_cu <= 0 || cus <= 0) {
                (void)hipGetLastError();
                c0->fm_slots = -1;
            } else c0->fm_slots = per_cu * cus;
            if (const char* e = getenv("HML_FUSED_MANY_SLOTS")) c0->fm_slots = atoi(e);
        }
        const uint64_t batches = (c0->T + HML_FUSED_SUB_POSITIONS - 1) / HML_FUSED_SUB_POSITIONS;
        const int live = c0->device < 64 ? g_live_ctx[c0->device].load() : n;
        const int sharers = G * std::max(1, (live + n - 1) / n);
        const int64_t slots = c0->fm_slots > 0 ? std::max<int64_t>(1, c0->fm_slots / sharers) : 0;
        const uint64_t m = slots > 0 ? (batches + (uint64_t)slots - 1) / (uint64_t)slots : HML_FUSED_MAX_SUB + 1;
        if (m > HML_FUSED_MAX_SUB) fm = false;
        else { fm_sub = (uint32_t)m; fm_wg = (uint32_t)((c0->T + m * HML_FUSED_SUB_POSITIONS - 1) / (m * HML_FUSED_SUB_POSITIONS)); }
    }
// ... 116 lines not shown
```

### include/hml.h

```cpp
#ifndef HML_H
#define HML_H

#include <stddef.h>
#include <stdint.h>

#ifdef __cplusplus
extern "C" {
#endif

typedef struct hml_ctx hml_ctx;

#define HML_METHOD_FB 'F'
#define HML_METHOD_MIXTURE 'M'

#define HML_OK 0
#define HML_ERR_ARG 1
#define HML_ERR_HIP 2
#define HML_ERR_MODEL 3

const char* hml_last_error(void);

uint32_t hml_abi_version(void);
const char* hml_device_arch(void);
int hml_device_count(int* n);

int hml_create(hml_ctx** out, int device, uint64_t seed, uint32_t chain_id, void* stream);
void hml_destroy(hml_ctx* ctx);

int hml_load_observations(hml_ctx* ctx, const float* x, uint64_t n_values);
int hml_load_observations_device(hml_ctx* ctx, const void* x_dev, uint64_t T);

int hml_attach_observations(hml_ctx* ctx, hml_ctx* source);

typedef struct hml_text hml_text;
int hml_text_open(hml_text** out, int device, uint64_t chunk_bytes);
void hml_text_close(hml_text* reader);
int hml_text_buffer(hml_text* reader, char** buf, uint64_t* capacity);
int hml_text_commit(hml_text* reader, uint64_t nbytes);
int hml_text_feed(hml_text* reader, const char* bytes, uint64_t nbytes);
int hml_text_reserve(hml_text* reader, uint64_t n_values);
int hml_text_finish(hml_text* reader, uint64_t* n_values, int* stopped);
int hml_text_values(hml_text* reader, float* out );
int hml_text_counters(hml_text* reader, uint64_t* bytes_in, uint64_t* irregular_tokens, uint64_t* host_chunks);

int hml_set_dimensions(hml_ctx* ctx, int D, int P);
int hml_get_dimensions(hml_ctx* ctx, int* D, int* P);

int hml_set_weights(hml_ctx* ctx, const float* w, uint64_t T);

int hml_noise_sigma(hml_ctx* ctx, double* sigma);

int hml_scale_weights(hml_ctx* ctx, float multiplier);

int hml_autoprior(hml_ctx* ctx, float s2, float p, float out4[4]);

int hml_set_model(hml_ctx* ctx, int K, const float nig4[4], float a_off, float a_diag, float pi_alpha,
                  int self_trans);

int hml_set_self_transitions(hml_ctx* ctx, int on);

int hml_sample_prior(hml_ctx* ctx);

int hml_set_static_blocks(hml_ctx* ctx);
int hml_set_dynamic(hml_ctx* ctx, int on);

int hml_create_blocks(hml_ctx* ctx, float threshold);

int hml_iterate(hml_ctx* ctx, char method, uint64_t iterations, uint64_t thinning);

typedef void (*hml_record_cb)(hml_ctx* ctx, uint64_t sweep_in_call, void* user);
int hml_set_recording(hml_ctx* ctx, int marginals, hml_record_cb cb, void* user);

int hml_set_option(hml_ctx* ctx, const char* name, int value);

int hml_iterate_many(hml_ctx* const* ctxs, int n, char method, uint64_t iterations, uint64_t thinning);

int hml_sync(hml_ctx* ctx);

int hml_get_num_blocks(hml_ctx* ctx, uint64_t* B);
int hml_get_blocks(hml_ctx* ctx, uint32_t* starts );
int hml_get_block_stats(hml_ctx* ctx, float* sum , float* sum_sq );
int hml_get_states(hml_ctx* ctx, int16_t* q );
int hml_get_theta(hml_ctx* ctx, float* mean_var );
int hml_get_transitions(hml_ctx* ctx, float* A , float* pi );
int hml_set_parameters(hml_ctx* ctx, const float* mean_var, const float* A, const float* pi);
int hml_get_threshold(hml_ctx* ctx, float* thr);
int hml_enable_probes(hml_ctx* ctx, int on);
int hml_get_block_loglik(hml_ctx* ctx, float* E );
int hml_get_forward_rows(hml_ctx* ctx, float* rows );
int hml_get_counts(hml_ctx* ctx, uint64_t* trans , uint64_t* occ , float* sum ,
                   float* sum_sq , uint64_t* nterms );
int hml_get_weights(hml_ctx* ctx, float* w );
int hml_get_coefficients(hml_ctx* ctx, float* c );
int hml_get_integral_array(hml_ctx* ctx, float* sum , float* sum_sq );

int hml_marginals_rle(hml_ctx* ctx, uint64_t* n_segments, int* n_columns, uint64_t* seg_len ,
                      int32_t* counts );
int hml_max_segmentation(hml_ctx* ctx, uint64_t* n_runs, uint64_t* run_len , int32_t* run_state );
int hml_marginals_dense_device(hml_ctx* ctx, void* out_dev, const int32_t* perm);
int hml_recorded_sweeps(hml_ctx* ctx, uint64_t* n);

int hml_set_level_recording(hml_ctx* ctx, int on);
int hml_levels_rle(hml_ctx* ctx, uint64_t* n_segments, uint64_t* n_recorded, uint64_t* seg_len ,
                   double* sum , double* sum_sq );
int hml_levels_dense_device(hml_ctx* ctx, void* out_dev );
int hml_levels_merge(hml_ctx* dst, hml_ctx* src);
int hml_levels_on_segments(hml_ctx* ctx, uint64_t n_cuts, const uint32_t* cuts ,
                           double* sum , double* sum_sq );

int hml_levels_agreement_rle(hml_ctx* const* ctxs, int n, uint64_t* n_segments, uint64_t* n_recorded, uint64_t* seg_len ,
                             double* within , double* between , double* rhat );
int hml_levels_agreement_dense_device(hml_ctx* const* ctxs, int n, void* out_dev );
int hml_levels_agreement_summary(hml_ctx* const* ctxs, int n, double threshold, uint64_t* n_above , double* max_finite ,
                                 uint64_t* n_infinite );

int hml_set_break_recording(hml_ctx* ctx, int on);
int hml_breaks_list(hml_ctx* ctx, uint64_t* n_breaks, uint64_t* n_recorded, uint32_t* pos , uint32_t* count );
int hml_breaks_dense_device(hml_ctx* ctx, void* out_dev , uint32_t window);
int hml_breaks_merge(hml_ctx* dst, hml_ctx* src);
int hml_breaks_consensus(hml_ctx* ctx, uint32_t window, uint64_t min_count, uint64_t* n_selected, uint32_t* pos ,
                         uint64_t* mass , uint32_t* peak );

int hml_set_level_bands(hml_ctx* ctx, int n_edges, const float* edges );
int hml_get_level_bands(hml_ctx* ctx, int* n_edges, float* edges );
int hml_bands_rle(hml_ctx* ctx, uint64_t* n_segments, int* n_columns, uint64_t* n_recorded, uint64_t* seg_len ,
                  int32_t* counts );
int hml_bands_dense_device(hml_ctx* ctx, void* out_dev , int cumulative);
int hml_bands_call(hml_ctx* ctx, uint64_t rank, uint64_t* n_runs, uint64_t* run_len , int32_t* run_band );
int hml_bands_merge(hml_ctx* dst, hml_ctx* src);

int hml_categorical_draw(hml_ctx* ctx, const float* weights, int K, uint32_t* index);

int hml_relabel_permutation(hml_ctx* ctx, int32_t* perm );
int hml_pool_payload_size(hml_ctx* ctx, uint64_t* n_int32);
int hml_pool_export(hml_ctx* ctx, void* payload_dev, int32_t* perm_out_or_null);
int hml_pool_install(hml_ctx* ctx, const void* payload_dev);
typedef struct hml_pool hml_pool;
#define HML_POOL_ID_BYTES 128
int hml_pool_unique_id(void* id );
int hml_pool_create(hml_pool** out, int device, int rank, int n_ranks, const void* id);
void hml_pool_destroy(hml_pool* pool);
int hml_pool_marginals(hml_pool* pool, hml_ctx* ctx, int32_t* perm_out_or_null);
int hml_pool_info(hml_pool* pool, int* rank, int* n_ranks, double* last_allreduce_ms, uint64_t* last_bytes, int* rccl_version);
int hml_pool_set_form(hml_pool* pool, int form);
int hml_pool_last(hml_pool* pool, int* form, uint64_t* entries);
int hml_allreduce_marginals(hml_ctx* const* ctxs, int n);
int hml_allreduce_marginals_perm(hml_ctx* const* ctxs, int n, int32_t* perms );
int hml_pool_permutation(hml_ctx* ctx, int32_t* perm );

typedef struct {
    uint64_t sweeps;
    uint64_t block_updates;
    uint64_t uniform_fallbacks;
    uint64_t forward_refits;
    uint64_t forward_serial;
    uint64_t forward_warmup;
    uint64_t fused_fallbacks;
    uint64_t buffer_growths;
    uint64_t block_capacity;
} hml_stats;
int hml_get_stats(hml_ctx* ctx, hml_stats* out);

int hml_profile_enable(hml_ctx* ctx, int level);
int hml_profile_get(hml_ctx* ctx, const char* name, double* total_ms, uint64_t* launches);

int hml_debug_eval(int device, int fn, const float* a, const float* b_or_null, float* out, uint64_t n, uint64_t seed);

int hml_synth_gauss(float* x, int16_t* states_or_null, uint64_t T, int K, const float* mu, float sigma,
                    double mean_dwell, uint64_t seed, int nthreads);

int hml_synth_depth(float* x, int16_t* states_or_null, uint64_t T, double depth, double ln_sigma, uint64_t seed, int nthreads);

#ifdef __cplusplus
}
#endif
#endif
```

Baseline: 3.072 billion block-updates/s.

## Fuse forward filtering into the fused block-compaction kernel with a halo lookback

Adds a variant of the fused block-compaction kernel that also runs the chunked forward filter for its own blocks. Each workgroup finds up to 32 preceding block boundaries (a halo) so it can warm up the forward recursion locally. Emission terms are kept in LDS, which avoids a separate forward kernel launch and rereading the emission plane from HBM. In exchange the kernel uses more LDS and registers, which may lower occupancy, and it only runs when the geometry and residency checks pass. Warmups that the halo cuts short can change the numerics, and these are counted.

```diff
diff --git a/hammlet_amd/capi.py b/hammlet_amd/capi.py
--- a/hammlet_amd/capi.py
+++ b/hammlet_amd/capi.py
@@ -17,7 +17,8 @@
 class HmlStats(C.Structure):
     _fields_ = [("sweeps", C.c_uint64), ("block_updates", C.c_uint64), ("uniform_fallbacks", C.c_uint64),
                 ("forward_refits", C.c_uint64), ("forward_serial", C.c_uint64), ("forward_warmup", C.c_uint64),
-                ("fused_fallbacks", C.c_uint64), ("buffer_growths", C.c_uint64), ("block_capacity", C.c_uint64)]
+                ("fused_fallbacks", C.c_uint64), ("buffer_growths", C.c_uint64), ("block_capacity", C.c_uint64),
+                ("fused_forward_sweeps", C.c_uint64), ("fused_forward_short_warmups", C.c_uint64)]
 
 
 RECORD_CB = C.CFUNCTYPE(None, C.c_void_p, C.c_uint64, C.c_void_p)
@@ -70,6 +71,7 @@
     "hml_enable_probes": (C.c_int, [_P, C.c_int]),
     "hml_get_block_loglik": (C.c_int, [_P, _P]),
     "hml_get_forward_rows": (C.c_int, [_P, _P]),
+    "hml_get_stored_rows": (C.c_int, [_P, _P]),
     "hml_get_counts": (C.c_int, [_P, _P, _P, _P, _P, _P]),
     "hml_get_weights": (C.c_int, [_P, _P]),
     "hml_get_coefficients": (C.c_int, [_P, _P]),
@@ -367,6 +369,11 @@
         _check(self.lib.hml_get_forward_rows(self.h, r.ctypes.data))
         return r
 
+    def stored_rows(self):
+        r = np.empty((self.num_blocks(), self.K), np.float32)
+        _check(self.lib.hml_get_stored_rows(self.h, r.ctypes.data))
+        return r
+
     def counts(self):
         K = self.K
         trans = np.empty((K, K), np.uint64)
diff --git a/hammlet_amd/csrc/hml_capi.hip b/hammlet_amd/csrc/hml_capi.hip
--- a/hammlet_amd/csrc/hml_capi.hip
+++ b/hammlet_amd/csrc/hml_capi.hip
@@ -179,6 +179,7 @@
     if (const char* e = getenv("HML_USE_GRAPH")) c->use_graph = atoi(e) != 0;
     if (const char* e = getenv("HML_WEIGHT_KEYS")) c->use_keys = atoi(e) != 0;
     if (const char* e = getenv("HML_FUSED_BLOCKS")) { c->fused_blocks = atoi(e) != 0; c->fused_keep = atoi(e) == 2; }
+    if (const char* e = getenv("HML_FUSED_FORWARD")) c->fused_forward = atoi(e) != 0;
     if (const char* e = getenv("HML_TRELLIS_FUSED")) c->tre_fused = atoi(e) != 0;
     if (const char* e = getenv("HML_TRELLIS_L")) { const int l = atoi(e); c->tre_L = (l <= 0) ? 0u : (l >= HML_TRE_MAX_L) ? (uint32_t)HML_TRE_MAX_L : (l < 32) ? 32u : (uint32_t)l / 32u * 32u; }
     if (const char* e = getenv("HML_TRELLIS_CKPT")) c->tre_ckpt = atoi(e) != 0;
@@ -1118,6 +1119,7 @@
 }
 
 static int sweep_dispatch(hml_ctx* c, char method, bool record) {
+    c->rows_plain = false;
     if (c->compat) return sweep_compat(c, method, record);
     if (c->wide) return sweep_wide(c, method, record);
     HML_KTAB(c->K, kt);
@@ -1205,6 +1207,7 @@
         }
         int r = 0;
         uint64_t reached = done;
+        for (int i = 0; i < n; ++i) cs[i]->rows_plain = false;
         { HML_KTAB(cs[0]->K, kt); r = kt->iterate_many(cs, n, done, iterations, thinning, &reached); }
         if (r) return r;
         hipEvent_t ev = ev_get(cs[0]);
@@ -1260,6 +1263,11 @@
     if (std::string(name) == "fused_blocks") {
         c->fused_blocks = value != 0;
         c->fused_keep = value == 2;
+        if (c->graph_exec) { hipGraphExecDestroy(c->graph_exec); c->graph_exec = nullptr; }
+        return 0;
+    }
+    if (std::string(name) == "fused_forward") {
+        c->fused_forward = value != 0;
         if (c->graph_exec) { hipGraphExecDestroy(c->graph_exec); c->graph_exec = nullptr; }
         return 0;
     }
@@ -1411,6 +1419,18 @@
     HIPCHK(hipMemcpy(rows, c->d_aprobe, ((uint64_t)b + 1) * c->K * sizeof(float), hipMemcpyDeviceToHost));
     return 0;
 }
+int hml_get_stored_rows(hml_ctx* c, float* rows) {
+    NEED_MODEL();
+    if (!c->rows_plain) return set_err(HML_ERR_ARG, "the last sweep kept no unscaled forward rows in the chunk-transposed layout");
+    uint32_t b; if (int r = current_B(c, &b)) return r;
+    const hml_layout lay = c->rows_lay;
+    const uint64_t plane = ((uint64_t)c->K << lay.lshift) * lay.cstride;
+    std::vector<float> h(plane);
+    HIPCHK(hipMemcpy(h.data(), c->d_rows, plane * sizeof(float), hipMemcpyDeviceToHost));
+    for (uint32_t i = 0; i < b; ++i)
+        for (int s = 0; s < c->K; ++s) rows[(uint64_t)i * c->K + s] = h[hml_bk(lay, i, c->K, s)];
+    return 0;
+}
 int hml_get_counts(hml_ctx* c, uint64_t* trans, uint64_t* occ, float* sum, float* sum_sq, uint64_t* nterms) {
     NEED_MODEL();
     hml_model m; if (int r = fetch_model(c, &m)) return r;
@@ -1482,6 +1502,7 @@
     out->forward_warmup = m.fwd_W;
     out->fused_fallbacks = m.fused_fallbacks;
     out->buffer_growths = c->grown; out->block_capacity = c->cap;
+    out->fused_forward_sweeps = m.ff_sweeps; out->fused_forward_short_warmups = m.ff_short_warmups;
     return 0;
 }
 
diff --git a/hammlet_amd/csrc/hml_ctx.hpp b/hammlet_amd/csrc/hml_ctx.hpp
--- a/hammlet_amd/csrc/hml_ctx.hpp
+++ b/hammlet_amd/csrc/hml_ctx.hpp
@@ -65,6 +65,8 @@
     uint32_t* d_wave_total = nullptr;
     int fused_slots = 0;
     uint32_t fused_spin_limit = 4096;
+    bool fused_forward = true;
+    int fused_fwd_slots = 0;
     bool fused_keep = false;
     unsigned long long* d_dbg = nullptr;
     bool use_graph = false;
@@ -79,6 +81,8 @@
     uint32_t* d_redo2 = nullptr;
     uint32_t* d_tre_bitmap = nullptr;
     uint32_t* d_tre_ckpt = nullptr;
+    bool rows_plain = false;
+    hml_layout rows_lay = {2, 0};
     bool late_rescale = true;
     uint32_t tre_L = 0;
     bool tre_autotune = true;
diff --git a/hammlet_amd/csrc/hml_fused_select.h b/hammlet_amd/csrc/hml_fused_select.h
--- /dev/null
+++ b/hammlet_amd/csrc/hml_fused_select.h
@@ -0,0 +1,19 @@
+#ifndef HML_FUSED_SELECT_H
+#define HML_FUSED_SELECT_H
+
+#include <stdint.h>
+
+#define HML_FF_HALO 32
+#define HML_FF_TILE_TERMS 448
+#define HML_FF_MAX_K 6
+#define HML_FF_MAX_L 8
+
+static inline bool hml_fused_forward_wanted(bool option, bool mixture, int D, bool dense_geo, bool mid_geo, bool late_rescale, bool probes,
+                                            uint32_t n_sub, int K, int L, uint32_t seen_W) {
+    if (!option || mixture || D != 1 || dense_geo || mid_geo || !late_rescale || probes) return false;
+    if (n_sub != 1u || K < 2 || K > HML_FF_MAX_K) return false;
+    if (L < 1 || L > HML_FF_MAX_L || (L & (L - 1)) != 0) return false;
+    return seen_W <= (uint32_t)(HML_FF_HALO - L);
+}
+
+#endif
diff --git a/hammlet_amd/csrc/hml_k_blocks_forward.h b/hammlet_amd/csrc/hml_k_blocks_forward.h
--- /dev/null
+++ b/hammlet_amd/csrc/hml_k_blocks_forward.h
@@ -0,0 +1,142 @@
+#ifndef HML_K_BLOCKS_FORWARD_H
+#define HML_K_BLOCKS_FORWARD_H
+
+#include "hml_fused_select.h"
+#include "hml_k_blocks.h"
+#include "hml_k_forward.h"
+
+struct hml_fused_fwd_args {
+    float* rows;
+    float* entry;
+    float* exitv;
+    uint32_t* fb_count;
+};
+
+template <int K, int NW, bool ON>
+struct hml_ff_lds {};
+template <int K, int NW>
+struct hml_ff_lds<K, NW, true> {
+    float e[K][HML_FF_HALO + HML_FF_TILE_TERMS];
+    uint32_t look_pos[NW][HML_FF_HALO];
+    uint32_t look_n[NW];
+};
+
+template <class LDS>
+__device__ __forceinline__ void hml_ff_lookback(LDS& ff, const float* __restrict__ w, uint32_t T, float thr, const hml_swar_ge sw_ge,
+                                                bool has_span, uint32_t span, uint32_t word, int lane, int wave) {
+    uint32_t m[4] = {0u, 0u, 0u, 0u};
+    if (has_span) {
+        const uint32_t fl = hml_swar_ge_apply(sw_ge, word);
+#pragma unroll
+        for (int q = 0; q < 4; ++q) {
+            const bool origin = (span == 0u && q == 0 && lane == 0);
+            if (((fl >> (8 * q + 7)) & 1u) || origin) {
+                m[q] = hml_group_mask16(w, (uint64_t)span * HML_SPAN + (uint64_t)(64 * q + lane) * 16u, T, thr);
+                if (origin) m[q] |= 1u;
+            }
+        }
+    }
+    uint32_t above = 0u;
+#pragma unroll
+    for (int q = 3; q >= 0; --q) {
+        const uint32_t c = (uint32_t)__popc(m[q]);
+        uint32_t incl = c;
+#pragma unroll
+        for (int d = 1; d < 64; d <<= 1) {
+            const uint32_t o = __shfl_up(incl, d);
+            if (lane >= d) incl += o;
+        }
+        const uint32_t tot = __shfl(incl, 63);
+        uint32_t r = above + (tot - incl);
+        uint32_t mm = m[q];
+        while (mm) {
+            const uint32_t bit = 31u - (uint32_t)__clz((int)mm);
+            mm &= ~(1u << bit);
+            if (r < (uint32_t)HML_FF_HALO) ff.look_pos[wave][r] = span * (uint32_t)HML_SPAN + (uint32_t)(64 * q + lane) * 16u + bit;
+            ++r;
+        }
+        above += tot;
+    }
+    if (lane == 0) ff.look_n[wave] = above;
+}
+
+template <int NW, class LDS>
+__device__ __forceinline__ uint32_t hml_ff_round_count(const LDS& ff) {
+    uint32_t acc = 0u;
+#pragma unroll
+    for (int q = 0; q < NW; ++q) {
+        const uint32_t n = ff.look_n[q];
+        if (acc < (uint32_t)HML_FF_HALO) acc += n < (uint32_t)HML_FF_HALO ? n : (uint32_t)HML_FF_HALO;
+    }
+    return acc < (uint32_t)HML_FF_HALO ? acc : (uint32_t)HML_FF_HALO;
+}
+template <int NW, class LDS>
+__device__ __forceinline__ uint32_t hml_ff_round_pos(const LDS& ff, uint32_t j) {
+    uint32_t acc = 0u, pos = 0u;
+    bool found = false;
+#pragma unroll
+    for (int q = 0; q < NW; ++q) {
+        const uint32_t n = ff.look_n[q];
+        const uint32_t nk = n < (uint32_t)HML_FF_HALO ? n : (uint32_t)HML_FF_HALO;
+        if (!found && j < acc + nk) { pos = ff.look_pos[q][j - acc]; found = true; }
+        acc += nk;
+    }
+    return pos;
+}
+
+template <int K, int NT, class LDS>
+__device__ __forceinline__ void hml_ff_filter(const LDS& ff, hml_model* __restrict__ mdl, const hml_model* __restrict__ mdl_ro,
+                                              const float* __restrict__ em, const hml_fused_fwd_args fa, const hml_layout lay,
+                                              uint32_t fb0, uint32_t nb, bool last_wg, uint32_t n_halo_blocks, uint32_t W) {
+    hml_fwd_ctx<K> cx;
+    cx.A.attach(mdl_ro, nullptr);
+    cx.invK = (float)(1.0 / (double)(float)K);
+    cx.self = mdl_ro->self_trans != 0;
+    cx.B = 0u;
+    const uint32_t L = 1u << lay.lshift;
+    const uint32_t end_blk = fb0 + nb;
+    const uint32_t c_lo = fb0 >> lay.lshift;
+    const uint32_t c_end = last_wg ? (end_blk + L - 1u) >> lay.lshift : end_blk >> lay.lshift;
+    const uint32_t lo = fb0 - n_halo_blocks;
+    auto terms = [&](uint32_t b, float (&e)[K]) {
+        const uint32_t ti = b + (uint32_t)HML_FF_HALO - fb0;
+        if (ti < (uint32_t)(HML_FF_HALO + HML_FF_TILE_TERMS)) {
+#pragma unroll
+            for (int s = 0; s < K; ++s) e[s] = ff.e[s][ti];
+        } else {
+#pragma unroll
+            for (int s = 0; s < K; ++s) e[s] = em[hml_bk(lay, b, K, s)];
+        }
+    };
+    uint32_t n_short = 0u;
+    for (uint32_t c = c_lo + threadIdx.x; c < c_end; c += (uint32_t)NT) {
+        const uint32_t first = c << lay.lshift;
+        const uint32_t last = (first + L < end_blk) ? first + L : end_blk;
+        const bool exact = hml_fwd_chunk_exact(c, (int)L, (int)W);
+        uint32_t ws = exact ? 0u : first - W;
+        if (ws < lo) { ws = lo; if (!exact) ++n_short; }
+        float alpha[K], e[K];
+#pragma unroll
+        for (int s = 0; s < K; ++s) alpha[s] = exact ? mdl_ro->pi[s] : cx.invK;
+        for (uint32_t b = ws; b < first; ++b) {
+            terms(b, e);
+            (void)hml_fwd_step<K>(cx, alpha, e);
+        }
+#pragma unroll
+        for (int s = 0; s < K; ++s) fa.entry[(uint64_t)c * K + s] = alpha[s];
+        uint32_t nfb = 0u;
+        for (uint32_t b = first; b < last; ++b) {
+            terms(b, e);
+            if (hml_fwd_step<K>(cx, alpha, e)) ++nfb;
+#pragma unroll
+            for (int s = 0; s < K; ++s) fa.rows[hml_bk(lay, b, K, s)] = alpha[s];
+        }
+#pragma unroll
+        for (int s = 0; s < K; ++s) fa.exitv[(uint64_t)c * K + s] = alpha[s];
+        fa.fb_count[c] = nfb;
+        if (nfb) atomicAdd(&mdl->uniform_fallbacks, (unsigned long long)nfb);
+    }
+    if (n_short) atomicAdd(&mdl->ff_short_warmups, (unsigned long long)n_short);
+}
+
+#endif
diff --git a/hammlet_amd/csrc/hml_k_blocks_fused.h b/hammlet_amd/csrc/hml_k_blocks_fused.h
--- a/hammlet_amd/csrc/hml_k_blocks_fused.h
+++ b/hammlet_amd/csrc/hml_k_blocks_fused.h
@@ -3,6 +3,7 @@
 
 #include "hml_k_blocks.h"
 #include "hml_k_forward.h"
+#include "hml_k_blocks_forward.h"
 
 #define HML_FUSED_WAVES 8
 #define HML_FUSED_WAVE_BATCH (HML_SUM_SPANS * HML_SPAN)
@@ -41,8 +42,8 @@
     return hml_group_word(gen, total, last1 ? last1 - 1u : 0u);
 }
 
-template <int K>
-HML_KERNEL __launch_bounds__(HML_FUSED_WAVES * 64, 6) void hml_k_blocks_fused(const uint8_t* __restrict__ summary, const float* __restrict__ w,
+template <int K, bool FWD>
+__device__ __forceinline__ void hml_b_blocks_fused(const uint8_t* __restrict__ summary, const float* __restrict__ w,
                                                           const float2* __restrict__ ia, uint32_t T,
                                                           hml_model* __restrict__ mdl, int32_t base,
                                                           unsigned long long* __restrict__ group_word,
@@ -51,7 +52,7 @@
                                                           float* __restrict__ gsc, float* __restrict__ eprobe, int mixture,
                                                           const hml_layout lay, uint32_t* __restrict__ host_words,
                                                           uint32_t n_sub, uint32_t spin_limit, unsigned long long* __restrict__ dbg,
-                                                          const hml_model* __restrict__ mdl_ro) {
+                                                          const hml_model* __restrict__ mdl_ro, const hml_fused_fwd_args fa) {
     if (dbg && threadIdx.x == 0) dbg[blockIdx.x * 4 + 0] = wall_clock64();
     static_assert(HML_FUSED_MAX_SUB * HML_FUSED_SUB_POSITIONS == (1 << HML_FUSED_POS_BITS), "tile geometry (bit fields of hml_group_word)");
     static_assert(HML_FUSED_MAX_SUB * HML_FUSED_WAVE_BATCH <= 65536, "16-bit offsets into a wavefront's eighth");
@@ -67,6 +68,8 @@
     constexpr bool LOOPED = K > 6;
     __shared__ hml_emit_lds<LOOPED ? K : 1> sm_emit;
     if (LOOPED) hml_emit_lds_fill<LOOPED ? K : 1>(sm_emit, mdl_ro, (int)threadIdx.x);
+    static_assert(!FWD || K <= HML_FF_MAX_K, "the filter phase is built for the non-looped emission form");
+    __shared__ hml_ff_lds<K, NW, FWD> ff;
 
     const int lane = threadIdx.x & 63, wave = threadIdx.x >> 6;
     const uint32_t g = blockIdx.x;
@@ -119,9 +122,15 @@
             placed += sum;
         }
     };
+    const uint32_t kthr = (thr != thr) ? 0u : hml_weight_key(thr, base);
+    const hml_swar_ge sw_ge = hml_swar_ge_make(kthr);
+    const uint32_t tile_first_span = g * (uint32_t)NW * n_sub * (uint32_t)HML_SUM_SPANS;
+    uint32_t look_word = 0u;
+    if constexpr (FWD) {
+        if ((uint32_t)wave < tile_first_span)
+            look_word = __builtin_nontemporal_load(reinterpret_cast<const uint32_t*>(summary) + (uint64_t)(tile_first_span - 1u - (uint32_t)wave) * 64u + lane);
+    }
     {
-        const uint32_t kthr = (thr != thr) ? 0u : hml_weight_key(thr, base);
-        const hml_swar_ge sw_ge = hml_swar_ge_make(kthr);
         auto load_batch = [&](uint32_t j, uint32_t (&gw)[HML_SUM_SPANS]) {
             const uint32_t span0 = (uint32_t)(wave_base / HML_SPAN) + j * HML_SUM_SPANS;
 #pragma unroll
@@ -182,6 +191,8 @@
         __hip_atomic_store(&group_word[g], hml_group_word(gen, wg_total, l1 ? l1 - 1u : 0u), __ATOMIC_RELAXED, __HIP_MEMORY_SCOPE_AGENT);
     }
     if ((uint32_t)(wave_base / HML_SPAN) < n_spans) expand(last_batch, n_listed);
+    if constexpr (FWD)
+        hml_ff_lookback(ff, w, T, thr, sw_ge, (uint32_t)wave < tile_first_span, tile_first_span - 1u - (uint32_t)wave, look_word, lane, wave);
     __syncthreads();
 
     auto start_at = [&](uint32_t k) -> uint32_t {
@@ -209,6 +220,21 @@
         first_n = first_t - prev_t;
         hml_block_stats_one(ia, prev_t, first_t, first_sx, first_sq);
         have_first = true;
+    }
+
+    uint32_t n_halo = 0u, h_hi = 0u, h_n = 0u;
+    float h_sx = 0.0f, h_sq = 0.0f;
+    bool h_have_hi = false, h_have = false;
+    const uint32_t h_i = NT - 1u - threadIdx.x;
+    if constexpr (FWD) {
+        n_halo = hml_ff_round_count<NW>(ff);
+        if (h_i < n_halo) { h_hi = hml_ff_round_pos<NW>(ff, h_i); h_have_hi = true; }
+        if (h_i + 1u < n_halo) {
+            const uint32_t h_lo = hml_ff_round_pos<NW>(ff, h_i + 1u);
+            h_n = h_hi - h_lo;
+            hml_block_stats_one(ia, h_lo, h_hi, h_sx, h_sq);
+            h_have = true;
+        }
     }
 
     unsigned long long acc = 0ull, near = 0ull;
@@ -252,6 +278,48 @@
     hml_emit_params<LOOPED ? 1 : K> p;
     if (!LOOPED) hml_emit_load<LOOPED ? 1 : K>(p, mdl_ro, mixture);
     const bool self_trans = mdl_ro->self_trans != 0;
+    const uint32_t fb0 = (g == 0u) ? 0u : before_group - 1u;
+    const uint32_t nb = n_items - ((g == 0u) ? 1u : 0u);
+    const bool ff_run = FWD && nb > 0u && before_group + n_items - 1u <= cap;
+    uint32_t ff_W = 0u;
+    if constexpr (FWD) {
+        const uint32_t Lf = 1u << lay.lshift;
+        const uint32_t Wcap = (uint32_t)HML_FF_HALO > Lf ? (uint32_t)HML_FF_HALO - Lf : 0u;
+        const uint32_t Wd = mdl_ro->fwd_W;
+        ff_W = Wd < Wcap ? Wd : Wcap;
+        uint32_t need_min = 0u;
+        if (ff_run && g > 0u) {
+            const uint32_t c_lo = fb0 >> lay.lshift;
+            const uint32_t c_end = last_wg ? (fb0 + nb + Lf - 1u) >> lay.lshift : (fb0 + nb) >> lay.lshift;
+            if (c_lo < c_end) need_min = hml_fwd_chunk_exact(c_lo, (int)Lf, (int)ff_W) ? before_group : fb0 - (c_lo << lay.lshift) + 1u;
+        }
+        for (uint32_t reach = (uint32_t)NW; n_halo < need_min && reach < tile_first_span; reach += (uint32_t)NW) {
+            __syncthreads();
+            const bool has = reach + (uint32_t)wave < tile_first_span;
+            const uint32_t span = tile_first_span - 1u - reach - (uint32_t)wave;
+            const uint32_t word = has ? reinterpret_cast<const uint32_t*>(summary)[(uint64_t)span * 64u + lane] : 0u;
+            hml_ff_lookback(ff, w, T, thr, sw_ge, has, span, word, lane, wave);
+            __syncthreads();
+            uint32_t n_r = hml_ff_round_count<NW>(ff);
+            if (n_r > (uint32_t)HML_FF_HALO - n_halo) n_r = (uint32_t)HML_FF_HALO - n_halo;
+            if (!h_have) {
+                if (!h_have_hi && h_i >= n_halo && h_i < n_halo + n_r) { h_hi = hml_ff_round_pos<NW>(ff, h_i - n_halo); h_have_hi = true; }
+                if (h_have_hi && h_i + 1u >= n_halo && h_i + 1u < n_halo + n_r) {
+                    const uint32_t h_lo = hml_ff_round_pos<NW>(ff, h_i + 1u - n_halo);
+                    h_n = h_hi - h_lo;
+                    hml_block_stats_one(ia, h_lo, h_hi, h_sx, h_sq);
+                    h_have = true;
+                }
+            }
+            n_halo += n_r;
+        }
+        if (h_have && ff_run) {
+            float E[K], ev[K], gv[K];
+            hml_emit_compute<K, true, false>(p, mdl, h_sx, h_sq, (float)h_n, mixture, E, ev, gv, false, sm_exp_tab);
+#pragma unroll
+            for (int s = 0; s < K; ++s) ff.e[s][(uint32_t)HML_FF_HALO - 1u - h_i] = ev[s];
+        }
+    }
     {
         uint32_t t = first_t, n = first_n;
         float sx = first_sx, sq = first_sq;
@@ -273,18 +341,70 @@
             bstat[b - 1u] = make_float2(sx, sq);
             if constexpr (LOOPED)
                 hml_emit_block_looped<K>(reinterpret_cast<const hml_emit_lds<K>&>(sm_emit), mdl, self_trans, b - 1u, sx, sq, (float)n, em, gsc, eprobe, mixture, lay, sm_exp_tab);
-            else
+            else if constexpr (FWD) {
+                float E[K], ev[K], gv[K];
+                hml_emit_compute<K, true>(p, mdl, sx, sq, (float)n, mixture, E, ev, gv, gsc != nullptr, sm_exp_tab);
+                hml_emit_store<K>(b - 1u, E, ev, gv, em, gsc, eprobe, mixture, lay);
+                const uint32_t ti = b - 1u - fb0;
+                if (ti < (uint32_t)HML_FF_TILE_TERMS) {
+#pragma unroll
+                    for (int s = 0; s < K; ++s) ff.e[s][(uint32_t)HML_FF_HALO + ti] = ev[s];
+                }
+            } else
                 hml_emit_block<LOOPED ? 1 : K, true>(p, mdl, b - 1u, sx, sq, (float)n, em, gsc, eprobe, mixture, lay, sm_exp_tab);
         }
+    }
+    if constexpr (FWD) {
+        __syncthreads();
+        if (ff_run) hml_ff_filter<K, (int)NT>(ff, mdl, mdl_ro, em, fa, lay, fb0, nb, last_wg, n_halo ? n_halo - 1u : 0u, ff_W);
     }
     if (dbg) { __syncthreads(); if (threadIdx.x == 0) dbg[blockIdx.x * 4 + 3] = wall_clock64(); }
     if (last_wg && threadIdx.x == 0) {
         const uint32_t Bn = before_group + wg_total;
         if (Bn > cap) { hml_halt(mdl, Bn, host_words); return; }
         mdl->B = Bn;
-        hml_warmup_for_many_blocks(mdl, Bn);
-        if (host_words) __hip_atomic_store(host_words, Bn, __ATOMIC_RELAXED, __HIP_MEMORY_SCOPE_SYSTEM);
+        const uint32_t Wd = mdl_ro->fwd_W;
+        if constexpr (FWD) {
+            if (ff_W < Wd) mdl->fwd_W = ff_W;
+            mdl->ff_sweeps += 1ull;
+        } else {
+            hml_warmup_for_many_blocks(mdl, Bn);
+        }
+        if (host_words) {
+            __hip_atomic_store(host_words, Bn, __ATOMIC_RELAXED, __HIP_MEMORY_SCOPE_SYSTEM);
+            __hip_atomic_store(host_words + 3, Wd, __ATOMIC_RELAXED, __HIP_MEMORY_SCOPE_SYSTEM);
+        }
     }
 }
 
+template <int K>
+HML_KERNEL __launch_bounds__(HML_FUSED_WAVES * 64, 6) void hml_k_blocks_fused(const uint8_t* __restrict__ summary, const float* __restrict__ w,
+                                                          const float2* __restrict__ ia, uint32_t T,
+                                                          hml_model* __restrict__ mdl, int32_t base,
+                                                          unsigned long long* __restrict__ group_word,
+                                                          uint16_t* __restrict__ stage, uint32_t* __restrict__ starts,
+                                                          float2* __restrict__ bstat, float* __restrict__ em,
+                                                          float* __restrict__ gsc, float* __restrict__ eprobe, int mixture,
+                                                          const hml_layout lay, uint32_t* __restrict__ host_words,
+                                                          uint32_t n_sub, uint32_t spin_limit, unsigned long long* __restrict__ dbg,
+                                                          const hml_model* __restrict__ mdl_ro) {
+    hml_b_blocks_fused<K, false>(summary, w, ia, T, mdl, base, group_word, stage, starts, bstat, em, gsc, eprobe, mixture, lay, host_words,
+                                 n_sub, spin_limit, dbg, mdl_ro, hml_fused_fwd_args{nullptr, nullptr, nullptr, nullptr});
+}
+
+template <int K>
+HML_KERNEL __launch_bounds__(HML_FUSED_WAVES * 64, 6) void hml_k_blocks_forward(const uint8_t* __restrict__ summary, const float* __restrict__ w,
+                                                          const float2* __restrict__ ia, uint32_t T,
+                                                          hml_model* __restrict__ mdl, int32_t base,
+                                                          unsigned long long* __restrict__ group_word,
+                                                          uint16_t* __restrict__ stage, uint32_t* __restrict__ starts,
+                                                          float2* __restrict__ bstat, float* __restrict__ em,
+                                                          float* __restrict__ gsc, float* __restrict__ eprobe, int mixture,
+                                                          const hml_layout lay, uint32_t* __restrict__ host_words,
+                                                          uint32_t n_sub, uint32_t spin_limit, unsigned long long* __restrict__ dbg,
+                                                          const hml_model* __restrict__ mdl_ro, const hml_fused_fwd_args fa) {
+    hml_b_blocks_fused<K, true>(summary, w, ia, T, mdl, base, group_word, stage, starts, bstat, em, gsc, eprobe, mixture, lay, host_words,
+                                n_sub, spin_limit, dbg, mdl_ro, fa);
+}
+
 #endif
diff --git a/hammlet_amd/csrc/hml_k_forward.h b/hammlet_amd/csrc/hml_k_forward.h
--- a/hammlet_amd/csrc/hml_k_forward.h
+++ b/hammlet_amd/csrc/hml_k_forward.h
@@ -39,7 +39,7 @@
     p.self = mdl->self_trans != 0 && !mixture;
 }
 
-template <int K, bool LEAN = false>
+template <int K, bool LEAN = false, bool RAISE = true>
 __device__ __forceinline__ void hml_emit_compute(const hml_emit_params<K>& p, hml_model* mdl, float sx, float sq, float N, int mixture,
                                                  float (&E)[K], float (&ev)[K], float (&gv)[K], bool want_g = true,
                                                  const uint64_t* exp_tab = nullptr) {
@@ -48,7 +48,7 @@
 #pragma unroll
     for (int s = 0; s < K; ++s) {
         const float ip = hml_inner_product(p.mu[s], p.var[s], p.rvar[s], sx, sq);
-        if (!hml_isfinite(ip)) hml_raise(mdl, HML_DEVERR_IP_NOT_FINITE, ip);
+        if (RAISE && !hml_isfinite(ip)) hml_raise(mdl, HML_DEVERR_IP_NOT_FINITE, ip);
         float e = (0.0f + ip) - N * p.logN[s];
         if (p.self) e += (N - 1.0f) * p.logA[s];
         E[s] = e;
diff --git a/hammlet_amd/csrc/hml_state.h b/hammlet_amd/csrc/hml_state.h
--- a/hammlet_amd/csrc/hml_state.h
+++ b/hammlet_amd/csrc/hml_state.h
@@ -99,6 +99,7 @@
     unsigned long long n_levels_recorded;
     unsigned long long n_breaks_recorded;
     unsigned long long n_bands_recorded;
+    unsigned long long ff_sweeps, ff_short_warmups;
 };
 
 #if defined(__HIPCC__)
diff --git a/hammlet_amd/csrc/hml_sweep.hip b/hammlet_amd/csrc/hml_sweep.hip
--- a/hammlet_amd/csrc/hml_sweep.hip
+++ b/hammlet_amd/csrc/hml_sweep.hip
@@ -24,11 +24,30 @@
 
 
 template <int KK>
+static bool fused_forward_resident(hml_ctx* c, uint32_t n_wg) {
+    if constexpr (KK <= HML_FF_MAX_K) {
+        if (c->fused_fwd_slots == 0) {
+            int per_cu = 0, cus = 0;
+            if (hipOccupancyMaxActiveBlocksPerMultiprocessor(&per_cu, hml_k_blocks_forward<KK>, HML_FUSED_WAVES * 64, 0) != hipSuccess ||
+                hipDeviceGetAttribute(&cus, hipDeviceAttributeMultiprocessorCount, c->device) != hipSuccess || per_cu <= 0 || cus <= 0) {
+                (void)hipGetLastError();
+                c->fused_fwd_slots = -1;
+            } else {
+                c->fused_fwd_slots = per_cu * cus;
+            }
+            if (getenv("HML_FUSED_SLOTS")) c->fused_fwd_slots = c->fused_slots;
+        }
+        return c->fused_fwd_slots > 0 && n_wg <= (uint32_t)c->fused_fwd_slots;
+    }
+    return false;
+}
+
+template <int KK>
 static int sweep_k(hml_ctx* c, char method, bool record) {
     hipStream_t s = c->stream;
     const bool mix = (method == HML_METHOD_MIXTURE);
     const uint32_t T = (uint32_t)c->T;
-    bool emitted = false, fused = false;
+    bool emitted = false, fused = false, fused_fwd = false;
     if (c->hint_stale && (c->dynamic || !c->blocks_valid)) {
         hipStreamCaptureStatus cap = hipStreamCaptureStatusNone;
         if (hipStreamIsCapturing(s, &cap) == hipSuccess && cap == hipStreamCaptureStatusNone) {
@@ -46,12 +65,24 @@
     const hml_layout lay = dense_geo ? c->lay_dense : mid_geo ? c->lay_mid : c->lay;
     float* const gsc_plane = (!dense_geo && c->late_rescale) ? nullptr : c->d_gsc;
     const uint32_t* const starts_for_maps = gsc_plane ? nullptr : c->d_starts;
+    c->rows_plain = !mix && !trellis && c->D == 1 && gsc_plane == nullptr;
+    c->rows_lay = lay;
     if (c->dynamic || !c->blocks_valid) {
         uint32_t n_sub = 0u, n_wg = 0u;
         if (c->h_B[1] && !c->fused_keep) c->fused_blocks = false;
         if (c->D == 1 && c->use_keys && c->fused_blocks && !shares_device(c) &&
             !(!c->summary_always && c->B_hint && (uint64_t)c->B_hint * 24u > c->T) && fused_geometry<KK>(c, &n_sub, &n_wg)) {
             ProfScope ps(c, "blocks_compact", 1);
+            if constexpr (KK <= HML_FF_MAX_K) {
+                fused_fwd = hml_fused_forward_wanted(c->fused_forward, mix, c->D, dense_geo, mid_geo, c->late_rescale, c->probes, n_sub, KK, L,
+                                                     c->h_B[3]) && fused_forward_resident<KK>(c, n_wg);
+                if (fused_fwd)
+                    hipLaunchKernelGGL(HIP_KERNEL_NAME(hml_k_blocks_forward<KK>), dim3(n_wg), dim3(HML_FUSED_WAVES * 64), 0, s, c->d_summary, c->d_w, c->d_ia,
+                                       T, c->d_mdl, c->key_base, c->d_group_word, c->d_stage, c->d_starts, c->d_bstat, c->d_em,
+                                       gsc_plane, (float*)nullptr, 0, lay, c->d_hB, n_sub, c->fused_spin_limit, c->d_dbg, c->d_mdl,
+                                       hml_fused_fwd_args{c->d_rows, c->d_entry, c->d_exitA, c->d_fb});
+            }
+            if (!fused_fwd)
             hipLaunchKernelGGL(HIP_KERNEL_NAME(hml_k_blocks_fused<KK>), dim3(n_wg), dim3(HML_FUSED_WAVES * 64), 0, s, c->d_summary, c->d_w, c->d_ia,
                                T, c->d_mdl, c->key_base, c->d_group_word, c->d_stage, c->d_starts, c->d_bstat, c->d_em,
                                gsc_plane, c->probes ? c->d_eprobe : nullptr, mix ? 1 : 0, lay, c->d_hB, n_sub, c->fused_spin_limit, c->d_dbg, c->d_mdl);
@@ -171,7 +202,7 @@
     } else if (!mix) {
         const uint64_t chunks = ((uint64_t)hint + L - 1) / L;
         const int gF = grid_for(chunks, 256, 16, 1 << 20);
-        {
+        if (!fused_fwd) {
             ProfScope ps(c, "forward");
             hipLaunchKernelGGL(HIP_KERNEL_NAME(hml_k_forward<KK>), dim3(gF), dim3(256), 0, s, c->d_em, gsc_plane, c->d_mdl, c->d_rows,
                                c->probes ? c->d_aprobe : nullptr, c->d_entry, c->d_exitA, c->d_fb, L, lay);
diff --git a/include/hml.h b/include/hml.h
--- a/include/hml.h
+++ b/include/hml.h
@@ -88,6 +88,7 @@
 int hml_enable_probes(hml_ctx* ctx, int on);
 int hml_get_block_loglik(hml_ctx* ctx, float* E );
 int hml_get_forward_rows(hml_ctx* ctx, float* rows );
+int hml_get_stored_rows(hml_ctx* ctx, float* rows );
 int hml_get_counts(hml_ctx* ctx, uint64_t* trans , uint64_t* occ , float* sum ,
                    float* sum_sq , uint64_t* nterms );
 int hml_get_weights(hml_ctx* ctx, float* w );
@@ -158,6 +159,8 @@
     uint64_t fused_fallbacks;
     uint64_t buffer_growths;
     uint64_t block_capacity;
+    uint64_t fused_forward_sweeps;
+    uint64_t fused_forward_short_warmups;
 } hml_stats;
 int hml_get_stats(hml_ctx* ctx, hml_stats* out);
 
```

Measured after the change: 2.772 billion block-updates/s. 0.902x the previous value.
